# zkkli/I-ViT

Hardware: AMD Instinct MI355X
Metric: images/sec + int8-MFMA-roofline% for DeiT-S bs256@224 on 1/2/4/8 MI355X (higher is better)
Workload: dtype int8; 1 GPU; deit_small int8 forward, batch 256/GPU, 224x224x3 synthetic int8 (BASELINE.json configs[1]: DeiT-S b256 on one GPU); weights seeded synthetic, activation scales from the reference calibration; global_batch=256, parallelism=dp1 (batch-sharded, weights RCCL-broadcast once), streams_per_gpu=1, hipgraph=False

## Files before the change

### i-vit_amd/_lib.py

```python
import ctypes
import os
import subprocess

_CSRC = os.path.join(os.path.dirname(os.path.abspath(__file__)), "csrc")
SO_PATH = os.environ.get("IVIT_LIB") or os.path.join(_CSRC, "libivit_hip.so")
SOURCES = ["ivit_hip.hip"] + sorted(f for f in os.listdir(_CSRC) if f.endswith(".h"))
_THIS = os.path.abspath(__file__)
HIPCC_FLAGS = ["--offload-arch=gfx950", "-O3", "-std=c++17", "-ffp-contract=off", "-Wno-pass-failed", "-fPIC", "-shared",
               "-Xclang", "-target-feature", "-Xclang", "-packed-fp32-ops"]


IVIT_OK, IVIT_ERR_INVALID, IVIT_ERR_HIP, IVIT_ERR_UNSUPPORTED, IVIT_ERR_NO_DEVICE = 0, 1, 2, 3, 4


class IvitError(RuntimeError):
    pass


class Dyadic(ctypes.Structure):
    _fields_ = [("m", ctypes.c_double), ("r", ctypes.c_double)]


def build(force=False, verbose=False):
    srcs = [os.path.join(_CSRC, s) for s in SOURCES]
# ... 1 lines not shown
    newest = max(os.path.getmtime(p) for p in srcs + [hdr, _THIS])
    if not force and os.path.exists(SO_PATH) and os.path.getmtime(SO_PATH) >= newest:
        return SO_PATH
    hipcc = os.environ.get("HIPCC", "/opt/rocm/bin/hipcc")
    import fcntl
    with open(SO_PATH + ".lock", "w") as lock:
        fcntl.flock(lock, fcntl.LOCK_EX)
        if not force and os.path.exists(SO_PATH) and os.path.getmtime(SO_PATH) >= newest:
            return SO_PATH
        tmp = "%s.%d.tmp" % (SO_PATH, os.getpid())
        cmd = [hipcc] + HIPCC_FLAGS + [os.path.join(_CSRC, "ivit_hip.hip"), "-o", tmp]
        if verbose:
            print(" ".join(cmd))
        try:
            subprocess.check_call(cmd)
            os.replace(tmp, SO_PATH)
        finally:
            if os.path.exists(tmp):
                os.remove(tmp)
    return SO_PATH


class VitConfig(ctypes.Structure):
    _fields_ = [(n, ctypes.c_int) for n in ("img_size", "patch_size", "in_chans", "embed_dim", "depth", "num_heads",
                                             "hidden_dim", "num_classes")]


class VitBlock(ctypes.Structure):
    _fields_ = [
        ("s_ln1", ctypes.c_float), ("n1_bias_int", ctypes.c_void_p), ("n1_sc", ctypes.c_void_p), ("n1_dy", ctypes.c_void_p),
        ("qkv_w", ctypes.c_void_p), ("qkv_b", ctypes.c_void_p), ("qkv_dy", ctypes.c_void_p),
        ("dy_qk", Dyadic), ("s_softmax", ctypes.c_float), ("dy_pv", Dyadic),
        ("exp_aq", ctypes.c_void_p), ("exp_t", ctypes.c_void_p), ("exp_cls", ctypes.c_void_p),
        ("exp_nc", ctypes.c_int), ("exp_tcount", ctypes.c_int), ("exp_dmin", ctypes.c_int),
        ("proj_w", ctypes.c_void_p), ("proj_b", ctypes.c_void_p), ("proj_dy", ctypes.c_void_p),
        ("res1_main", Dyadic), ("res1_res", Dyadic),
        ("s_ln2", ctypes.c_float), ("n2_bias_int", ctypes.c_void_p), ("n2_sc", ctypes.c_void_p), ("n2_dy", ctypes.c_void_p),
        ("fc1_w", ctypes.c_void_p), ("fc1_b", ctypes.c_void_p), ("fc1_dy", ctypes.c_void_p),
        ("s_gelu", ctypes.c_float), ("dy_gelu", Dyadic),
        ("fc2_w", ctypes.c_void_p), ("fc2_b", ctypes.c_void_p), ("fc2_dy", ctypes.c_void_p),
        ("res2_main", Dyadic), ("res2_res", Dyadic),
    ]


class VitParams(ctypes.Structure):
    _fields_ = [
        ("pe_w", ctypes.c_void_p), ("pe_b", ctypes.c_void_p), ("pe_dy", ctypes.c_void_p),
        ("z_cls", ctypes.c_void_p), ("pos", ctypes.c_void_p), ("dy_x", Dyadic), ("dy_pos", Dyadic),
        ("blocks_host", ctypes.POINTER(VitBlock)),
        ("s_ln", ctypes.c_float), ("n_bias_int", ctypes.c_void_p), ("n_sc", ctypes.c_void_p), ("n_dy", ctypes.c_void_p),
        ("head_w", ctypes.c_void_p), ("head_b", ctypes.c_void_p),
    ]


class LnParams(ctypes.Structure):
    _fields_ = [("bias_int", ctypes.c_void_p), ("sc", ctypes.c_void_p), ("dy", ctypes.c_void_p)]


class LinParams(ctypes.Structure):
    _fields_ = [("w", ctypes.c_void_p), ("b", ctypes.c_void_p), ("dy", ctypes.c_void_p)]


class SwinConfigC(ctypes.Structure):
    _fields_ = [(n, ctypes.c_int) for n in ("img_size", "patch_size", "in_chans", "embed_dim", "num_layers", "window_size",
                                             "mlp_ratio", "num_classes")] + [("depths", ctypes.c_int * 4), ("num_heads", ctypes.c_int * 4)]


class SwinBlock(ctypes.Structure):
    _fields_ = [
        ("s_in", ctypes.c_float), ("n1", LnParams), ("qkv", LinParams),
        ("dy_qk", Dyadic), ("dy_a", Dyadic), ("relb", ctypes.c_void_p),
        ("s_softmax", ctypes.c_float), ("dy_pv", Dyadic), ("proj", LinParams),
        ("res1_main", Dyadic), ("res1_res", Dyadic),
        ("s_mid", ctypes.c_float), ("n2", LnParams), ("fc1", LinParams), ("s_gelu", ctypes.c_float), ("dy_gelu", Dyadic),
        ("fc2", LinParams), ("res2_main", Dyadic), ("res2_res", Dyadic),
        ("exp_aq", ctypes.c_void_p), ("exp_t", ctypes.c_void_p), ("exp_cls", ctypes.c_void_p),
        ("exp_nc", ctypes.c_int), ("exp_tcount", ctypes.c_int), ("exp_dmin", ctypes.c_int),
    ]


class SwinMerge(ctypes.Structure):
    _fields_ = [("s_in", ctypes.c_float), ("n", LnParams), ("red", LinParams)]


class SwinParams(ctypes.Structure):
    _fields_ = [
        ("pe", LinParams), ("s_bn", ctypes.c_float), ("pn", LnParams), ("dy_qact1", ctypes.c_void_p),
        ("blocks_host", ctypes.POINTER(SwinBlock)), ("merges_host", ctypes.POINTER(SwinMerge)),
        ("s_norm_in", ctypes.c_float), ("n", LnParams), ("dy_pool", Dyadic),
        ("head_w", ctypes.c_void_p), ("head_b", ctypes.c_void_p), ("s_pool", ctypes.c_float),
    ]


_P = ctypes.c_void_p
_I = ctypes.c_int
_L = ctypes.c_int64
_F = ctypes.c_float

SIGNATURES = {
    "ivit_create": [ctypes.POINTER(_P), _I, _P],
    "ivit_destroy": [_P],
    "ivit_set_stream": [_P, _P],
    "ivit_set_cu_share": [_P, ctypes.c_int],
    "ivit_quantize_input_f32": [_P, _P, _F, _P, _L],
    "ivit_normalize_quantize_u8": [_P, _P, _I, _I, _I, ctypes.POINTER(_F), ctypes.POINTER(_F), _F, _P],
    "ivit_resize_center_crop_u8": [_P, _P, _I, _I, _I, _I, _I, _P, _P],
    "ivit_requant_i16": [_P, _P, _P, _I, _P, _P, _I, _P, _L, _I],
    "ivit_layernorm_tokenorder_requant": [_P, _P, _L, _I, _F, _P, _P, _P, _I, _P],
    "ivit_patch_norm_tokenorder": [_P, _P, _L, _I, _F, _P, _P, _P, Dyadic, _I, _P],
    "ivit_window_attention_fused": [_P, _P, Dyadic, Dyadic, _P, _F, Dyadic, _P, _I, _I, _I, _I, _I, _I],
    "ivit_window_attention_fused_lut": [_P, _P, Dyadic, Dyadic, _P, _F, _P, _P, _P, _I, _I, _I, Dyadic, _P, _I, _I, _I, _I, _I, _I],
    "ivit_mlp_plan_create": [_P, _P, _P, ctypes.POINTER(_P)],
    "ivit_mlp_fused_planned": [_P, _P, _P, _P, Dyadic, Dyadic, _P, _P, _L],
    "ivit_layernorm_mlp_fused_planned": [_P, _P, _P, _F, _P, _P, _P, _P, _P, Dyadic, Dyadic, _P, _L],
    "ivit_layernorm_mlp_lockstep_planned": [_P, _P, _P, _F, _P, _P, _P, _P, Dyadic, Dyadic, _P, _L],
    "ivit_mlp_fused": [_P, _P, _P, _P, _P, _P, _P, _P, _P, Dyadic, Dyadic, _P, _P, _L, _I, _I],
    "ivit_patch_merge_gather": [_P, _P, _I, _I, _I, _I, _P],
    "ivit_widen_i8_i16": [_P, _P, _P, _L],
    "ivit_linear_i8_requant8_store16": [_P, _P, _P, _P, _P, _P, _I, _I, _I],
    "ivit_patch_merge_layernorm_requant": [_P, _P, _I, _I, _I, _F, _P, _P, _P, _P],
    "ivit_swin_create": [_P, ctypes.POINTER(SwinConfigC), ctypes.POINTER(SwinParams), _I, ctypes.POINTER(_P)],
    "ivit_swin_destroy": [_P],
    "ivit_swin_workspace_bytes": [_P, _I, _I, ctypes.POINTER(ctypes.c_size_t)],
    "ivit_swin_forward": [_P, _P, _I, _I, _P, ctypes.c_size_t, _P],
    "ivit_swin_graph_create": [_P, _P, _I, _I, _P, ctypes.c_size_t, _P, ctypes.POINTER(_P)],
    "ivit_vit_create": [_P, ctypes.POINTER(VitConfig), ctypes.POINTER(VitParams), _I, ctypes.POINTER(_P)],
    "ivit_vit_destroy": [_P],
    "ivit_vit_workspace_bytes": [_P, _I, _I, ctypes.POINTER(ctypes.c_size_t)],
    "ivit_vit_fused_mlp_blocks": [_P, _I, ctypes.POINTER(_I)],
    "ivit_vit_fused_ln_mlp_blocks": [_P, _I, ctypes.POINTER(_I)],
    "ivit_vit_fused_qkv_blocks": [_P, _I, ctypes.POINTER(_I)],
    "ivit_vit_cls_tail": [_P, _I, ctypes.POINTER(_I)],
    "ivit_swin_fused_mlp_blocks": [_P, _I, ctypes.POINTER(_I * 4)],
    "ivit_vit_workspace_init": [_P, _P, ctypes.c_size_t, _I, _I],
    "ivit_vit_forward": [_P, _P, _I, _I, _P, ctypes.c_size_t, _P],
    "ivit_vit_graph_create": [_P, _P, _I, _I, _P, ctypes.c_size_t, _P, ctypes.POINTER(_P)],
    "ivit_graph_launch": [_P],
    "ivit_graph_destroy": [_P],
    "ivit_linear_i8": [_P, _P, _P, _P, _P, _I, _I, _I],
    "ivit_linear_i8_requant": [_P, _P, _P, _P, _P, _I, _P, _I, _I, _I],
    "ivit_linear_i8_requant_residual": [_P, _P, _P, _P, _P, Dyadic, Dyadic, _P, _P, _I, _I, _I],
    "ivit_linear_i8_qkv": [_P, _P, _P, _P, _P, _P, _P, _P, _I, _I, _I, _I, _I],
    "ivit_constants_upload": [_P, _P, ctypes.c_size_t, _P],
    "ivit_constants_broadcast": [_P, _P, ctypes.c_size_t, _I, _P],
    "ivit_linear_plan_create": [_P, _P, _P, _P, _I, _I, ctypes.POINTER(_P)],
    "ivit_linear_i8_requant_planned": [_P, _P, _P, _I, _P, _I],
    "ivit_linear_i8_requant_residual_planned": [_P, _P, _P, Dyadic, Dyadic, _P, _P, _I],
    "ivit_linear_i8_qkv_planned": [_P, _P, _P, _P, _P, _P, _I, _I, _I, _I, _I],
    "ivit_linear_plan_prepare_ws": [_P, _P],
    "ivit_layernorm_linear_i8_requant_planned": [_P, _P, _P, _F, _P, _P, _P, _P, _I],
    "ivit_linear_i8_requant_residual_layernorm_planned": [_P, _P, _P, Dyadic, Dyadic, _P, _P, _I, _F, _P, _P, _P, _P],
    "ivit_layernorm_linear_i8_qkv_planned": [_P, _P, _P, _F, _P, _P, _P, _P, _P, _P, _I, _I, _I, _I],
    "ivit_layernorm_linear_i8_qkv_ldv_planned": [_P, _P, _P, _F, _P, _P, _P, _P, _P, _P, _I, _I, _I, _I, _I],
    "ivit_bmm_nt_i8": [_P, _P, _P, _P, _I, _I, _I, _I, _I, _I, _I, _L, _L, _L],
    "ivit_bmm_nt_u16i8": [_P, _P, _P, _P, _I, _I, _I, _I, _I, _I, _I, _L, _L, _L],
    "ivit_attn_qk_requant": [_P, _P, _P, Dyadic, _P, _I, _I, _I, _I],
    "ivit_attn_pv_requant": [_P, _P, _P, Dyadic, _P, _I, _I, _I, _I, _I, _I],
    "ivit_attention_fused": [_P, _P, _P, _P, Dyadic, _F, Dyadic, _P, _I, _I, _I, _I, _I],
    "ivit_attention_fused_lut": [_P, _P, _P, _P, Dyadic, _F, _P, _P, _P, _I, _I, _I, Dyadic, _P, _I, _I, _I, _I, _I],
    "ivit_shiftmax_rowtable": [_P, _P, _P, _P, _I, _I, _I, _P],
    "ivit_attention_fused_rowlut": [_P, _P, _P, _P, Dyadic, _F, _P, _I, Dyadic, _P, _I, _I, _I, _I, _I],
    "ivit_attention_fused_cls": [_P, _P, _P, _P, Dyadic, _F, Dyadic, _P, _P, _P, _I, _I, _I, _I, _I],
    "ivit_attention_fused_lut_cls": [_P, _P, _P, _P, Dyadic, _F, _P, _P, _P, _I, _I, _I, Dyadic, _P, _P, _P, _I, _I, _I, _I, _I],
    "ivit_attention_fused_rowlut_cls": [_P, _P, _P, _P, Dyadic, _F, _P, _I, Dyadic, _P, _P, _P, _I, _I, _I, _I, _I],
    "ivit_gather_rows_i16": [_P, _P, _L, _I, _L, _P],
    "ivit_requant_i32": [_P, _P, _P, _I, _P, _P, _I, _P, _L, _I],
    "ivit_requant_f32": [_P, _P, _P, _I, _P, _P, _I, _P, _L, _I],
    "ivit_shiftmax": [_P, _P, _L, _I, _I, _F, _I, _P, _I],
    "ivit_shiftgelu": [_P, _P, _L, _I, _F, _P],
    "ivit_shiftgelu_requant": [_P, _P, _L, _I, _F, Dyadic, _P],
    "ivit_shiftgelu_build_table": [_P, _F, Dyadic, _P],
    "ivit_shiftgelu_requant_lut": [_P, _P, _L, _I, _P, _P],
    "ivit_layernorm": [_P, _P, _L, _I, _F, _P, _P, _P],
    "ivit_layernorm_requant": [_P, _P, _L, _I, _L, _F, _P, _P, _P, _P],
    "ivit_shiftmax_masked": [_P, _P, _L, _I, _I, _F, _I, _P, _I, _I, _P, _I],
    "ivit_requant_i32_bcast": [_P, _P, Dyadic, _P, _L, Dyadic, _I, _P, _L],
    "ivit_avgpool_requant": [_P, _P, _I, _I, _I, Dyadic, _P],
    "ivit_avgpool_requant_scaled": [_P, _P, _I, _I, _I, _F, Dyadic, _P],
    "ivit_layernorm_tokenorder": [_P, _P, _L, _I, _F, _P, _P, _I, _P],
    "ivit_debug_div": [_P, _P, _P, _P, _P, _L],
    "ivit_debug_requotient": [_P, _P, _P, _P, _P, _L],
    "ivit_im2col_patch": [_P, _P, _I, _I, _I, _I, _I, _P],
    "ivit_embed_finish": [_P, _P, _P, _P, Dyadic, Dyadic, _P, _I, _I, _I],
    "ivit_patch_embed": [_P, _P, _I, _I, _I, _I, _I, _P, _P, _P, _P, _P, Dyadic, Dyadic, _P, _I],
    "ivit_logits_topk": [_P, _P, _P, _I, _I, _I, _P, _P],
    "ivit_vit_predict": [_P, _P, _I, _I, _P, ctypes.c_size_t, _P, _P, _I, _P, _P],
    "ivit_swin_predict": [_P, _P, _I, _I, _P, ctypes.c_size_t, _P, _P, _I, _P, _P],
    "ivit_vit_predict_graph_create": [_P, _P, _I, _I, _P, ctypes.c_size_t, _P, _P, _I, _P, _P, ctypes.POINTER(_P)],
    "ivit_swin_predict_graph_create": [_P, _P, _I, _I, _P, ctypes.c_size_t, _P, _P, _I, _P, _P, ctypes.POINTER(_P)],
}
OTHER_SYMBOLS = ["ivit_version", "ivit_status_string", "ivit_last_error", "ivit_linear_plan_destroy", "ivit_mlp_plan_destroy", "ivit_linear_plan_query", "ivit_mlp_plan_select"]

_lib = None


def load():
    global _lib
    if _lib is not None:
        return _lib
    if not os.path.exists(SO_PATH):
        raise IvitError(f"{SO_PATH} not built — run `python -c 'import __graft_entry__ as g; g.build()'`; "
                        "there is no CPU fallback for the product path")
    lib = ctypes.CDLL(SO_PATH)
    for name, args in SIGNATURES.items():
        fn = getattr(lib, name)
        fn.argtypes = args
        fn.restype = ctypes.c_int
    lib.ivit_version.restype = ctypes.c_int
    lib.ivit_status_string.restype = ctypes.c_char_p
    lib.ivit_status_string.argtypes = [ctypes.c_int]
    lib.ivit_last_error.restype = ctypes.c_char_p
    lib.ivit_last_error.argtypes = [_P]
    lib.ivit_linear_plan_destroy.argtypes = [_P]
    lib.ivit_linear_plan_destroy.restype = ctypes.c_int
    lib.ivit_linear_plan_query.argtypes = [_P, ctypes.POINTER(_I), ctypes.POINTER(_I)]
    lib.ivit_linear_plan_query.restype = ctypes.c_int
    lib.ivit_mlp_plan_select.argtypes = [_P, _I]
    lib.ivit_mlp_plan_select.restype = ctypes.c_int
    lib.ivit_mlp_plan_destroy.argtypes = [_P]
    lib.ivit_mlp_plan_destroy.restype = ctypes.c_int
    _lib = lib
    return lib


class Handle:

    def __init__(self, device=0, stream=None):
        self.lib = load()
        h = _P()
        st = self.lib.ivit_create(ctypes.byref(h), int(device), _P(stream or 0))
        if st != 0:
            raise IvitError(f"ivit_create(device={device}): {self.lib.ivit_status_string(st).decode()}")
        self.h = h
        self.device = device

    def set_stream(self, stream):
        self._check(self.lib.ivit_set_stream(self.h, _P(stream or 0)), "ivit_set_stream")

    def set_cu_share(self, cus):
        self._check(self.lib.ivit_set_cu_share(self.h, int(cus)), "ivit_set_cu_share")

    def _check(self, st, name):
        if st != 0:
            raise IvitError(f"{name}: {self.lib.ivit_status_string(st).decode()} "
                            f"({self.lib.ivit_last_error(self.h).decode()})")

    def call(self, name, *args):
        self._check(getattr(self.lib, name)(self.h, *args), name)

    def try_call(self, name, *args):
        self.unsupported = False

        def check(st, nm):
            if st == IVIT_ERR_UNSUPPORTED:
                self.unsupported = True
            else:
                self._check_plain(st, nm)
        self._check_plain, self._check = self._check, check
        try:
            self.call(name, *args)
        finally:
            self._check = self._check_plain
        return not self.unsupported

    def linear_plan(self, w, bias, dy, N, K):
        return LinearPlan(self, w, bias, dy, N, K)

    def close(self):
        if self.h:
            self.lib.ivit_destroy(self.h)
            self.h = None

    def __del__(self):
        try:
            self.close()
        except Exception:
            pass


class LinearPlan:

    def __init__(self, handle, w, bias, dy, N, K):
        self.lib = handle.lib
        p = _P()
        handle._check(self.lib.ivit_linear_plan_create(handle.h, w, bias, dy, int(N), int(K), ctypes.byref(p)),
                      "ivit_linear_plan_create")
        self.p = p
        a, b = _I(0), _I(0)
        self.lib.ivit_linear_plan_query(p, ctypes.byref(a), ctypes.byref(b))
        self.pipelined_ok, self.single_fma_ok = bool(a.value), bool(b.value)

    def close(self):
        if self.p:
            self.lib.ivit_linear_plan_destroy(self.p)
            self.p = None

    def __del__(self):
        try:
            self.close()
        except Exception:
            pass
```

### i-vit_amd/csrc/ivit_gemm_ws.h

```cpp
#pragma once
#include "ivit_layernorm.h"
#include <type_traits>

template <int K_, int MAXT_, bool VT_>
struct WsGeo {
    static constexpr int K = K_;
    static constexpr int KS = K_ / 32;
    static constexpr int KB = K_ / 64;
    static constexpr int MAXT = MAXT_;
    static constexpr int TOK = MAXT * 32;
    static constexpr int KBLK = TOK * 64;
    static constexpr int SOFF = KB * KBLK;
    static constexpr int SBIAS = SOFF + TOK * 4;
    static constexpr int MAXN = 1536;
    static constexpr int SCQ = SBIAS + MAXN * 4;
    static constexpr int SLN = SCQ + MAXN * 8;
    static constexpr int SVOFF = SLN + K * 20;
    static constexpr bool VT = VT_;
    static constexpr int SMEM = SVOFF + (VT ? TOK * 4 : 0);
    static_assert(K % 64 == 0 && TOK <= 512 && KBLK % 256 == 0, "whole K blocks; one thread per token of a panel; K blocks a whole number of bank periods apart");
    static_assert(SMEM <= 160 * 1024, "one workgroup per CU");
};
typedef WsGeo<384, 7, false> Ws384Geo;
typedef WsGeo<192, 14, true> Ws192Geo;
#define WS_MAXN 1536
inline bool ws_width(int K) { return K == Ws384Geo::K || K == Ws192Geo::K; }
#define WS_THREADS 512
#define WS_MAGIC 6755399441055744.0

struct WsArgs {
    const int8_t *x;
    const v4i *wf;
    const int32_t *bias;
    const double *cq;
    int8_t *q, *k, *v;
    int M, N, T, H;
    void *dummy;
    const int16_t *x16;
    float ln_s;
    int ldv;
    const float *ln_bias_int, *ln_sc;
    const ivit_dyadic *ln_dy;
    const int16_t *residual;
    int16_t *out16;
    double cm, cr;
    int8_t *ln_out8;
};
#define WS_EPI_QKV8 0
#define WS_EPI_RES16 1
#define WS_EPI_RQ8 2

__device__ __forceinline__ int ws_chan_of_row(int rho) { return ((rho >> 2) & 1) * 16 + (rho >> 3) * 4 + (rho & 3); }
__device__ __forceinline__ int ws_g(int tok) { return ((tok >> 1) & 3) ^ ((tok >> 3) & 3) ^ ((tok >> 4) & 1); }

__global__ __launch_bounds__(256) void ws_swizzle_kernel(const int8_t *__restrict__ w, v4i *__restrict__ wf, int N, int K) {
    const int nks = K / 32, nfrag = N / 32 * nks;
    for (int i = blockIdx.x * 256 + threadIdx.x; i < nfrag * 64; i += gridDim.x * 256) {
        const int l = i & 63, f = i >> 6, ct = f / nks, ks = f - ct * nks;
        const int ch = 32 * ct + ws_chan_of_row(l & 31);
        wf[i] = *reinterpret_cast<const v4i *>(w + (size_t)ch * K + 32 * ks + 16 * (l >> 5));
    }
}

template <class G, bool FMA, bool LN, int EPI = WS_EPI_QKV8, bool VT = false>
__global__ __launch_bounds__(WS_THREADS, 2) void gemm_ws_qkv_kernel(WsArgs p) {
    static_assert(!VT || (G::VT && EPI == WS_EPI_QKV8), "the v^T store form belongs to the qkv scatter of a geometry that keeps its table");
    static_assert(!(LN && EPI == WS_EPI_RES16) || G::K == 384, "norm2 in the proj launch is built at 384 only");
    extern __shared__ __attribute__((aligned(256))) char sm[];
    typedef double v2d __attribute__((ext_vector_type(2)));
    typedef __attribute__((address_space(3))) char lds_c;
    typedef __attribute__((address_space(3))) v4i lds_v4i;
    typedef __attribute__((address_space(3))) int lds_i32;
    typedef __attribute__((address_space(3))) unsigned lds_u32;
    typedef __attribute__((address_space(3))) v2d lds_v2d;
    const int wave = __builtin_amdgcn_readfirstlane(threadIdx.x >> 6);
    const unsigned sm_lds = (unsigned)(size_t)(lds_c *)sm;
    int tid = threadIdx.x;
    asm volatile("" : "+v"(tid));
    const int lane = tid & 63, tok = lane & 31, kh = lane >> 5, e = kh ^ ws_g(tok);

    const int ntt = (p.M + 31) >> 5;
    const int t_beg = (int)((long long)ntt * blockIdx.x / gridDim.x), t_end = (int)((long long)ntt * (blockIdx.x + 1) / gridDim.x);
    const int ncp = p.N >> 6, ncp3 = ncp / 3;
    for (int i = tid; i < p.N; i += WS_THREADS) {
        reinterpret_cast<int *>(sm + G::SBIAS)[i] = p.bias[i];
        reinterpret_cast<double *>(sm + G::SCQ)[i] = p.cq[i];
    }
    const unsigned lane16 = lane * 16;
    double *cC = reinterpret_cast<double *>(sm + G::SLN);
    float *cB = reinterpret_cast<float *>(sm + G::SLN + G::K * 8), *cSc = cB + G::K, *cY = cSc + G::K;
    bool ln_fast = false;
    constexpr bool LN_HEAD = LN && EPI != WS_EPI_RES16, LN_TAIL = LN && EPI == WS_EPI_RES16;
    if constexpr (LN) ln_fast = ln_stage_constants<G::K, WS_THREADS>(p.ln_bias_int, p.ln_sc, p.ln_dy, cC, cB, cSc, cY);

    for (int t0 = t_beg; t0 < t_end; t0 += G::MAXT) {
        const int n_own = min(G::MAXT, t_end - t0);
        if (t0 != t_beg) __syncthreads();
        if constexpr (LN_HEAD) {
            typedef LnGroup<G::K, 2> LG;
            const int j = lane & 7, k = j >> 1, hh = j & 1;
            const float ys = rcp_rn(p.ln_s);
            for (int r0 = wave * 8; r0 < n_own * 32; r0 += 64) {
                const int tokl = r0 + (lane >> 3);
                const long long row_raw = (long long)t0 * 32 + tokl;
                const bool live = row_raw < p.M;
                const int16_t *xp = p.x16 + (live ? row_raw : (long long)p.M - 1) * G::K + 8 * k + 4 * hh;
                float xv[LG::NSTEP][LG::EPC];
#pragma unroll
                for (int i = 0; i < LG::NSTEP; ++i) {
                    const LnRaw<4>::T t = *reinterpret_cast<const LnRaw<4>::T *>(xp + 32 * i);
#pragma unroll
                    for (int c = 0; c < 4; ++c) xv[i][c] = requotient_m((float)t[c], p.ln_s, ys);
                }
                const unsigned rowa = sm_lds + tokl * 64 + (k & 1) * 8 + 4 * hh, gk = (unsigned)((k >> 1) ^ ws_g(tokl));
                LG::run(xv, j, k, 8 * k + 4 * hh, ln_fast, live, cC, cB, cSc, cY,
                       [&](int i, unsigned pk0, unsigned) __attribute__((always_inline)) {
                           *(lds_u32 *)(size_t)(rowa + (i >> 1) * G::KBLK + ((gk ^ ((i & 1) * 2)) << 4)) = pk0;
                       });
            }
        } else {
            for (int tg = wave; tg < n_own * 2; tg += 8) {
                const int tokl = tg * 16 + (lane >> 2), c = (lane & 3) ^ ws_g(tokl);
                const long long grow = min((long long)t0 * 32 + tokl, (long long)p.M - 1);
                const int8_t *src = p.x + grow * G::K + c * 16;
#pragma unroll
                for (int kb = 0; kb < G::KB; ++kb) {
                    const unsigned dst = __builtin_amdgcn_readfirstlane((unsigned)(kb * G::KBLK + tg * 1024));
                    __builtin_amdgcn_global_load_lds((const __attribute__((address_space(1))) void *)(src + kb * 64),
                                                     (__attribute__((address_space(3))) void *)(sm + dst), 16, 0, 0);
                }
            }
        }
        if (tid < G::TOK) {
            const int row = min(t0 * 32 + tid, p.M - 1), b = row / p.T;
            reinterpret_cast<int *>(sm + G::SOFF)[tid] = (b * p.H * p.T + (row - b * p.T)) * 64;
            if constexpr (VT) reinterpret_cast<int *>(sm + G::SVOFF)[tid] = b * p.H * 64 * p.ldv + (row - b * p.T);
        }
        const int na = (n_own + 1) >> 1, ntask = n_own > 1 ? 2 * ncp : ncp;
        asm volatile("s_waitcnt vmcnt(0)" ::: "memory");
        __syncthreads();

        const unsigned fa0 = sm_lds + tok * 64 + e * 16, fa1 = sm_lds + tok * 64 + (e ^ 2) * 16;
        for (int task = wave; task < ntask; task += 8) {
            const int half = task >= ncp, cp = task - half * ncp;
            const int tb0 = half ? na : 0, te = half ? n_own : na;
            v4i W[2][G::KS];
            {
                const char *wq = reinterpret_cast<const char *>(p.wf + (size_t)cp * 2 * G::KS * 64);
#pragma unroll
                for (int c = 0; c < 2; ++c)
#pragma unroll
                    for (int ks = 0; ks < G::KS; ++ks) W[c][ks] = *reinterpret_cast<const v4i *>(wq + lane16 + (c * G::KS + ks) * 1024);
            }
            const int chb = 64 * cp + 16 * kh;
            const int which = EPI == WS_EPI_QKV8 ? cp / max(ncp3, 1) : 0;
            int8_t *obase = (which == 0 ? p.q : which == 1 ? p.k : p.v) + (size_t)(cp - which * ncp3) * p.T * 64 + 16 * kh;
            const bool vslab = VT && which == 2;
            int8_t *vbase = VT ? p.v + (size_t)((cp - 2 * ncp3) * 64 + 16 * kh) * p.ldv : nullptr;
            auto sweep = [&](auto nt_c, const int tb) __attribute__((always_inline)) {
                constexpr int NT = decltype(nt_c)::value;
                v4i bf[2][NT];
                v16i acc[2][NT];
                const unsigned fb0 = fa0 + tb * 2048, fb1 = fa1 + tb * 2048;
                int toff[NT];
#pragma unroll
                for (int t = 0; t < NT; ++t)
                    toff[t] = *(lds_i32 *)(size_t)(sm_lds + (vslab ? G::SVOFF : G::SOFF) + ((tb + t) * 32 + tok) * 4);
                auto load_b = [&](int ks, int slot) __attribute__((always_inline)) {
#pragma unroll
                    for (int t = 0; t < NT; ++t)
                        bf[slot][t] = *(lds_v4i *)(size_t)(((ks & 1) ? fb1 : fb0) + (ks >> 1) * G::KBLK + t * 2048);
                };
                load_b(0, 0);
                v4i idr[EPI == WS_EPI_RES16 ? 2 : 1][EPI == WS_EPI_RES16 ? NT : 1][2];
                if constexpr (EPI == WS_EPI_RES16) {
#pragma unroll
                    for (int c = 0; c < 2; ++c)
#pragma unroll
                        for (int t = 0; t < NT; ++t) {
                            const long long row = min((long long)(t0 + tb + t) * 32 + tok, (long long)p.M - 1);
                            const int16_t *rp = p.residual + row * p.N + chb + 32 * c;
                            idr[c][t][0] = *reinterpret_cast<const v4i *>(rp);
                            idr[c][t][1] = *reinterpret_cast<const v4i *>(rp + 8);
                        }
                }
#pragma unroll
                for (int c = 0; c < 2; ++c)
#pragma unroll
                    for (int q4 = 0; q4 < 4; ++q4) {
                        const v4i b4 = *(lds_v4i *)(size_t)(sm_lds + G::SBIAS + (chb + 32 * c + 4 * q4) * 4);
#pragma unroll
                        for (int t = 0; t < NT; ++t) { acc[c][t][4 * q4] = b4[0]; acc[c][t][4 * q4 + 1] = b4[1]; acc[c][t][4 * q4 + 2] = b4[2]; acc[c][t][4 * q4 + 3] = b4[3]; }
                    }
#pragma unroll
                for (int ks = 0; ks < G::KS; ++ks) {
                    __builtin_amdgcn_sched_barrier(0);
                    if (ks + 1 < G::KS) load_b(ks + 1, (ks + 1) & 1);
                    __builtin_amdgcn_sched_barrier(0);
#pragma unroll
                    for (int c = 0; c < 2; ++c)
#pragma unroll
                        for (int t = 0; t < NT; ++t)
                            acc[c][t] = __builtin_amdgcn_mfma_i32_32x32x32_i8(W[c][ks], bf[ks & 1][t], acc[c][t], 0, 0, 0);
                }
#pragma unroll
                for (int c = 0; c < 2; ++c) {
                    v2d cqv[8];
#pragma unroll
                    for (int j = 0; j < 8; ++j) cqv[j] = *(lds_v2d *)(size_t)(sm_lds + G::SCQ + (chb + 32 * c + 2 * j) * 8);
#pragma unroll
                    for (int t = 0; t < NT; ++t) {
                        if constexpr (EPI == WS_EPI_RES16) {
                            v4i o0, o1;
#pragma unroll
                            for (int d = 0; d < 8; ++d) {
                                const unsigned rw = (unsigned)(d < 4 ? idr[c][t][0][d] : idr[c][t][1][d - 4]);
                                int o[2];
#pragma unroll
                                for (int h2 = 0; h2 < 2; ++h2) {
                                    const int v = 2 * d + h2;
                                    const double m = cqv[v >> 1][v & 1];
                                    const double tq = FMA ? __builtin_fma((double)acc[c][t][v], m, WS_MAGIC) : ((double)acc[c][t][v] * m + WS_MAGIC);
                                    const int t16 = min(max(__double2loint(tq), -32768), 32767);
                                    const int r = h2 ? ((int)rw >> 16) : (int)(short)(rw & 0xffffu);
                                    o[h2] = rq_fast(r, p.cr) + rq_fast(t16, p.cm);
                                }
                                int pk;
                                asm("v_cvt_pk_i16_i32 %0, %1, %2" : "=v"(pk) : "v"(o[0]), "v"(o[1]));
                                if (d < 4) o0[d] = pk; else o1[d - 4] = pk;
                            }
                            asm volatile("" : "+v"(o0), "+v"(o1));
                            const long long row = (long long)(t0 + tb + t) * 32 + tok;
                            if (row < p.M) {
                                int16_t *op = p.out16 + row * p.N + chb + 32 * c;
                                *reinterpret_cast<v4i *>(op) = o0;
                                *reinterpret_cast<v4i *>(op + 8) = o1;
                            }
                            continue;
                        }
                        v4i o4;
#pragma unroll
                        for (int q4 = 0; q4 < 4; ++q4) {
                            int o[4];
#pragma unroll
                            for (int i = 0; i < 4; ++i) {
                                const double m = cqv[2 * q4 + (i >> 1)][i & 1];
                                const double tq = FMA ? __builtin_fma((double)acc[c][t][4 * q4 + i], m, WS_MAGIC + 128.0)
                                                      : ((double)acc[c][t][4 * q4 + i] * m + (WS_MAGIC + 128.0));
                                o[i] = __double2loint(tq);
                            }
                            unsigned p01, p23, b01, b23;
                            asm("v_cvt_pk_i16_i32 %0, %1, %2" : "=v"(p01) : "v"(o[0]), "v"(o[1]));
                            asm("v_cvt_pk_i16_i32 %0, %1, %2" : "=v"(p23) : "v"(o[2]), "v"(o[3]));
                            asm("v_sat_pk_u8_i16 %0, %1" : "=v"(b01) : "v"(p01));
                            asm("v_sat_pk_u8_i16 %0, %1" : "=v"(b23) : "v"(p23));
                            int hq = (int)(__builtin_amdgcn_perm(b23, b01, 0x05040100u) ^ 0x80808080u);
                            asm volatile("" : "+v"(hq));
                            o4[q4] = hq;
                        }
                        const int row = (t0 + tb + t) * 32 + tok;
                        if constexpr (EPI == WS_EPI_RQ8) {
                            if (row < p.M) *reinterpret_cast<v4i *>(p.q + (long long)row * p.N + chb + 32 * c) = o4;
                        } else if (vslab) {
                            if (row < p.M) {
                                int8_t *vp = vbase + toff[t] + (size_t)(32 * c) * p.ldv;
#pragma unroll
                                for (int i = 0; i < 16; ++i) vp[(size_t)i * p.ldv] = (int8_t)(o4[i >> 2] >> (8 * (i & 3)));
                            }
                        } else if constexpr (G::MAXT > 8) {
                            if (row < p.M) *reinterpret_cast<v4i *>(obase + toff[t] + 32 * c) = o4;
                        } else {
                            *reinterpret_cast<v4i *>(row < p.M ? obase + toff[t] + 32 * c : (int8_t *)p.dummy + lane16) = o4;
                        }
                    }
                }
            };
            int tb = tb0;
            if constexpr (G::MAXT <= 8) {
                if (te - tb > 2) { sweep(std::integral_constant<int, 2>{}, tb); tb += 2; }
                if (te - tb == 2) sweep(std::integral_constant<int, 2>{}, tb);
                else sweep(std::integral_constant<int, 1>{}, tb);
            } else {
                for (; te - tb >= 2; tb += 2) sweep(std::integral_constant<int, 2>{}, tb);
                if (te - tb == 1) sweep(std::integral_constant<int, 1>{}, tb);
            }
        }
        if constexpr (LN_TAIL) {
            asm volatile("s_waitcnt vmcnt(0)" ::: "memory");
            __syncthreads();
            typedef LnGroup<G::K, 2> LG;
            const int j = lane & 7, k = j >> 1, hh = j & 1;
            const float ys = rcp_rn(p.ln_s);
            for (int r0 = wave * 8; r0 < n_own * 32; r0 += 64) {
                const long long row_raw = (long long)t0 * 32 + r0 + (lane >> 3);
                const bool live = row_raw < p.M;
                const long long row = live ? row_raw : (long long)p.M - 1;
                const int16_t *xp = p.out16 + row * G::K + 8 * k + 4 * hh;
                float xv[LG::NSTEP][LG::EPC];
#pragma unroll
                for (int i = 0; i < LG::NSTEP; ++i) {
                    const LnRaw<4>::T t = *reinterpret_cast<const LnRaw<4>::T *>(xp + 32 * i);
#pragma unroll
                    for (int c = 0; c < 4; ++c) xv[i][c] = requotient_m((float)t[c], p.ln_s, ys);
                }
                LG::run(xv, j, k, 8 * k + 4 * hh, ln_fast, live, cC, cB, cSc, cY, p.ln_out8 + row * G::K + 8 * k + 4 * hh);
            }
        }
    }
}
```

### i-vit_amd/csrc/ivit_hip.hip

```cpp
#include <hip/hip_runtime.h>
#include <algorithm>
#include <stdio.h>
#include <stdlib.h>
#include <string.h>
#include <new>
#include <dlfcn.h>
#include <mutex>
#include <atomic>
#include <type_traits>
#include "ivit_device.h"
#include "ivit_elementwise.h"
#include "ivit_layernorm.h"
#include "ivit_gemm.h"
#include "ivit_attention.h"
#include "ivit_gemm2.h"
#include "ivit_gemm3.h"
#include "ivit_gemm_wreg.h"
#include "ivit_swin.h"
#include "ivit_mlp.h"
#include "ivit_mlp_rs.h"
#include "ivit_swin_mlp_rs.h"
#include "ivit_gemm_ws.h"
#include "ivit_swin12.h"
#include "ivit_topk.h"

#define IVIT_MAX_DEVICES 64
struct ivit_ctx {
    int device;
    hipStream_t stream;
    int num_cu;
    int cu_share;
    char err[256];
};
static inline int persistent_cus(const ivit_ctx *h) { return h->cu_share > 0 ? h->cu_share : h->num_cu; }

struct ivit_device_guard {
    int prev = -1;
    bool restore = false;
    bool enter(int dev) {
        if (hipGetDevice(&prev) != hipSuccess) prev = -1;
        if (prev == dev) return true;
        if (hipSetDevice(dev) != hipSuccess) return false;
        restore = prev >= 0;
        return true;
    }
    ~ivit_device_guard() { if (restore) (void)hipSetDevice(prev); }
};
#define CHECK_H(h) if (!(h)) return IVIT_ERR_INVALID; ivit_device_guard ivit_dev_guard_; if (!ivit_dev_guard_.enter((h)->device)) return IVIT_ERR_HIP
#define REQUIRE(h, cond, msg) do { if (!(cond)) { snprintf((h)->err, sizeof((h)->err), "%s: %s", __func__, msg); return IVIT_ERR_INVALID; } } while (0)
#define LAUNCH_CHECK(h) do { hipError_t e_ = hipGetLastError(); if (e_ != hipSuccess) { snprintf((h)->err, sizeof((h)->err), "%s: %s", __func__, hipGetErrorString(e_)); return IVIT_ERR_HIP; } } while (0)

template <auto Kernel, class... Args>
static int launch_dyn(ivit_handle h, dim3 grid, dim3 block, size_t lds, const Args &...args) {
    if (lds > 65536) {
        static std::atomic<int> max_dev[IVIT_MAX_DEVICES];
        const bool cached = h->device >= 0 && h->device < IVIT_MAX_DEVICES;
        if (!cached || max_dev[h->device].load(std::memory_order_acquire) < (int)lds) {
            hipError_t e = hipFuncSetAttribute((const void *)Kernel, hipFuncAttributeMaxDynamicSharedMemorySize, (int)lds);
            if (e != hipSuccess) { snprintf(h->err, sizeof(h->err), "hipFuncSetAttribute: %s", hipGetErrorString(e)); return IVIT_ERR_HIP; }
            if (cached) max_dev[h->device].store((int)lds, std::memory_order_release);
        }
    }
    Kernel<<<grid, block, lds, h->stream>>>(args...);
    return IVIT_OK;
}

template <class F>
static inline auto with_bool(bool on, F &&f) {
    if (on) return f(std::true_type{});
    return f(std::false_type{});
}
template <class F>
static inline auto with_width(int C, F &&f) {
    if (C == 96) return f(std::integral_constant<int, 96>{});
    return f(std::integral_constant<int, 128>{});
}

static inline bool rq_fast(ivit_dyadic d) { return fabs(d.m * d.r) < RQ_FAST_CLIM; }
static inline bool rq_fast2(ivit_dyadic a, ivit_dyadic b) { return rq_fast(a) && rq_fast(b); }
static inline bool attn_fast(ivit_dyadic dy_qk, ivit_dyadic dy_pv) { return fabs(dy_qk.m * dy_qk.r) < 512.0 && fabs(dy_pv.m * dy_pv.r) < 512.0; }

extern "C" {

int ivit_version(void) { return IVIT_VERSION; }

const char *ivit_status_string(int s) {
    switch (s) {
        case IVIT_OK: return "ok";
        case IVIT_ERR_INVALID: return "invalid argument";
        case IVIT_ERR_HIP: return "HIP runtime error";
        case IVIT_ERR_UNSUPPORTED: return "unsupported shape";
        case IVIT_ERR_NO_DEVICE: return "no HIP device";
        default: return "unknown status";
    }
}

int ivit_create(ivit_handle *out, int device, void *hip_stream) {
    if (!out) return IVIT_ERR_INVALID;
    int n = 0;
    if (hipGetDeviceCount(&n) != hipSuccess || n <= 0 || device < 0 || device >= n) return IVIT_ERR_NO_DEVICE;
    if (hipSetDevice(device) != hipSuccess) return IVIT_ERR_HIP;
    ivit_ctx *c = new (std::nothrow) ivit_ctx();
    if (!c) return IVIT_ERR_HIP;
    c->device = device;
    c->stream = (hipStream_t)hip_stream;
    c->err[0] = 0;
    c->cu_share = 0;
    hipDeviceProp_t prop;
    c->num_cu = (hipGetDeviceProperties(&prop, device) == hipSuccess) ? prop.multiProcessorCount : 256;
    *out = c;
    return IVIT_OK;
}

int ivit_destroy(ivit_handle h) {
    CHECK_H(h);
    delete h;
    return IVIT_OK;
}

int ivit_set_stream(ivit_handle h, void *hip_stream) {
    CHECK_H(h);
    h->stream = (hipStream_t)hip_stream;
    return IVIT_OK;
}

int ivit_set_cu_share(ivit_handle h, int cus) {
    CHECK_H(h);
    REQUIRE(h, cus >= 0, "cus must be >= 0 (0 = the whole device)");
    h->cu_share = cus > h->num_cu ? h->num_cu : cus;
    return IVIT_OK;
}

const char *ivit_last_error(ivit_handle h) { return h ? h->err : "null handle"; }

static inline int grid_for(ivit_handle h, long long work_items, int per_block) {
    long long g = (work_items + per_block - 1) / per_block;
    long long cap = (long long)h->num_cu * 16;
    if (g > cap) g = cap;
    if (g < 1) g = 1;
    return (int)g;
}

int ivit_quantize_input_f32(ivit_handle h, const float *x, float scale, int8_t *q, int64_t n) {
    CHECK_H(h);
    REQUIRE(h, x && q && n >= 0 && scale > 0.f, "bad arguments");
    if (n == 0) return IVIT_OK;
    quantize_input_kernel<<<grid_for(h, n, 1024), 256, 0, h->stream>>>(x, scale, q, n);
    LAUNCH_CHECK(h);
    return IVIT_OK;
}

int ivit_resize_center_crop_u8(ivit_handle h, const uint8_t *hwc, int B, int H0, int W0, int size, int crop,
                               float *workspace, uint8_t *out_hwc) {
    CHECK_H(h);
    REQUIRE(h, hwc && workspace && out_hwc && B > 0 && H0 > 0 && W0 > 0 && size > 0 && crop > 0, "bad arguments");
    int Hr, Wr;
    if (H0 <= W0) { Hr = size; Wr = (int)((long long)size * W0 / H0); }
    else { Wr = size; Hr = (int)((long long)size * H0 / W0); }
    REQUIRE(h, crop <= Hr && crop <= Wr, "crop larger than the resized image");
    const int top = (int)__builtin_rint((Hr - crop) / 2.0), left = (int)__builtin_rint((Wr - crop) / 2.0);
    resize_h_kernel<<<grid_for(h, (long long)B * H0 * crop, 256), 256, 0, h->stream>>>(hwc, B, H0, W0, Wr, left, crop, workspace);
    resize_v_kernel<<<grid_for(h, (long long)B * crop * crop, 256), 256, 0, h->stream>>>(workspace, B, H0, Hr, top, crop, out_hwc);
    LAUNCH_CHECK(h);
    return IVIT_OK;
}

int ivit_normalize_quantize_u8(ivit_handle h, const uint8_t *hwc, int B, int H, int W, const float mean[3],
// ... 220 lines not shown
    });
    if (!fn) { snprintf(h->err, sizeof(h->err), "ivit_constants_broadcast: librccl.so / ncclBroadcast not found"); return IVIT_ERR_UNSUPPORTED; }
    const int rc = fn(device_blob, device_blob, bytes,  1, root, rccl_comm, h->stream);
    if (rc != 0) { snprintf(h->err, sizeof(h->err), "ivit_constants_broadcast: ncclBroadcast returned %d", rc); return IVIT_ERR_HIP; }
    return IVIT_OK;
}

}

__global__ __launch_bounds__(256) void linear_plan_kernel(const int8_t *__restrict__ w, const int32_t *__restrict__ bias,
                                                          const ivit_dyadic *__restrict__ dy, int N, int K,
                                                          double *__restrict__ cq, int *__restrict__ bad) {
    const int lane = threadIdx.x & 63, n = blockIdx.x * 4 + (threadIdx.x >> 6);
    if (n >= N) return;
    const int8_t *wp = w + (long long)n * K;
    int l1 = 0;
    for (int k = lane; k < K; k += 64) l1 += abs((int)wp[k]);
#pragma unroll
    for (int o = 32; o > 0; o >>= 1) l1 += __shfl_xor(l1, o);
    if (lane == 0) {
        const double c = dy[n].m * dy[n].r;
        cq[n] = c;
        const double zmax = 128.0 * (double)l1 + fabs((double)(bias ? bias[n] : 0));
        int b = 0;
        if (!(fabs(c) * zmax < 2147483000.0)) b |= 1;
        if (!(fabs(dy[n].m) * zmax < 9007199254740992.0)) b |= 4;
        if (b) atomicOr(bad, b);
    }
}

__global__ __launch_bounds__(256) void linear_plan_fma_kernel(const int8_t *__restrict__ w, const int32_t *__restrict__ bias,
                                                              const ivit_dyadic *__restrict__ dy, int N, int K, int *__restrict__ bad) {
    __shared__ int s_l1, s_fail;
    const int n = blockIdx.x, tid = threadIdx.x;
    if (tid == 0) { s_l1 = 0; s_fail = 0; }
    __syncthreads();
    int l1 = 0;
    for (int k = tid; k < K; k += 256) l1 += abs((int)w[(long long)n * K + k]);
    atomicAdd(&s_l1, l1);
    __syncthreads();
    const double m = dy[n].m, r = dy[n].r, c = m * r;
    const double zmax = 128.0 * (double)s_l1 + fabs((double)(bias ? bias[n] : 0));
    if (fabs(m) * zmax < 9007199254740992.0) return;
    if (!(c > 0.0) || !(zmax < 2147483000.0)) { if (tid == 0) atomicOr(bad, 2); return; }
    auto f1 = [&](double z) { return __double2loint(__builtin_fma(z, c, 6755399441055744.0)); };
    auto f2 = [&](double z) { return (int)__builtin_rint((z * m) * r); };
    bool fail = false;
    for (int i = 0; i < 256 && !fail; ++i) {
        const int k = -32767 + tid + 256 * i;
        double z0 = __builtin_ceil(((double)k - 0.5) / c);
        for (int it = 0; it < 4 && z0 - 1.0 >= -zmax && f1(z0 - 1.0) >= k; ++it) z0 -= 1.0;
        for (int it = 0; it < 4 && z0 <= zmax && f1(z0) < k; ++it) z0 += 1.0;
        if (fabs(z0) * fabs(m) < 9.0e15) continue;
        if (z0 <= zmax && z0 >= -zmax && (f1(z0) < k || f2(z0) < k)) fail = true;
        if (z0 - 1.0 <= zmax && z0 - 1.0 >= -zmax && (f1(z0 - 1.0) >= k || f2(z0 - 1.0) >= k)) fail = true;
    }
    if (fail) atomicOr(&s_fail, 1);
    __syncthreads();
    if (tid == 0 && s_fail) atomicOr(bad, 2);
}

struct ivit_linear_plan_s {
    const int8_t *w;
    const int32_t *bias;
    const int32_t *bias_eff;
    const ivit_dyadic *dy;
    int N, K;
    char *dev;
    double *cq;
    void *dummy;
    int pipelined_ok, single_fma_ok;
    v4i *wf;
    int device;
};

extern "C" {

int ivit_linear_plan_create(ivit_handle h, const int8_t *w, const int32_t *bias, const ivit_dyadic *dy_ch, int N, int K,
                            ivit_linear_plan *out) {
    CHECK_H(h);
    REQUIRE(h, w && dy_ch && out && N > 0 && K > 0, "bad arguments");
    const size_t cq_bytes = ((size_t)N * 8 + 255) & ~(size_t)255, b_bytes = ((size_t)N * 4 + 255) & ~(size_t)255;
    char *dev = nullptr;
    hipError_t e = hipMalloc((void **)&dev, cq_bytes + b_bytes + 256 + 1024 + 8192);
    if (e != hipSuccess) { snprintf(h->err, sizeof(h->err), "ivit_linear_plan_create: hipMalloc: %s", hipGetErrorString(e)); return IVIT_ERR_HIP; }
    int *flag = (int *)(dev + cq_bytes + b_bytes);
    int host_bad = 3;
    bool ok = hipMemsetAsync(dev + cq_bytes, 0, b_bytes + 256 + 1024 + 8192, h->stream) == hipSuccess;
    if (ok) {
        linear_plan_kernel<<<(N + 3) / 4, 256, 0, h->stream>>>(w, bias, dy_ch, N, K, (double *)dev, flag);
        ok = hipGetLastError() == hipSuccess;
    }
    ok = ok && hipMemcpyAsync(&host_bad, flag, sizeof(int), hipMemcpyDeviceToHost, h->stream) == hipSuccess;
    ok = ok && hipStreamSynchronize(h->stream) == hipSuccess;
    if (ok && (host_bad & 4) && !(host_bad & 1)) {
        linear_plan_fma_kernel<<<N, 256, 0, h->stream>>>(w, bias, dy_ch, N, K, flag);
        ok = hipGetLastError() == hipSuccess;
        ok = ok && hipMemcpyAsync(&host_bad, flag, sizeof(int), hipMemcpyDeviceToHost, h->stream) == hipSuccess;
        ok = ok && hipStreamSynchronize(h->stream) == hipSuccess;
    } else if (host_bad & 4) {
        host_bad |= 2;
    }
    if (!ok) {
        snprintf(h->err, sizeof(h->err), "ivit_linear_plan_create: HIP error");
        (void)hipFree(dev);
        return IVIT_ERR_HIP;
    }
    ivit_linear_plan_s *p = new (std::nothrow) ivit_linear_plan_s();
    if (!p) { (void)hipFree(dev); return IVIT_ERR_HIP; }
    p->w = w; p->bias = bias; p->dy = dy_ch; p->N = N; p->K = K; p->dev = dev; p->cq = (double *)dev;
    p->bias_eff = bias ? bias : (const int32_t *)(dev + cq_bytes);
    p->dummy = dev + cq_bytes + b_bytes + 256;
    p->pipelined_ok = !(host_bad & 1);
    p->single_fma_ok = !(host_bad & 2);
    p->device = h->device;
    p->wf = nullptr;
    *out = p;
    return IVIT_OK;
}

int ivit_linear_plan_destroy(ivit_linear_plan p) {
    if (!p) return IVIT_ERR_INVALID;
    ivit_device_guard g;
    if (!g.enter(p->device)) return IVIT_ERR_HIP;
    (void)hipFree(p->dev);
    if (p->wf) (void)hipFree(p->wf);
    delete p;
    return IVIT_OK;
}

int ivit_linear_plan_query(ivit_linear_plan p, int *pipelined_ok, int *single_fma_ok) {
    if (!p) return IVIT_ERR_INVALID;
    if (pipelined_ok) *pipelined_ok = p->pipelined_ok;
    if (single_fma_ok) *single_fma_ok = p->single_fma_ok;
    return IVIT_OK;
}

}

static inline bool use_gemm3(const ivit_linear_plan_s *pl, const GemmArgs &a, int epi_bit) {
    constexpr int res_min_n = 512;
    if (epi_bit == 4 && a.N < res_min_n) return false;
    return pl->pipelined_ok && (a.K % 64) == 0 && a.K >= 320 && (a.N % 16) == 0 && (a.ldc % 16) == 0 &&
           (a.lda % 16) == 0 && (a.ldb % 16) == 0 && a.M >= 128;
}

static inline bool ws_plan_ok(const ivit_linear_plan_s *pl, long long M) { return pl->wf && ws_width(pl->K) && M < (1 << 26); }
static inline bool qkv_ws_ok(const ivit_linear_plan_s *pl, int B, int T, int H, int dh, int ldv = 0) {
    if (!(pl->wf && dh == 64 && ws_width(pl->K) && pl->N == 3 * H * dh && pl->N % 192 == 0 && (long long)B * H * T * 64 < (1ll << 31) &&
          (long long)B * T < (1ll << 26)))
        return false;
    return ldv == 0 || (pl->K == Ws192Geo::K && ldv >= T && ldv % 16 == 0 && (long long)B * H * 64 * ldv < (1ll << 31));
}
template <class G, bool LN, int EPI, bool VT = false>
static int ws_launch(ivit_handle h, const ivit_linear_plan_s *pl, const WsArgs &a) {
    const int ntt = (a.M + 31) / 32;
    const unsigned grid = (unsigned)(ntt < persistent_cus(h) ? ntt : persistent_cus(h));
    return with_bool(pl->single_fma_ok, [&](auto FMA) {
        return launch_dyn<gemm_ws_qkv_kernel<G, FMA(), LN, EPI, VT>>(h, grid, WS_THREADS, G::SMEM, a);
    });
}
template <class G>
static int launch_qkv_ws_g(ivit_handle h, const ivit_linear_plan_s *pl, const int8_t *x8, const int16_t *x16, float ln_s,
                           const float *ln_bias_int, const float *ln_sc, const ivit_dyadic *ln_dy, int8_t *q, int8_t *k, int8_t *v,
                           int B, int T, int H, int ldv) {
    if (h->device != pl->device) { snprintf(h->err, sizeof(h->err), "qkv: plan and handle live on different devices"); return IVIT_ERR_INVALID; }
    if (ldv != 0 && !G::VT) { snprintf(h->err, sizeof(h->err), "qkv: no v^T store form at K = %d", G::K); return IVIT_ERR_UNSUPPORTED; }
    WsArgs a;
    a.x = x8; a.wf = pl->wf; a.bias = pl->bias_eff; a.cq = pl->cq; a.q = q; a.k = k; a.v = v;
    a.M = B * T; a.N = pl->N; a.T = T; a.H = H; a.dummy = pl->dummy;
    a.x16 = x16; a.ln_s = ln_s; a.ln_bias_int = ln_bias_int; a.ln_sc = ln_sc; a.ln_dy = ln_dy;
    a.residual = nullptr; a.out16 = nullptr; a.cm = a.cr = 0.0; a.ln_out8 = nullptr; a.ldv = ldv;
    if (H == 0) { a.T = 1; a.H = 1; }
    const int st = with_bool(x16 != nullptr, [&](auto LN) {
        if (H == 0) return ws_launch<G, LN(), WS_EPI_RQ8>(h, pl, a);
        if constexpr (G::VT) {
            if (ldv != 0) return ws_launch<G, LN(), WS_EPI_QKV8, true>(h, pl, a);
        }
        return ws_launch<G, LN(), WS_EPI_QKV8>(h, pl, a);
    });
    if (st) return st;
    LAUNCH_CHECK(h);
    return IVIT_OK;
}
static int launch_qkv_ws(ivit_handle h, const ivit_linear_plan_s *pl, const int8_t *x8, const int16_t *x16, float ln_s,
                         const float *ln_bias_int, const float *ln_sc, const ivit_dyadic *ln_dy, int8_t *q, int8_t *k, int8_t *v,
                         int B, int T, int H, int ldv = 0) {
    return pl->K == Ws192Geo::K ? launch_qkv_ws_g<Ws192Geo>(h, pl, x8, x16, ln_s, ln_bias_int, ln_sc, ln_dy, q, k, v, B, T, H, ldv)
                                : launch_qkv_ws_g<Ws384Geo>(h, pl, x8, x16, ln_s, ln_bias_int, ln_sc, ln_dy, q, k, v, B, T, H, ldv);
}

template <class G>
static int launch_res_ws_g(ivit_handle h, const ivit_linear_plan_s *pl, const int8_t *x8, ivit_dyadic dy_main, ivit_dyadic dy_res, const int16_t *residual,
                           int16_t *out, int M, float ln_s, const float *ln_bias_int, const float *ln_sc, const ivit_dyadic *ln_dy,
                           int8_t *ln_out8) {
    constexpr bool TAIL = G::K == 384;
    if (h->device != pl->device) { snprintf(h->err, sizeof(h->err), "linear: plan and handle live on different devices"); return IVIT_ERR_INVALID; }
    if (ln_out8 && !TAIL) { snprintf(h->err, sizeof(h->err), "linear: no LayerNorm tail at K = %d", G::K); return IVIT_ERR_UNSUPPORTED; }
    WsArgs a;
    a.x = x8; a.wf = pl->wf; a.bias = pl->bias_eff; a.cq = pl->cq; a.q = a.k = a.v = nullptr;
    a.M = M; a.N = pl->N; a.T = 1; a.H = 1; a.dummy = pl->dummy;
    a.x16 = nullptr; a.ln_s = ln_s; a.ln_bias_int = ln_bias_int; a.ln_sc = ln_sc; a.ln_dy = ln_dy;
    a.residual = residual; a.out16 = out; a.cm = dy_main.m * dy_main.r; a.cr = dy_res.m * dy_res.r; a.ln_out8 = ln_out8; a.ldv = 0;
    int st = IVIT_OK;
    if (!ln_out8) st = ws_launch<G, false, WS_EPI_RES16>(h, pl, a);
    else if constexpr (TAIL) st = ws_launch<G, true, WS_EPI_RES16>(h, pl, a);
    if (st) return st;
    LAUNCH_CHECK(h);
    return IVIT_OK;
}
static int launch_res_ws(ivit_handle h, const ivit_linear_plan_s *pl, const int8_t *x8, ivit_dyadic dy_main, ivit_dyadic dy_res, const int16_t *residual,
                         int16_t *out, int M, float ln_s = 0.f, const float *ln_bias_int = nullptr, const float *ln_sc = nullptr,
                         const ivit_dyadic *ln_dy = nullptr, int8_t *ln_out8 = nullptr) {
    return pl->K == Ws192Geo::K ? launch_res_ws_g<Ws192Geo>(h, pl, x8, dy_main, dy_res, residual, out, M, ln_s, ln_bias_int, ln_sc, ln_dy, ln_out8)
                                : launch_res_ws_g<Ws384Geo>(h, pl, x8, dy_main, dy_res, residual, out, M, ln_s, ln_bias_int, ln_sc, ln_dy, ln_out8);
}

template <int EPI>
static int launch_gemm3(ivit_handle h, const ivit_linear_plan_s *pl, GemmArgs &a) {
    a.tiles_n = (a.N + 127) / 128;
    a.cq = pl->cq;
    a.bias = pl->bias_eff;
    a.dummy = pl->dummy;
    constexpr int wg_per_cu = 2;
    const bool fma = pl->single_fma_ok != 0;
    const long long out_bytes = (EPI == EPI_QKV) ? std::max((long long)a.M * a.D, (long long)(a.M / (a.T > 0 ? a.T : 1) + 1) * a.D * a.ldv)
                                                 : (long long)a.M * a.ldc * ((EPI == EPI_RQ8_CH) ? 1 : 2);
    const bool astat = (a.K % (GA_BK * GA_NK)) == 0 && a.M >= 256 && (a.N % 32) == 0 &&
                       (long long)a.M * a.lda < (1LL << 32) && (long long)a.N * a.ldb < (1LL << 32) &&
                       out_bytes < (1LL << 31) &&
                       (EPI != EPI_QKV || ((a.D % 128) == 0 && (a.dh % 32) == 0));
    if (astat) {
        const long long nunits = (long long)((a.M + 255) / 256) * a.tiles_n;
        long long grid = h->num_cu;
        if (grid > nunits) grid = nunits;
        const dim3 g((unsigned)grid);
        with_bool(fma, [&](auto FMA) {
            if (a.K == GA_BK * GA_NK) gemm_as_kernel<EPI, false, FMA()><<<g, 512, 0, h->stream>>>(a);
            else gemm_as_kernel<EPI, true, FMA()><<<g, 512, 0, h->stream>>>(a);
        });
    } else {
        const long long nunits = (long long)((a.M + 127) / 128) * a.tiles_n;
        long long grid = (long long)h->num_cu * wg_per_cu;
        if (grid > nunits) grid = nunits;
        with_bool(fma, [&](auto FMA) { gemm_ps_kernel<EPI, FMA(), false><<<dim3((unsigned)grid), 256, 0, h->stream>>>(a); });
    }
    LAUNCH_CHECK(h);
    return IVIT_OK;
}

extern "C" {

int ivit_linear_i8_requant_planned(ivit_handle h, ivit_linear_plan pl, const int8_t *x, int bits, void *out, int M) {
    CHECK_H(h);
    REQUIRE(h, pl && x && out && M > 0, "bad arguments");
    REQUIRE(h, bits == 8 || bits == 16, "bits must be 8 or 16");
    GemmArgs a = linear_args(x, pl->w, pl->bias, M, pl->N, pl->K);
    a.out = out; a.dy_ch = pl->dy;
    if (bits == 8 && ws_plan_ok(pl, M))
        return launch_qkv_ws(h, pl, x, nullptr, 0.f, nullptr, nullptr, nullptr, (int8_t *)out, nullptr, nullptr, M, 1, 0);
    if (use_gemm3(pl, a, 1)) return bits == 8 ? launch_gemm3<EPI_RQ8_CH>(h, pl, a) : launch_gemm3<EPI_RQ16_CH>(h, pl, a);
    return ivit_linear_i8_requant(h, x, pl->w, pl->bias, pl->dy, bits, out, M, pl->N, pl->K);
}

int ivit_layernorm_linear_i8_requant_planned(ivit_handle h, ivit_linear_plan pl, const int16_t *x16, float scale, const float *bias_int,
                                             const float *sc, const ivit_dyadic *ln_dy, int8_t *out8, int M) {
    CHECK_H(h);
    REQUIRE(h, pl && x16 && bias_int && sc && ln_dy && out8 && M > 0, "bad arguments");
    if (!ws_plan_ok(pl, M)) {
        snprintf(h->err, sizeof(h->err), "%s: needs ivit_linear_plan_prepare_ws on a K = 192 or 384 plan", __func__);
        return IVIT_ERR_UNSUPPORTED;
    }
    return launch_qkv_ws(h, pl, nullptr, x16, scale, bias_int, sc, ln_dy, out8, nullptr, nullptr, M, 1, 0);
}

int ivit_linear_i8_requant_residual_planned(ivit_handle h, ivit_linear_plan pl, const int8_t *x, ivit_dyadic dy_main,
                                            ivit_dyadic dy_res, const int16_t *residual, int16_t *out, int M) {
    CHECK_H(h);
    REQUIRE(h, pl && x && out && residual && M > 0, "bad arguments");
    GemmArgs a = linear_args(x, pl->w, pl->bias, M, pl->N, pl->K);
    a.out = out; a.dy_ch = pl->dy; a.dy_main = dy_main; a.dy_res = dy_res; a.residual = residual;
    const bool res_fast = rq_fast2(dy_main, dy_res);
    if (res_fast && ws_plan_ok(pl, M)) return launch_res_ws(h, pl, x, dy_main, dy_res, residual, out, M);
    if (use_gemm3(pl, a, 4) && res_fast) return launch_gemm3<EPI_RQ16_CH_RES>(h, pl, a);
    return ivit_linear_i8_requant_residual(h, x, pl->w, pl->bias, pl->dy, dy_main, dy_res, residual, out, M, pl->N, pl->K);
}

int ivit_linear_i8_requant_residual_layernorm_planned(ivit_handle h, ivit_linear_plan pl, const int8_t *x, ivit_dyadic dy_main,
                                                      ivit_dyadic dy_res, const int16_t *residual, int16_t *out, int M, float ln_scale,
                                                      const float *ln_bias_int, const float *ln_sc, const ivit_dyadic *ln_dy,
                                                      int8_t *ln_out8) {
    CHECK_H(h);
    REQUIRE(h, pl && x && out && residual && M > 0 && ln_bias_int && ln_sc && ln_dy && ln_out8, "bad arguments");
    if (!(pl->wf && rq_fast2(dy_main, dy_res) && pl->K == Ws384Geo::K && pl->N == Ws384Geo::K && M < (1 << 26))) {
        snprintf(h->err, sizeof(h->err), "%s: needs ivit_linear_plan_prepare_ws on a 384 x 384 plan and residual multipliers in the fast range", __func__);
        return IVIT_ERR_UNSUPPORTED;
    }
    return launch_res_ws(h, pl, x, dy_main, dy_res, residual, out, M, ln_scale, ln_bias_int, ln_sc, ln_dy, ln_out8);
}

int ivit_linear_i8_qkv_planned(ivit_handle h, ivit_linear_plan pl, const int8_t *x, int8_t *q, int8_t *k, int8_t *vt,
                               int B, int T, int H, int dh, int ldv) {
    CHECK_H(h);
    REQUIRE(h, pl && x && q && k && vt && B > 0 && T > 0 && H > 0 && dh > 0, "bad arguments");
    REQUIRE(h, (dh % 16) == 0, "head dim must be a multiple of 16");
    REQUIRE(h, ldv == 0 || ldv >= T, "ldv < T (0 = v row-major [B*H, T, dh])");
    const int D = H * dh;
    REQUIRE(h, pl->N == 3 * D && pl->K == D, "plan shape is not [3*H*dh, H*dh]");
    GemmArgs a = linear_args(x, pl->w, pl->bias, B * T, 3 * D, D);
    a.dy_ch = pl->dy; a.q = q; a.k = k; a.vt = vt;
    a.T = T; a.H = H; a.dh = dh; a.ldv = ldv; a.D = D;
    if (qkv_ws_ok(pl, B, T, H, dh, ldv)) return launch_qkv_ws(h, pl, x, nullptr, 0.f, nullptr, nullptr, nullptr, q, k, vt, B, T, H, ldv);
    if (use_gemm3(pl, a, 2) && (long long)B * T < (1 << 23)) return launch_gemm3<EPI_QKV>(h, pl, a);
    return ivit_linear_i8_qkv(h, x, pl->w, pl->bias, pl->dy, q, k, vt, B, T, H, dh, ldv);
}

int ivit_linear_plan_prepare_ws(ivit_handle h, ivit_linear_plan pl) {
    CHECK_H(h);
    REQUIRE(h, pl, "null plan");
    REQUIRE(h, h->device == pl->device, "plan and handle live on different devices");
    if (pl->wf) return IVIT_OK;
    if (!ws_width(pl->K) || pl->N % 64 != 0 || pl->N > WS_MAXN || !pl->pipelined_ok) {
        snprintf(h->err, sizeof(h->err), "%s: built for K = 192 or 384, N a multiple of 64 up to %d, |(acc + bias) * c| < 2^31", __func__, WS_MAXN);
        return IVIT_ERR_UNSUPPORTED;
    }
    v4i *wf = nullptr;
    hipError_t e = hipMalloc((void **)&wf, (size_t)pl->N * pl->K);
    if (e != hipSuccess) { snprintf(h->err, sizeof(h->err), "%s: hipMalloc: %s", __func__, hipGetErrorString(e)); return IVIT_ERR_HIP; }
    ws_swizzle_kernel<<<64, 256, 0, h->stream>>>(pl->w, wf, pl->N, pl->K);
    e = hipGetLastError();
    if (e == hipSuccess) e = hipStreamSynchronize(h->stream);
    if (e != hipSuccess) { (void)hipFree(wf); snprintf(h->err, sizeof(h->err), "%s: %s", __func__, hipGetErrorString(e)); return IVIT_ERR_HIP; }
    pl->wf = wf;
    return IVIT_OK;
}

int ivit_layernorm_linear_i8_qkv_planned(ivit_handle h, ivit_linear_plan pl, const int16_t *x16, float scale, const float *bias_int,
                                         const float *sc, const ivit_dyadic *ln_dy, int8_t *q, int8_t *k, int8_t *v, int B, int T,
                                         int H, int dh) {
    return ivit_layernorm_linear_i8_qkv_ldv_planned(h, pl, x16, scale, bias_int, sc, ln_dy, q, k, v, B, T, H, dh, 0);
}

int ivit_layernorm_linear_i8_qkv_ldv_planned(ivit_handle h, ivit_linear_plan pl, const int16_t *x16, float scale, const float *bias_int,
                                             const float *sc, const ivit_dyadic *ln_dy, int8_t *q, int8_t *k, int8_t *vt, int B, int T,
                                             int H, int dh, int ldv) {
    CHECK_H(h);
    REQUIRE(h, pl && x16 && bias_int && sc && ln_dy && q && k && vt && B > 0 && T > 0 && H > 0 && dh > 0, "bad arguments");
    REQUIRE(h, pl->N == 3 * H * dh && pl->K == H * dh, "plan shape is not [3*H*dh, H*dh]");
    REQUIRE(h, ldv == 0 || (ldv >= T && ldv % 16 == 0), "ldv: 0 (v row-major [B*H, T, dh]) or a multiple of 16 >= T (v^T)");
    if (!qkv_ws_ok(pl, B, T, H, dh, ldv)) {
        snprintf(h->err, sizeof(h->err), "%s: needs ivit_linear_plan_prepare_ws on a K = 192 or 384, dh = 64 plan, B*H*T*64 < 2^31, and K = 192 "
                                         "with B*H*64*ldv < 2^31 for v^T", __func__);
        return IVIT_ERR_UNSUPPORTED;
    }
    return launch_qkv_ws(h, pl, nullptr, x16, scale, bias_int, sc, ln_dy, q, k, vt, B, T, H, ldv);
}

}

struct ivit_mlp_plan_s {
    ivit_linear_plan fc1, fc2;
    int width;
    v4i *w1f, *w2f;
    v4i *w1r, *w2r;
    int fma;
    int kernel;
    int device;
};

extern "C" {

int ivit_mlp_plan_create(ivit_handle h, ivit_linear_plan fc1, ivit_linear_plan fc2, ivit_mlp_plan *out) {
    CHECK_H(h);
    REQUIRE(h, fc1 && fc2 && out, "null argument");
    const bool w384 = fc1->K == Mlp384Geo::C && fc1->N == Mlp384Geo::HD && fc2->K == Mlp384Geo::HD && fc2->N == Mlp384Geo::C;
    const bool w192 = fc1->K == Mlp192Geo::C && fc1->N == Mlp192Geo::HD && fc2->K == Mlp192Geo::HD && fc2->N == Mlp192Geo::C;
    const bool w256 = fc1->K == Mlp256Geo::C && fc1->N == Mlp256Geo::HD && fc2->K == Mlp256Geo::HD && fc2->N == Mlp256Geo::C;
    if (!w384 && !w256 && !w192) {
        snprintf(h->err, sizeof(h->err), "%s: built for 384 -> 1536 -> 384, 256 -> 1024 -> 256 and 192 -> 768 -> 192", __func__);
        return IVIT_ERR_UNSUPPORTED;
    }
    if (!fc1->pipelined_ok || !fc2->pipelined_ok) {
        snprintf(h->err, sizeof(h->err), "%s: |(acc + bias) * c| < 2^31 not provable for these weights", __func__);
        return IVIT_ERR_UNSUPPORTED;
    }
    const size_t wbytes = (size_t)fc1->K * fc1->N;
    char *dev = nullptr;
    if (hipMalloc((void **)&dev, (w384 ? 4 : 2) * wbytes) != hipSuccess) { snprintf(h->err, sizeof(h->err), "%s: hipMalloc failed", __func__); return IVIT_ERR_HIP; }
    if (w384) {
        mlp_swizzle_kernel<<<256, 256, 0, h->stream>>>(fc1->w, fc1->N, fc1->K, (v4i *)dev);
        mlp_swizzle_kernel<<<256, 256, 0, h->stream>>>(fc2->w, fc2->N, fc2->K, (v4i *)(dev + wbytes));
        rs_swizzle_w1_kernel<<<144, 256, 0, h->stream>>>(fc1->w, (v4i *)(dev + 2 * wbytes));
        rs_swizzle_w2_kernel<<<144, 256, 0, h->stream>>>(fc2->w, (v4i *)(dev + 3 * wbytes));
    } else if (w256) {
        mlp256_swizzle_kernel<<<256, 256, 0, h->stream>>>(fc1->w, fc1->N, fc1->K, (v4i *)dev);
        mlp256_swizzle_kernel<<<256, 256, 0, h->stream>>>(fc2->w, fc2->N, fc2->K, (v4i *)(dev + wbytes));
    } else {
        mlp192_swizzle_kernel<<<144, 256, 0, h->stream>>>(fc1->w, fc1->N, fc1->K, (v4i *)dev);
        mlp192_swizzle_kernel<<<144, 256, 0, h->stream>>>(fc2->w, fc2->N, fc2->K, (v4i *)(dev + wbytes));
    }
    hipError_t e = hipGetLastError();
    if (e == hipSuccess) e = hipStreamSynchronize(h->stream);
    ivit_mlp_plan_s *p = e == hipSuccess ? new (std::nothrow) ivit_mlp_plan_s() : nullptr;
    if (!p) {
        (void)hipFree(dev);
        snprintf(h->err, sizeof(h->err), "%s: %s", __func__, e == hipSuccess ? "out of memory" : hipGetErrorString(e));
        return IVIT_ERR_HIP;
    }
    p->fc1 = fc1; p->fc2 = fc2; p->width = fc1->K; p->w1f = (v4i *)dev; p->w2f = (v4i *)(dev + wbytes);
    p->w1r = w384 ? (v4i *)(dev + 2 * wbytes) : nullptr; p->w2r = w384 ? (v4i *)(dev + 3 * wbytes) : nullptr;
    p->fma = fc1->single_fma_ok && fc2->single_fma_ok;
    p->kernel = 0;
    p->device = h->device;
    *out = p;
    return IVIT_OK;
}

int ivit_mlp_plan_select(ivit_mlp_plan p, int kernel) {
    if (!p || kernel < 0 || kernel > 2) return IVIT_ERR_INVALID;
    if (p->width != Mlp384Geo::C && kernel == 2) return IVIT_ERR_UNSUPPORTED;
    p->kernel = kernel;
    return IVIT_OK;
}

int ivit_mlp_plan_destroy(ivit_mlp_plan p) {
    if (!p) return IVIT_ERR_INVALID;
    ivit_device_guard g;
    if (!g.enter(p->device)) return IVIT_ERR_HIP;
    (void)hipFree(p->w1f);
    delete p;
    return IVIT_OK;
}

static bool mlp_role_split(const ivit_ctx *h, ivit_mlp_plan p, long long M) {
    if (p->width != Mlp384Geo::C) return false;
    const long long ntiles = (M + 15) / 16, nunits = (ntiles + MLP_TT - 2) / (MLP_TT - 1);
    return p->kernel == 2 || (p->kernel == 0 && nunits > (long long)persistent_cus(h));
}
static bool ln_mlp_lockstep_ok(ivit_mlp_plan p, ivit_dyadic dy_main, ivit_dyadic dy_res) {
    return p && (p->width == Mlp192Geo::C || p->width == Mlp384Geo::C) && rq_fast2(dy_main, dy_res);
}
enum { LN_MLP_TWO_LAUNCHES = 0, LN_MLP_ROLE_SPLIT = 1, LN_MLP_LOCKSTEP = 2 };
static int ln_mlp_plan_fuses(const ivit_ctx *h, ivit_mlp_plan p, ivit_dyadic dy_main, ivit_dyadic dy_res, long long M) {
    if (!p || !rq_fast2(dy_main, dy_res)) return LN_MLP_TWO_LAUNCHES;
    if (mlp_role_split(h, p, M)) return LN_MLP_ROLE_SPLIT;
    return ln_mlp_lockstep_ok(p, dy_main, dy_res) ? LN_MLP_LOCKSTEP : LN_MLP_TWO_LAUNCHES;
}

static int mlp_fused_launch(ivit_handle h, ivit_mlp_plan p, const int8_t *x, const int8_t *gelu_table, ivit_dyadic dy_main,
                            ivit_dyadic dy_res, const int16_t *residual, int16_t *out, int64_t M, float ln_s, const float *ln_bias_int,
                            const float *ln_sc, const ivit_dyadic *ln_dy, bool ln_lockstep = false) {
    MlpArgs a;
    a.ln_s = ln_s; a.ln_bias_int = ln_bias_int; a.ln_sc = ln_sc; a.ln_dy = ln_dy;
    a.x = x; a.w1f = p->w1f; a.w2f = p->w2f; a.b1 = p->fc1->bias_eff; a.b2 = p->fc2->bias_eff;
    a.cq1 = p->fc1->cq; a.cq2 = p->fc2->cq; a.tab = gelu_table; a.residual = residual; a.out = out;
    a.cm = dy_main.m * dy_main.r; a.cr = dy_res.m * dy_res.r; a.M = M;
    if (!rq_fast2(dy_main, dy_res)) {
        snprintf(h->err, sizeof(h->err), "%s: residual multipliers out of the fast range", __func__);
        return IVIT_ERR_UNSUPPORTED;
    }
    REQUIRE(h, h->device == p->device, "plan and handle live on different devices");
    const long long ntiles = (M + 15) / 16;
    if (p->width != Mlp384Geo::C) {
        const bool w256 = p->width == Mlp256Geo::C;
        const long long slots = (long long)(w256 ? Mlp256Geo::WG_PER_CU : Mlp192Geo::WG_PER_CU) * persistent_cus(h);
        const unsigned grid = (unsigned)(ntiles < slots ? ntiles : slots);
        a.balanced = 1;
        const int st = with_bool(p->fma, [&](auto FMA) {
            if (ln_lockstep) return launch_dyn<mlp192ln_kernel<FMA()>>(h, grid, Mlp192Geo::THREADS, Mlp192Geo::SMEM_LN, a);
            return w256 ? launch_dyn<mlp256_kernel<FMA()>>(h, grid, Mlp256Geo::THREADS, Mlp256Geo::SMEM, a)
                        : launch_dyn<mlp192_kernel<FMA()>>(h, grid, Mlp192Geo::THREADS, Mlp192Geo::SMEM, a);
        });
        if (st) return st;
        LAUNCH_CHECK(h);
        return IVIT_OK;
    }
    const long long nunits = (ntiles + MLP_TT - 2) / (MLP_TT - 1);
    const unsigned grid = (unsigned)(nunits < persistent_cus(h) ? nunits : persistent_cus(h));
    const long long rounds_fixed = (nunits + grid - 1) / grid, rounds_bal = (ntiles + (long long)MLP_TT * grid - 1) / ((long long)MLP_TT * grid);
    a.balanced = rounds_bal < rounds_fixed;
    const bool role_split = !ln_lockstep && mlp_role_split(h, p, M);
    if (ln_dy && !role_split && !ln_lockstep) {
        snprintf(h->err, sizeof(h->err), "%s: the LayerNorm prologue exists in the role-split kernel only (two units per CU or more)", __func__);
        return IVIT_ERR_UNSUPPORTED;
    }
    if (role_split) { a.w1f = p->w1r; a.w2f = p->w2r; }
    const int st = with_bool(p->fma, [&](auto FMA) {
        if (ln_lockstep) return launch_dyn<mlp384ln_kernel<FMA()>>(h, grid, MLP_THREADS, Mlp384Geo::SMEM_LN, a);
        if (!role_split) return launch_dyn<mlp384_kernel<FMA()>>(h, grid, MLP_THREADS, MLP_SMEM, a);
        return ln_dy ? launch_dyn<mlp384rs_kernel<FMA(), 1>>(h, grid, RS_THREADS, RS_SMEM, a)
                     : launch_dyn<mlp384rs_kernel<FMA()>>(h, grid, RS_THREADS, RS_SMEM, a);
    });
    if (st) return st;
    LAUNCH_CHECK(h);
    return IVIT_OK;
}

static int mlp128_launch(ivit_handle h, const int8_t *x, const int8_t *w1, const int32_t *b1, const ivit_dyadic *dy1, const int8_t *gelu_table,
                         const int8_t *w2, const int32_t *b2, const ivit_dyadic *dy2, ivit_dyadic dy_main, ivit_dyadic dy_res,
                         const int16_t *residual, int16_t *out, int64_t M) {
    MlpArgs a;
    memset(&a, 0, sizeof(a));
    a.x = x; a.w1f = reinterpret_cast<const v4i *>(w1); a.w2f = reinterpret_cast<const v4i *>(w2); a.b1 = b1; a.b2 = b2;
    a.cq1 = reinterpret_cast<const double *>(dy1); a.cq2 = reinterpret_cast<const double *>(dy2);
    a.tab = gelu_table; a.residual = residual; a.out = out;
    a.cm = dy_main.m * dy_main.r; a.cr = dy_res.m * dy_res.r; a.M = M; a.balanced = 1;
    if (!rq_fast2(dy_main, dy_res)) {
        snprintf(h->err, sizeof(h->err), "ivit_mlp_fused: residual multipliers out of the fast range at C = 128");
        return IVIT_ERR_UNSUPPORTED;
    }
// ... 42 lines not shown

template <int NB, bool FAST, int TT = 0, int LUT = 0, bool VROW = false, bool CLS = false>
static int launch_attn2(ivit_handle h, const AttnArgs &a, int BH) {
    const size_t lds = AttCfg<NB>::SMEM + (LUT == 2 ? (size_t)ATT_ROWLINE_BYTES
                                                   : (LUT == 1 ? (size_t)((a.t_count + 3) & ~3) * 4 + (size_t)a.nc * 512 + 256 : 0));
    if (int st = launch_dyn<attn_fused_kernel<NB, FAST, TT, LUT, VROW, CLS>>(h, BH, ATT_WAVES * 64, lds, a)) return st;
    LAUNCH_CHECK(h);
    return IVIT_OK;
}

template <int NB>
static int launch_attn(ivit_handle h, const AttnArgs &a, int BH) {
    const bool fast = attn_fast(a.dy_qk, a.dy_pv);
    const bool lut = a.aq && a.et && a.cls;
    if (a.rowtab)
        return with_bool(a.ldv == 0, [&](auto VROW) {
            if (NB == 4 && a.T == 197) return launch_attn2<NB, true, 197, 2, VROW()>(h, a, BH);
            if (NB == 10 && a.T == 577) return launch_attn2<NB, true, 577, 2, VROW()>(h, a, BH);
            return launch_attn2<NB, true, 0, 2, VROW()>(h, a, BH);
        });
    if (fast) {
        if (NB == 4 && a.T == 197) return lut ? launch_attn2<NB, true, 197, true>(h, a, BH) : launch_attn2<NB, true, 197>(h, a, BH);
        if (NB == 10 && a.T == 577) return lut ? launch_attn2<NB, true, 577, true>(h, a, BH) : launch_attn2<NB, true, 577>(h, a, BH);
    }
    if (fast && lut) return launch_attn2<NB, true, 0, true>(h, a, BH);
    return fast ? launch_attn2<NB, true>(h, a, BH) : launch_attn2<NB, false>(h, a, BH);
}

template <int NB>
static int launch_attn_cls(ivit_handle h, const AttnArgs &a, int BH) {
    const bool fast = attn_fast(a.dy_qk, a.dy_pv);
    const bool lut = a.aq && a.et && a.cls;
    if (a.rowtab) return with_bool(a.ldv == 0, [&](auto VROW) { return launch_attn2<NB, true, 0, 2, VROW(), true>(h, a, BH); });
    if (fast && lut) return launch_attn2<NB, true, 0, 1, false, true>(h, a, BH);
    return fast ? launch_attn2<NB, true, 0, 0, false, true>(h, a, BH) : launch_attn2<NB, false, 0, 0, false, true>(h, a, BH);
}

static int attention_fused_impl(ivit_handle h, const int8_t *q, const int8_t *k, const int8_t *vt, ivit_dyadic dy_qk,
                                float s_softmax, ivit_dyadic dy_pv, int8_t *ctx8, int B, int H, int T, int dh, int ldv,
                                const uint16_t *aq, const float *et, const uint8_t *cls, int nc, int t_count, int dmin,
                                const float *rowtab = nullptr, bool cls_out = false, const int16_t *x16 = nullptr, int16_t *x_cls = nullptr) {
    CHECK_H(h);
    REQUIRE(h, q && k && vt && ctx8 && B > 0 && H > 0 && T > 0 && s_softmax > 0.f, "bad arguments");
    REQUIRE(h, (x16 == nullptr) == (x_cls == nullptr) && (cls_out || !x16), "x16 and x_cls go together (both null: no identity rows)");
    REQUIRE(h, !cls_out || (((uintptr_t)x16 | (uintptr_t)x_cls | (uintptr_t)ctx8) & 15) == 0, "ctx_cls, x16 and x_cls must be 16-byte aligned");
    REQUIRE(h, ((ldv % 16) == 0 && ldv >= T) || (ldv == 0 && rowtab), "ldv must be a multiple of 16 and >= T (0 = v row-major: ivit_attention_fused_rowlut only)");
    if (dh != 64 || T > 640) {
        snprintf(h->err, sizeof(h->err), "ivit_attention_fused: built for dh == 64, T <= 640");
        return IVIT_ERR_UNSUPPORTED;
    }
    if (aq) REQUIRE(h, et && cls && nc >= 1 && nc <= 64 && t_count >= 1 && t_count <= 16384 && dmin <= 0 && dmin >= -255,
                    "bad Shiftmax tables");
    if (aq) REQUIRE(h, (((uintptr_t)aq | (uintptr_t)et) & 15) == 0 && ((uintptr_t)cls & 3) == 0,
                    "Shiftmax tables: exp_aq and exp_t must be 16-byte aligned, exp_cls 4-byte aligned (copied in 16-byte pieces)");
    AttnArgs a;
    a.q = q; a.k = k; a.vt = vt; a.ctx = ctx8; a.T = T; a.H = H; a.ldv = ldv;
    a.s_softmax = s_softmax; a.dy_qk = dy_qk; a.dy_pv = dy_pv;
    a.aq = aq; a.et = et; a.cls = cls; a.nc = nc; a.t_count = t_count; a.dmin = dmin; a.rowtab = rowtab;
    a.nq = cls_out ? 1 : 0; a.ctx_rows = cls_out ? 1 : T; a.x16 = x16; a.x_cls = x_cls;
    if (cls_out) {
        if (T <= 64) return launch_attn_cls<1>(h, a, B * H);
        if (T <= 256) return launch_attn_cls<4>(h, a, B * H);
        return launch_attn_cls<10>(h, a, B * H);
    }
    if (T <= 64) return launch_attn<1>(h, a, B * H);
    if (T <= 256) return launch_attn<4>(h, a, B * H);
    return launch_attn<10>(h, a, B * H);
}

extern "C" int ivit_attention_fused(ivit_handle h, const int8_t *q, const int8_t *k, const int8_t *vt,
                                    ivit_dyadic dy_qk, float s_softmax, ivit_dyadic dy_pv, int8_t *ctx8, int B,
                                    int H, int T, int dh, int ldv) {
    return attention_fused_impl(h, q, k, vt, dy_qk, s_softmax, dy_pv, ctx8, B, H, T, dh, ldv, nullptr, nullptr, nullptr, 0, 0, 0);
}

extern "C" int ivit_attention_fused_lut(ivit_handle h, const int8_t *q, const int8_t *k, const int8_t *vt,
                                        ivit_dyadic dy_qk, float s_softmax, const uint16_t *exp_aq, const float *exp_t,
                                        const uint8_t *exp_cls, int nclass, int t_count, int dmin, ivit_dyadic dy_pv,
                                        int8_t *ctx8, int B, int H, int T, int dh, int ldv) {
    if (h && !(exp_aq && exp_t && exp_cls)) { snprintf(h->err, sizeof(h->err), "ivit_attention_fused_lut: null table"); return IVIT_ERR_INVALID; }
    return attention_fused_impl(h, q, k, vt, dy_qk, s_softmax, dy_pv, ctx8, B, H, T, dh, ldv, exp_aq, exp_t, exp_cls, nclass, t_count, dmin);
}

__global__ __launch_bounds__(64) void shiftmax_rowtable_kernel(const uint16_t *__restrict__ aq, const float *__restrict__ et,
                                                               const uint8_t *__restrict__ cls, int dmin, float *__restrict__ rowtab) {
    const int q = blockIdx.x, dd = threadIdx.x, R = 1 - dmin;
    int vi = q + dmin + dd;
    float val = 0.f;
    if (dd < R && (vi >= 0 || dd == 0)) {
        vi = vi < 0 ? 0 : vi;
        val = et[(int)aq[(int)cls[q] * 256 + vi] + dd];
    }
    rowtab[q * 64 + dd] = val;
}

extern "C" int ivit_shiftmax_rowtable(ivit_handle h, const uint16_t *exp_aq, const float *exp_t, const uint8_t *exp_cls,
                                      int nclass, int t_count, int dmin, float *rowtab) {
    CHECK_H(h);
    REQUIRE(h, exp_aq && exp_t && exp_cls && rowtab && nclass >= 1 && nclass <= 64 && t_count >= 1 && t_count <= 16384 &&
                   dmin <= 0 && dmin >= -255, "bad Shiftmax tables");
    if (1 - dmin > 64) {
        snprintf(h->err, sizeof(h->err), "%s: a table line holds 64 entries, this scale needs %d (use ivit_attention_fused_lut)", __func__, 1 - dmin);
        return IVIT_ERR_UNSUPPORTED;
    }
    REQUIRE(h, ((uintptr_t)rowtab & 15) == 0, "rowtab must be 16-byte aligned");
    shiftmax_rowtable_kernel<<<256, 64, 0, h->stream>>>(exp_aq, exp_t, exp_cls, dmin, rowtab);
    LAUNCH_CHECK(h);
    return IVIT_OK;
}

static int attention_rowlut(ivit_handle h, const int8_t *q, const int8_t *k, const int8_t *vt, ivit_dyadic dy_qk, float s_softmax,
                            const float *rowtab, int dmin, ivit_dyadic dy_pv, int8_t *ctx8, int B, int H, int T, int dh, int ldv,
                            bool cls_out, const int16_t *x16, int16_t *x_cls) {
    if (!h) return IVIT_ERR_INVALID;
    const char *entry = cls_out ? "ivit_attention_fused_rowlut_cls" : "ivit_attention_fused_rowlut";
    if (!(rowtab && ((uintptr_t)rowtab & 15) == 0 && dmin <= 0 && dmin >= -63)) {
        snprintf(h->err, sizeof(h->err), "%s: bad row table (16-byte aligned, 1 - dmin <= 64)", entry);
        return IVIT_ERR_INVALID;
    }
    if (!attn_fast(dy_qk, dy_pv)) {
        snprintf(h->err, sizeof(h->err), "%s: requant multipliers out of the fast range (use ivit_attention_fused_lut%s)", entry, cls_out ? "_cls" : "");
        return IVIT_ERR_UNSUPPORTED;
    }
    return attention_fused_impl(h, q, k, vt, dy_qk, s_softmax, dy_pv, ctx8, B, H, T, dh, ldv, nullptr, nullptr, nullptr, 0, 0, dmin, rowtab,
                                cls_out, x16, x_cls);
}

extern "C" int ivit_attention_fused_rowlut(ivit_handle h, const int8_t *q, const int8_t *k, const int8_t *vt,
                                           ivit_dyadic dy_qk, float s_softmax, const float *rowtab, int dmin, ivit_dyadic dy_pv,
                                           int8_t *ctx8, int B, int H, int T, int dh, int ldv) {
    return attention_rowlut(h, q, k, vt, dy_qk, s_softmax, rowtab, dmin, dy_pv, ctx8, B, H, T, dh, ldv, false, nullptr, nullptr);
}

extern "C" int ivit_attention_fused_cls(ivit_handle h, const int8_t *q, const int8_t *k, const int8_t *vt, ivit_dyadic dy_qk,
                                        float s_softmax, ivit_dyadic dy_pv, int8_t *ctx_cls, const int16_t *x16, int16_t *x_cls,
                                        int B, int H, int T, int dh, int ldv) {
    return attention_fused_impl(h, q, k, vt, dy_qk, s_softmax, dy_pv, ctx_cls, B, H, T, dh, ldv, nullptr, nullptr, nullptr, 0, 0, 0,
                                nullptr, true, x16, x_cls);
}

extern "C" int ivit_attention_fused_lut_cls(ivit_handle h, const int8_t *q, const int8_t *k, const int8_t *vt, ivit_dyadic dy_qk,
                                            float s_softmax, const uint16_t *exp_aq, const float *exp_t, const uint8_t *exp_cls,
                                            int nclass, int t_count, int dmin, ivit_dyadic dy_pv, int8_t *ctx_cls,
                                            const int16_t *x16, int16_t *x_cls, int B, int H, int T, int dh, int ldv) {
    if (h && !(exp_aq && exp_t && exp_cls)) { snprintf(h->err, sizeof(h->err), "%s: null table", __func__); return IVIT_ERR_INVALID; }
    return attention_fused_impl(h, q, k, vt, dy_qk, s_softmax, dy_pv, ctx_cls, B, H, T, dh, ldv, exp_aq, exp_t, exp_cls, nclass, t_count,
                                dmin, nullptr, true, x16, x_cls);
}

extern "C" int ivit_attention_fused_rowlut_cls(ivit_handle h, const int8_t *q, const int8_t *k, const int8_t *vt, ivit_dyadic dy_qk,
                                               float s_softmax, const float *rowtab, int dmin, ivit_dyadic dy_pv, int8_t *ctx_cls,
                                               const int16_t *x16, int16_t *x_cls, int B, int H, int T, int dh, int ldv) {
    return attention_rowlut(h, q, k, vt, dy_qk, s_softmax, rowtab, dmin, dy_pv, ctx_cls, B, H, T, dh, ldv, true, x16, x_cls);
}

__global__ __launch_bounds__(256) void gather_rows16_kernel(const int16_t *__restrict__ x, long long row_stride, int C8, long long n,
                                                            int16_t *__restrict__ out) {
    const long long i = (long long)blockIdx.x * 256 + threadIdx.x;
    if (i >= n) return;
    const long long r = i / C8;
    const int c = (int)(i - r * C8);
    reinterpret_cast<v4i *>(out)[i] = *reinterpret_cast<const v4i *>(x + r * row_stride + c * 8);
}

extern "C" int ivit_gather_rows_i16(ivit_handle h, const int16_t *x, int64_t rows, int C, int64_t row_stride, int16_t *out) {
    CHECK_H(h);
    REQUIRE(h, x && out && rows > 0 && C > 0 && row_stride >= C, "bad arguments");
    REQUIRE(h, (C % 8) == 0 && (row_stride % 8) == 0 && (((uintptr_t)x | (uintptr_t)out) & 15) == 0, "C and row_stride multiples of 8, x and out 16-byte aligned");
    const long long n = (long long)rows * (C / 8);
    REQUIRE(h, n < (1LL << 31) * 256, "too many rows");
    gather_rows16_kernel<<<(unsigned)((n + 255) / 256), 256, 0, h->stream>>>(x, row_stride, C / 8, n, out);
    LAUNCH_CHECK(h);
    return IVIT_OK;
}

template <typename ZT>
static int requant_any(ivit_handle h, const ZT *z, const ivit_dyadic *dy, int nch, const int32_t *z_id,
                       const ivit_dyadic *dy_id, int bits, void *out, int64_t rows, int C) {
    const long long total = (long long)rows * C;
    if ((C % 8) == 0 && nch == 1) {
        const int g8 = grid_for(h, total / 8, 256 * 2);
        if (bits == 8) requant_vec8_kernel<ZT, 8><<<g8, 256, 0, h->stream>>>(z, dy, nch, z_id, dy_id, out, total / 8, C / 8);
        else if (bits == 16) requant_vec8_kernel<ZT, 16><<<g8, 256, 0, h->stream>>>(z, dy, nch, z_id, dy_id, out, total / 8, C / 8);
        else requant_vec8_kernel<ZT, 32><<<g8, 256, 0, h->stream>>>(z, dy, nch, z_id, dy_id, out, total / 8, C / 8);
        LAUNCH_CHECK(h);
        return IVIT_OK;
    }
    const int g = grid_for(h, total, 256 * 4);
    if (bits == 8) requant_kernel<ZT, 8><<<g, 256, 0, h->stream>>>(z, dy, nch, z_id, dy_id, out, total, C);
    else if (bits == 16) requant_kernel<ZT, 16><<<g, 256, 0, h->stream>>>(z, dy, nch, z_id, dy_id, out, total, C);
    else requant_kernel<ZT, 32><<<g, 256, 0, h->stream>>>(z, dy, nch, z_id, dy_id, out, total, C);
    LAUNCH_CHECK(h);
    return IVIT_OK;
}

extern "C" {

int ivit_requant_i32(ivit_handle h, const int32_t *z, const ivit_dyadic *dy, int nch, const int32_t *z_id,
                     const ivit_dyadic *dy_id, int bits, void *out, int64_t rows, int C) {
    CHECK_H(h);
    REQUIRE(h, z && dy && out && rows > 0 && C > 0, "bad arguments");
    REQUIRE(h, nch == 1 || nch == C, "nch must be 1 or C");
    REQUIRE(h, bits == 8 || bits == 16 || bits == 32, "bits must be 8, 16 or 32");
    REQUIRE(h, (z_id == nullptr) == (dy_id == nullptr), "z_id and dy_id go together");
    return requant_any<int32_t>(h, z, dy, nch, z_id, dy_id, bits, out, rows, C);
}

int ivit_requant_i16(ivit_handle h, const int16_t *z, const ivit_dyadic *dy, int nch, const int32_t *z_id,
                     const ivit_dyadic *dy_id, int bits, void *out, int64_t rows, int C) {
    CHECK_H(h);
    REQUIRE(h, z && dy && out && rows > 0 && C > 0, "bad arguments");
    REQUIRE(h, nch == 1 || nch == C, "nch must be 1 or C");
    REQUIRE(h, bits == 8 || bits == 16 || bits == 32, "bits must be 8, 16 or 32");
    REQUIRE(h, (z_id == nullptr) == (dy_id == nullptr), "z_id and dy_id go together");
    return requant_any<int16_t>(h, z, dy, nch, z_id, dy_id, bits, out, rows, C);
}

int ivit_requant_f32(ivit_handle h, const float *z, const ivit_dyadic *dy, int nch, const int32_t *z_id,
                     const ivit_dyadic *dy_id, int bits, void *out, int64_t rows, int C) {
    CHECK_H(h);
    REQUIRE(h, z && dy && out && rows > 0 && C > 0, "bad arguments");
    REQUIRE(h, nch == 1 || nch == C, "nch must be 1 or C");
    REQUIRE(h, bits == 8 || bits == 16 || bits == 32, "bits must be 8, 16 or 32");
    REQUIRE(h, (z_id == nullptr) == (dy_id == nullptr), "z_id and dy_id go together");
    return requant_any<float>(h, z, dy, nch, z_id, dy_id, bits, out, rows, C);
}


int ivit_shiftmax(ivit_handle h, const int8_t *x, int64_t rows, int n, int ld_in, float scale, int out_bits,
                  uint16_t *out, int ld_out) {
    CHECK_H(h);
    REQUIRE(h, x && out && rows > 0 && n > 0 && ld_in >= n && ld_out >= n && scale > 0.f, "bad arguments");
    REQUIRE(h, out_bits == 8 || out_bits == 16, "out_bits must be 8 or 16");
    const size_t lds = (size_t)4 * n * sizeof(float);
    REQUIRE(h, lds <= 160 * 1024, "row too long for LDS staging");
    if (int st = launch_dyn<shiftmax_kernel>(h, (unsigned)((rows + 3) / 4), 256, lds, x, rows, n, ld_in, scale, out_bits, out, ld_out)) return st;
    LAUNCH_CHECK(h);
    return IVIT_OK;
}

static float host_shift_exp(float x, float x0, float nx0, int n) {
    float t = x + floorf(x * 0.5f);
    t = t - floorf(x * 0.0625f);
    t = fmaxf(t, nx0);
    const float q = floorf(t / x0);
    const float r = t - x0 * q;
    float e = r * 0.5f - x0;
    e = floorf(ldexpf(e, n - (int)q));
    return fmaxf(e, 0.0f);
}

static void shiftgelu_product_range(float s, int *lo, int *hi) {
    static thread_local float cs = 0.f;
    static thread_local int clo = 0, chi = 0;
    if (s != cs) {
        const float x0 = floorf(-1.0f / (s * 1.702f)), nx0 = 23.0f * x0;
        float p[256];
        for (int q = -128; q < 128; ++q) p[q + 128] = ((float)q * s) / s;
        float mn = 0.f, mxv = 0.f;
        for (int qmax = -128; qmax < 128; ++qmax) {
            const float mx = p[qmax + 128];
            const float emax = host_shift_exp(-mx, x0, nx0, 23);
            for (int q = -128; q <= qmax; ++q) {
                const float e = host_shift_exp(p[q + 128] - mx, x0, nx0, 23);
                const float S = fminf(e + emax, 2147483648.0f);
                const float F = floorf((1.0f / S) * 2147483648.0f);
                const float sig = floorf((e * F) * 5.9604644775390625e-08f);
                const float prod = rintf(p[q + 128] * sig);
                mn = fminf(mn, prod);
                mxv = fmaxf(mxv, prod);
            }
        }
        clo = (int)fmaxf(mn, -2147483648.0f);
        chi = (int)fminf(mxv, 2147483520.0f);
        cs = s;
    }
    *lo = clo;
    *hi = chi;
}

int ivit_shiftgelu(ivit_handle h, const int8_t *x, int64_t rows, int C, float scale, int16_t *out16) {
    CHECK_H(h);
    REQUIRE(h, x && out16 && rows > 0 && C > 0 && scale > 0.f, "bad arguments");
    REQUIRE(h, (C % 16) == 0, "C must be a multiple of 16");
    int lo, hi;
    shiftgelu_product_range(scale, &lo, &hi);
    if (lo < -32768 || hi > 32767) {
        snprintf(h->err, sizeof(h->err),
                 "ivit_shiftgelu: at scale %.9g Q*sigmoid_int spans [%d, %d] and does not fit the 16-bit output; use "
                 "ivit_shiftgelu_requant or the table form", (double)scale, lo, hi);
        return IVIT_ERR_UNSUPPORTED;
    }
    ivit_dyadic d = {0.0, 0.0};
    shiftgelu_kernel<false><<<(unsigned)((rows + 3) / 4), 256, 0, h->stream>>>(x, rows, C, scale, d, out16);
    LAUNCH_CHECK(h);
    return IVIT_OK;
}

int ivit_shiftgelu_requant(ivit_handle h, const int8_t *x, int64_t rows, int C, float scale, ivit_dyadic dy,
                           int8_t *out8) {
    CHECK_H(h);
    REQUIRE(h, x && out8 && rows > 0 && C > 0 && scale > 0.f, "bad arguments");
    REQUIRE(h, (C % 16) == 0, "C must be a multiple of 16");
    shiftgelu_kernel<true><<<(unsigned)((rows + 3) / 4), 256, 0, h->stream>>>(x, rows, C, scale, dy, out8);
    LAUNCH_CHECK(h);
    return IVIT_OK;
// ... 440 lines not shown
```

### i-vit_amd/csrc/ivit_model.h

```cpp
#pragma once
#include <vector>

struct ivit_graph_s {
    ivit_handle h;
    hipGraph_t graph;
    hipGraphExec_t exec;
};

namespace {

struct SliceRunner {
    std::vector<ivit_handle> slice_h;
    std::vector<hipStream_t> streams;
    std::vector<hipEvent_t> done;
    hipEvent_t fork = nullptr;

    bool create(ivit_handle h, int max_slices) {
        if (max_slices <= 1) return true;
        bool ok = hipEventCreateWithFlags(&fork, hipEventDisableTiming) == hipSuccess;
        for (int i = 0; ok && i < max_slices; ++i) {
            hipStream_t st = nullptr;
            hipEvent_t ev = nullptr;
            ivit_handle sh = nullptr;
            ok = hipStreamCreateWithFlags(&st, hipStreamNonBlocking) == hipSuccess;
            if (ok) streams.push_back(st);
            ok = ok && hipEventCreateWithFlags(&ev, hipEventDisableTiming) == hipSuccess;
            if (ok) done.push_back(ev);
            ok = ok && ivit_create(&sh, h->device, st) == IVIT_OK;
            if (ok) slice_h.push_back(sh);
        }
        return ok;
    }
    void destroy() {
        for (auto sh : slice_h) ivit_destroy(sh);
        for (auto ev : done) (void)hipEventDestroy(ev);
        for (auto st : streams) (void)hipStreamDestroy(st);
        if (fork) (void)hipEventDestroy(fork);
    }
};

inline int slice_begin(int batch, int nslices, int i) { return (int)(((long long)batch * i) / nslices); }
inline int max_slice(int batch, int nslices) { return (batch + nslices - 1) / nslices; }

template <class Body>
int fork_join(const SliceRunner &r, ivit_handle h, int batch, int nslices, Body &&body) {
    if (nslices == 1) return body(h, 0, 0, batch);
    if (hipEventRecord(r.fork, h->stream) != hipSuccess) return IVIT_ERR_HIP;
    for (int i = 0; i < nslices; ++i) {
        const int b0 = slice_begin(batch, nslices, i), b1 = slice_begin(batch, nslices, i + 1);
        if (hipStreamWaitEvent(r.streams[i], r.fork, 0) != hipSuccess) return IVIT_ERR_HIP;
        r.slice_h[i]->cu_share = std::max(1, persistent_cus(h) / nslices);
        const int rc = body(r.slice_h[i], i, b0, b1 - b0);
        if (rc != IVIT_OK) { snprintf(h->err, sizeof(h->err), "%s", r.slice_h[i]->err); return rc; }
        if (hipEventRecord(r.done[i], r.streams[i]) != hipSuccess) return IVIT_ERR_HIP;
    }
    for (int i = 0; i < nslices; ++i)
        if (hipStreamWaitEvent(h->stream, r.done[i], 0) != hipSuccess) return IVIT_ERR_HIP;
    return IVIT_OK;
}

template <class Fwd>
int graph_capture(ivit_handle h, ivit_graph *out, Fwd &&forward) {
    REQUIRE(h, out, "null argument");
    REQUIRE(h, h->stream != nullptr, "graph capture needs a non-default stream on the handle");
    hipError_t e = hipStreamBeginCapture(h->stream, hipStreamCaptureModeRelaxed);
    if (e != hipSuccess) { snprintf(h->err, sizeof(h->err), "begin capture: %s", hipGetErrorString(e)); return IVIT_ERR_HIP; }
    const int rc = forward();
    hipGraph_t graph = nullptr;
    e = hipStreamEndCapture(h->stream, &graph);
    if (rc != IVIT_OK) { if (graph) (void)hipGraphDestroy(graph); return rc; }
    if (e != hipSuccess || !graph) { snprintf(h->err, sizeof(h->err), "end capture: %s", hipGetErrorString(e)); return IVIT_ERR_HIP; }
    hipGraphExec_t exec = nullptr;
    e = hipGraphInstantiate(&exec, graph, nullptr, nullptr, 0);
    if (e != hipSuccess) { (void)hipGraphDestroy(graph); snprintf(h->err, sizeof(h->err), "instantiate: %s", hipGetErrorString(e)); return IVIT_ERR_HIP; }
    ivit_graph_s *g = new (std::nothrow) ivit_graph_s();
    if (!g) { (void)hipGraphExecDestroy(exec); (void)hipGraphDestroy(graph); return IVIT_ERR_HIP; }
    g->h = h; g->graph = graph; g->exec = exec;
    *out = g;
    return IVIT_OK;
}

#define RUN(call) do { const int rc_ = (call); if (rc_ != IVIT_OK) return rc_; } while (0)
template <class Fallback>
int fused_or(int fused, Fallback &&fallback) { return fused == IVIT_ERR_UNSUPPORTED ? fallback() : fused; }

template <class Model>
int8_t *gelu_table(const Model *m, int i) { return m->gelu_tab + (size_t)i * 65536; }

}

struct ivit_vit_s {
    ivit_handle h;
    ivit_vit_config cfg;
    ivit_vit_params prm;
    std::vector<ivit_vit_block> blocks;
    int T, ld, Kp, num_patches;
    bool fused_attention;
    int8_t *gelu_tab;
    float *rowtab;
    std::vector<char> has_rowtab;
    std::vector<ivit_linear_plan> plans;
    std::vector<ivit_mlp_plan> mlp_plans;
    int max_slices;
    SliceRunner run;
};

namespace {

inline size_t al256(size_t n) { return (n + 255) & ~(size_t)255; }

struct SliceLayout {
    size_t patches, patch16, xa, xb, a8, q, k, vt, ctx8, h8, g8, cls8, s8, p16, total;
};

SliceLayout slice_layout(const ivit_vit_s *m, int B) {
    const ivit_vit_config &c = m->cfg;
    const size_t M = (size_t)B * m->T, D = c.embed_dim, H = c.num_heads, dh = D / H, Hd = c.hidden_dim;
    SliceLayout L;
    size_t o = 0;
    auto take = [&](size_t bytes) { size_t at = o; o = al256(o + bytes); return at; };
    L.patches = take((size_t)B * m->num_patches * m->Kp);
    L.patch16 = take((size_t)B * m->num_patches * D * 2);
    L.xa = take(M * D * 2);
    L.xb = take(M * D * 2);
    L.a8 = take(M * D);
    L.q = take((size_t)B * H * m->T * dh);
    L.k = take((size_t)B * H * m->T * dh);
    L.vt = take((size_t)B * H * dh * m->ld);
    L.ctx8 = take(M * D);
    L.h8 = take(M * Hd);
    L.g8 = take(M * Hd);
    L.cls8 = take((size_t)B * D);
    L.s8 = L.p16 = 0;
    if (!m->fused_attention) {
        L.s8 = take((size_t)B * H * m->T * m->ld);
        L.p16 = take((size_t)B * H * m->T * m->ld * 2);
    }
    L.total = o;
    return L;
}

inline bool mlp_plan_shape(int C, int Hd) {
    return (C == Mlp384Geo::C && Hd == Mlp384Geo::HD) || (C == Mlp256Geo::C && Hd == Mlp256Geo::HD) || (C == Mlp192Geo::C && Hd == Mlp192Geo::HD);
}

inline bool mlp_plan_fuses(ivit_mlp_plan mp, ivit_dyadic res_main, ivit_dyadic res_res, long long ) {
    return mp && rq_fast2(res_main, res_res);
}

inline bool qkv_plan_fuses(const ivit_vit_s *m, int i, int B) {
    const int H = m->cfg.num_heads, ldv = (m->fused_attention && m->has_rowtab[i]) ? 0 : m->ld;
    return qkv_ws_ok(m->plans[4 * i], B, m->T, H, m->cfg.embed_dim / H, ldv);
}

inline bool cls_tail(const ivit_vit_s *m) {
    return m->fused_attention && (size_t)m->num_patches * m->Kp >= (size_t)m->cfg.embed_dim;
}

int vit_attention(const ivit_vit_s *m, ivit_handle h, int i, const int8_t *q, const int8_t *k, const int8_t *vt, int8_t *ctx, int B, int ldv,
                  bool cls, const int16_t *x16, int16_t *x_cls) {
    const ivit_vit_block &b = m->blocks[i];
    const int T = m->T, H = m->cfg.num_heads, dh = m->cfg.embed_dim / H;
    if (m->has_rowtab[i]) {
        const float *rowtab = m->rowtab + (size_t)i * 256 * 64;
        return cls ? ivit_attention_fused_rowlut_cls(h, q, k, vt, b.dy_qk, b.s_softmax, rowtab, b.exp_dmin, b.dy_pv, ctx, x16, x_cls, B, H, T, dh, ldv)
                   : ivit_attention_fused_rowlut(h, q, k, vt, b.dy_qk, b.s_softmax, rowtab, b.exp_dmin, b.dy_pv, ctx, B, H, T, dh, ldv);
    }
    if (b.exp_aq)
        return cls ? ivit_attention_fused_lut_cls(h, q, k, vt, b.dy_qk, b.s_softmax, b.exp_aq, b.exp_t, b.exp_cls, b.exp_nc, b.exp_tcount, b.exp_dmin,
                                                  b.dy_pv, ctx, x16, x_cls, B, H, T, dh, ldv)
                   : ivit_attention_fused_lut(h, q, k, vt, b.dy_qk, b.s_softmax, b.exp_aq, b.exp_t, b.exp_cls, b.exp_nc, b.exp_tcount, b.exp_dmin,
                                              b.dy_pv, ctx, B, H, T, dh, ldv);
    return cls ? ivit_attention_fused_cls(h, q, k, vt, b.dy_qk, b.s_softmax, b.dy_pv, ctx, x16, x_cls, B, H, T, dh, ldv)
               : ivit_attention_fused(h, q, k, vt, b.dy_qk, b.s_softmax, b.dy_pv, ctx, B, H, T, dh, ldv);
}

int run_slice(const ivit_vit_s *m, ivit_handle h, const int8_t *images, int B, int Bmax, char *ws, int32_t *logits) {
    const ivit_vit_config &c = m->cfg;
    const ivit_vit_params &P = m->prm;
    const int T = m->T, D = c.embed_dim, H = c.num_heads, dh = D / H, Hd = c.hidden_dim, ld = m->ld;
    const int M = B * T;
    const SliceLayout L = slice_layout(m, Bmax);
    int8_t *patches = (int8_t *)(ws + L.patches), *a8 = (int8_t *)(ws + L.a8), *q = (int8_t *)(ws + L.q),
           *k = (int8_t *)(ws + L.k), *vt = (int8_t *)(ws + L.vt), *ctx8 = (int8_t *)(ws + L.ctx8),
           *h8 = (int8_t *)(ws + L.h8), *g8 = (int8_t *)(ws + L.g8), *cls8 = (int8_t *)(ws + L.cls8);
    int16_t *patch16 = (int16_t *)(ws + L.patch16), *x = (int16_t *)(ws + L.xa), *y = (int16_t *)(ws + L.xb);
    RUN(fused_or((m->Kp == c.in_chans * c.patch_size * c.patch_size)
                     ? ivit_patch_embed(h, images, B, c.in_chans, c.img_size, c.img_size, c.patch_size, P.pe_w, P.pe_b, P.pe_dy, P.z_cls, P.pos, P.dy_x, P.dy_pos, x, D)
                     : IVIT_ERR_UNSUPPORTED,
                 [&] {
                     RUN(ivit_im2col_patch(h, images, B, c.in_chans, c.img_size, c.img_size, c.patch_size, patches));
                     RUN(ivit_linear_i8_requant(h, patches, P.pe_w, P.pe_b, P.pe_dy, 16, patch16, B * m->num_patches, D, m->Kp));
                     return ivit_embed_finish(h, patch16, P.z_cls, P.pos, P.dy_x, P.dy_pos, x, B, T, D);
                 }));
    for (int i = 0; i < c.depth; ++i) {
        const ivit_vit_block &b = m->blocks[i];
        const int ldv = (m->fused_attention && m->has_rowtab[i]) ? 0 : ld;
        const bool tail = i == c.depth - 1 && cls_tail(m);
        const int Mb = tail ? B : M;
        RUN(fused_or(qkv_plan_fuses(m, i, B) ? ivit_layernorm_linear_i8_qkv_ldv_planned(h, m->plans[4 * i], x, b.s_ln1, b.n1_bias_int, b.n1_sc, b.n1_dy,
                                                                                        q, k, vt, B, T, H, dh, ldv)
                                             : IVIT_ERR_UNSUPPORTED,
                     [&] {
                         RUN(ivit_layernorm_requant(h, x, M, D, D, b.s_ln1, b.n1_bias_int, b.n1_sc, b.n1_dy, a8));
                         return ivit_linear_i8_qkv_planned(h, m->plans[4 * i], a8, q, k, vt, B, T, H, dh, ldv);
                     }));
        if (tail) {
            ctx8 = patches;
            RUN(vit_attention(m, h, i, q, k, vt, ctx8, B, ldv, true, x, patch16));
            x = patch16;
        } else if (m->fused_attention) {
            RUN(vit_attention(m, h, i, q, k, vt, ctx8, B, ldv, false, nullptr, nullptr));
        } else {
            int8_t *s8 = (int8_t *)(ws + L.s8);
            uint16_t *p16 = (uint16_t *)(ws + L.p16);
            RUN(ivit_attn_qk_requant(h, q, k, b.dy_qk, s8, B * H, T, dh, ld));
            RUN(ivit_shiftmax(h, s8, (int64_t)B * H * T, T, ld, b.s_softmax, 16, p16, ld));
            RUN(ivit_attn_pv_requant(h, p16, vt, b.dy_pv, ctx8, B, H, T, dh, ld, ld));
        }
        const bool mlp_fast = mlp_plan_fuses(m->mlp_plans[i], b.res2_main, b.res2_res, Mb);
        const bool ln_lockstep = ln_mlp_plan_fuses(h, m->mlp_plans[i], b.res2_main, b.res2_res, Mb) == LN_MLP_LOCKSTEP;
        RUN(ivit_linear_i8_requant_residual_planned(h, m->plans[4 * i + 1], ctx8, b.res1_main, b.res1_res, x, y, Mb));
        { int16_t *t = x; x = y; y = t; }
        const int8_t *tab = gelu_table(m, i);
        RUN(fused_or(mlp_fast ? ivit_layernorm_mlp_fused_planned(h, m->mlp_plans[i], x, b.s_ln2, b.n2_bias_int, b.n2_sc, b.n2_dy, a8, tab, b.res2_main,
                                                                 b.res2_res, y, Mb)
                              : IVIT_ERR_UNSUPPORTED,
                     [&] {
                         return fused_or(ln_lockstep ? ivit_layernorm_mlp_lockstep_planned(h, m->mlp_plans[i], x, b.s_ln2, b.n2_bias_int, b.n2_sc,
                                                                                           b.n2_dy, tab, b.res2_main, b.res2_res, y, Mb)
                                                     : IVIT_ERR_UNSUPPORTED,
                                         [&] {
                                             RUN(ivit_layernorm_requant(h, x, Mb, D, D, b.s_ln2, b.n2_bias_int, b.n2_sc, b.n2_dy, a8));
                                             if (mlp_fast)
                                                 return ivit_mlp_fused_planned(h, m->mlp_plans[i], a8, tab, b.res2_main, b.res2_res, x, y, Mb);
                                             RUN(ivit_linear_i8_requant_planned(h, m->plans[4 * i + 2], a8, 8, h8, Mb));
                                             RUN(ivit_shiftgelu_requant_lut(h, h8, Mb, Hd, tab, g8));
                                             return ivit_linear_i8_requant_residual_planned(h, m->plans[4 * i + 3], g8, b.res2_main, b.res2_res, x, y, Mb);
                                         });
                     }));
        { int16_t *t = x; x = y; y = t; }
    }
    RUN(ivit_layernorm_requant(h, x, B, D, cls_tail(m) ? (int64_t)D : (int64_t)T * D, P.s_ln, P.n_bias_int, P.n_sc, P.n_dy, cls8));
    RUN(ivit_linear_i8(h, cls8, P.head_w, P.head_b, logits, B, c.num_classes, D));
    return IVIT_OK;
}

}

extern "C" {

int ivit_vit_create(ivit_handle h, const ivit_vit_config *cfg, const ivit_vit_params *params, int max_slices,
                    ivit_vit *out) {
    CHECK_H(h);
    REQUIRE(h, cfg && params && out && params->blocks_host, "null argument");
    REQUIRE(h, cfg->depth > 0 && cfg->embed_dim > 0 && cfg->num_heads > 0 && cfg->embed_dim % cfg->num_heads == 0 &&
                   cfg->patch_size > 0 && cfg->img_size % cfg->patch_size == 0 && cfg->hidden_dim > 0 &&
                   cfg->num_classes > 0 && cfg->in_chans > 0,
            "bad model configuration");
    REQUIRE(h, max_slices >= 1 && max_slices <= 16, "max_slices must be in [1, 16]");
    ivit_vit_s *m = new (std::nothrow) ivit_vit_s();
    if (!m) return IVIT_ERR_HIP;
    m->h = h;
    m->cfg = *cfg;
    m->prm = *params;
    m->blocks.assign(params->blocks_host, params->blocks_host + cfg->depth);
    m->prm.blocks_host = m->blocks.data();
    const int g = cfg->img_size / cfg->patch_size;
    m->num_patches = g * g;
    m->T = m->num_patches + 1;
    m->ld = (m->T + 15) / 16 * 16;
    m->Kp = cfg->in_chans * cfg->patch_size * cfg->patch_size;
    m->fused_attention = (cfg->embed_dim / cfg->num_heads == 64) && m->T <= 640;
    m->gelu_tab = nullptr;
    m->rowtab = nullptr;
    m->has_rowtab.assign(cfg->depth, 0);
    m->max_slices = max_slices;
    hipError_t e = hipMalloc((void **)&m->gelu_tab, (size_t)cfg->depth * 65536);
    if (e == hipSuccess && m->fused_attention) e = hipMalloc((void **)&m->rowtab, (size_t)cfg->depth * 256 * 64 * sizeof(float));
    if (e != hipSuccess) {
        snprintf(h->err, sizeof(h->err), "ivit_vit_create: hipMalloc: %s", hipGetErrorString(e));
        delete m;
        return IVIT_ERR_HIP;
    }
    for (int i = 0; i < cfg->depth; ++i) {
        int rc = ivit_shiftgelu_build_table(h, m->blocks[i].s_gelu, m->blocks[i].dy_gelu, gelu_table(m, i));
        if (rc != IVIT_OK) { ivit_vit_destroy(m); return rc; }
        const ivit_vit_block &b = m->blocks[i];
        if (m->rowtab && b.exp_aq && 1 - b.exp_dmin <= 64 && attn_fast(b.dy_qk, b.dy_pv)) {
            rc = ivit_shiftmax_rowtable(h, b.exp_aq, b.exp_t, b.exp_cls, b.exp_nc, b.exp_tcount, b.exp_dmin, m->rowtab + (size_t)i * 256 * 64);
            if (rc != IVIT_OK) { ivit_vit_destroy(m); return rc; }
            m->has_rowtab[i] = 1;
        }
        const int D = cfg->embed_dim, Hd = cfg->hidden_dim;
        const struct { const int8_t *w; const int32_t *bias; const ivit_dyadic *dy; int N, K; } lin[4] = {
            {b.qkv_w, b.qkv_b, b.qkv_dy, 3 * D, D}, {b.proj_w, b.proj_b, b.proj_dy, D, D},
            {b.fc1_w, b.fc1_b, b.fc1_dy, Hd, D}, {b.fc2_w, b.fc2_b, b.fc2_dy, D, Hd}};
        for (int k = 0; k < 4; ++k) {
            ivit_linear_plan pl = nullptr;
            rc = ivit_linear_plan_create(h, lin[k].w, lin[k].bias, lin[k].dy, lin[k].N, lin[k].K, &pl);
            if (rc != IVIT_OK) { ivit_vit_destroy(m); return rc; }
            if (k == 0 && ws_width(D) && D / cfg->num_heads == 64) (void)ivit_linear_plan_prepare_ws(h, pl);
            if (k == 1 && ws_width(D)) (void)ivit_linear_plan_prepare_ws(h, pl);
            m->plans.push_back(pl);
        }
        ivit_mlp_plan mp = nullptr;
        if (mlp_plan_shape(D, Hd) && ivit_mlp_plan_create(h, m->plans[4 * i + 2], m->plans[4 * i + 3], &mp) != IVIT_OK) mp = nullptr;
        m->mlp_plans.push_back(mp);
    }
    if (!m->run.create(h, max_slices)) {
        snprintf(h->err, sizeof(h->err), "ivit_vit_create: stream/event creation failed");
        ivit_vit_destroy(m);
        return IVIT_ERR_HIP;
    }
    *out = m;
    return IVIT_OK;
}

int ivit_vit_destroy(ivit_vit m) {
    if (!m) return IVIT_ERR_INVALID;
    m->run.destroy();
    if (m->gelu_tab) (void)hipFree(m->gelu_tab);
    if (m->rowtab) (void)hipFree(m->rowtab);
    for (auto mp : m->mlp_plans) if (mp) (void)ivit_mlp_plan_destroy(mp);
    for (auto pl : m->plans) (void)ivit_linear_plan_destroy(pl);
    delete m;
    return IVIT_OK;
}

int ivit_vit_workspace_bytes(ivit_vit m, int batch, int nslices, size_t *bytes) {
    if (!m) return IVIT_ERR_INVALID;
    REQUIRE(m->h, bytes && batch > 0 && nslices >= 1 && nslices <= m->max_slices && nslices <= batch, "bad arguments");
    *bytes = slice_layout(m, max_slice(batch, nslices)).total * (size_t)nslices;
    return IVIT_OK;
}

int ivit_vit_fused_mlp_blocks(ivit_vit m, int batch, int *blocks) {
    if (!m) return IVIT_ERR_INVALID;
    REQUIRE(m->h, blocks && batch > 0, "bad arguments");
    int n = 0;
    for (int i = 0; i < m->cfg.depth; ++i)
        n += mlp_plan_fuses(m->mlp_plans[i], m->blocks[i].res2_main, m->blocks[i].res2_res, (long long)batch * m->T);
    *blocks = n;
    return IVIT_OK;
}

int ivit_vit_fused_ln_mlp_blocks(ivit_vit m, int batch, int *blocks) {
    if (!m) return IVIT_ERR_INVALID;
    REQUIRE(m->h, blocks && batch > 0, "bad arguments");
    int n = 0;
    for (int i = 0; i < m->cfg.depth; ++i) {
        const bool tail = i == m->cfg.depth - 1 && cls_tail(m);
        n += ln_mlp_plan_fuses(m->h, m->mlp_plans[i], m->blocks[i].res2_main, m->blocks[i].res2_res, tail ? batch : (long long)batch * m->T) !=
             LN_MLP_TWO_LAUNCHES;
// ... 394 lines not shown
```

### include/ivit.h

```cpp
#ifndef IVIT_H
#define IVIT_H

#include <stddef.h>
#include <stdint.h>

#ifdef __cplusplus
extern "C" {
#endif

typedef struct ivit_ctx *ivit_handle;

typedef struct ivit_dyadic {
    double m;
    double r;
} ivit_dyadic;

enum {
    IVIT_OK = 0,
    IVIT_ERR_INVALID = 1,
    IVIT_ERR_HIP = 2,
    IVIT_ERR_UNSUPPORTED = 3,
    IVIT_ERR_NO_DEVICE = 4
};

#define IVIT_VERSION 111
int ivit_version(void);
const char *ivit_status_string(int status);

int ivit_create(ivit_handle *out, int device, void *hip_stream);
int ivit_destroy(ivit_handle h);
int ivit_set_stream(ivit_handle h, void *hip_stream);
int ivit_set_cu_share(ivit_handle h, int cus);
const char *ivit_last_error(ivit_handle h);

int ivit_quantize_input_f32(ivit_handle h, const float *x, float scale, int8_t *q, int64_t n);
int ivit_normalize_quantize_u8(ivit_handle h, const uint8_t *hwc, int B, int H, int W, const float mean_host[3],
                               const float std_host[3], float scale, int8_t *nchw);

int ivit_resize_center_crop_u8(ivit_handle h, const uint8_t *hwc, int B, int H0, int W0, int size, int crop,
                               float *workspace, uint8_t *out_hwc);

int ivit_linear_i8(ivit_handle h, const int8_t *x, const int8_t *w, const int32_t *bias,
                   int32_t *acc, int M, int N, int K);

int ivit_linear_i8_requant(ivit_handle h, const int8_t *x, const int8_t *w, const int32_t *bias,
                           const ivit_dyadic *dy_ch, int bits, void *out, int M, int N, int K);

int ivit_linear_i8_requant_residual(ivit_handle h, const int8_t *x, const int8_t *w,
                                    const int32_t *bias, const ivit_dyadic *dy_ch,
                                    ivit_dyadic dy_main, ivit_dyadic dy_res,
                                    const int16_t *residual, int16_t *out, int M, int N, int K);

int ivit_linear_i8_qkv(ivit_handle h, const int8_t *x, const int8_t *w, const int32_t *bias,
                       const ivit_dyadic *dy_ch, int8_t *q, int8_t *k, int8_t *vt, int B, int T,
                       int H, int dh, int ldv);

int ivit_constants_upload(ivit_handle h, const void *host_blob, size_t bytes, void *device_blob);
int ivit_constants_broadcast(ivit_handle h, void *device_blob, size_t bytes, int root, void *rccl_comm);

typedef struct ivit_linear_plan_s *ivit_linear_plan;
int ivit_linear_plan_create(ivit_handle h, const int8_t *w, const int32_t *bias, const ivit_dyadic *dy_ch, int N, int K,
                            ivit_linear_plan *out);
int ivit_linear_plan_destroy(ivit_linear_plan p);
int ivit_linear_plan_query(ivit_linear_plan p, int *pipelined_ok, int *single_fma_ok);
int ivit_linear_i8_requant_planned(ivit_handle h, ivit_linear_plan p, const int8_t *x, int bits, void *out, int M);
int ivit_linear_i8_requant_residual_planned(ivit_handle h, ivit_linear_plan p, const int8_t *x, ivit_dyadic dy_main,
                                            ivit_dyadic dy_res, const int16_t *residual, int16_t *out, int M);
int ivit_linear_i8_qkv_planned(ivit_handle h, ivit_linear_plan p, const int8_t *x, int8_t *q, int8_t *k, int8_t *vt,
                               int B, int T, int H, int dh, int ldv);
int ivit_linear_plan_prepare_ws(ivit_handle h, ivit_linear_plan p);
int ivit_layernorm_linear_i8_requant_planned(ivit_handle h, ivit_linear_plan p, const int16_t *x16, float scale,
                                             const float *bias_int, const float *sc, const ivit_dyadic *ln_dy, int8_t *out8, int M);
int ivit_linear_i8_requant_residual_layernorm_planned(ivit_handle h, ivit_linear_plan p, const int8_t *x, ivit_dyadic dy_main,
                                                      ivit_dyadic dy_res, const int16_t *residual, int16_t *out, int M,
                                                      float ln_scale, const float *ln_bias_int, const float *ln_sc,
                                                      const ivit_dyadic *ln_dy, int8_t *ln_out8);
int ivit_layernorm_linear_i8_qkv_planned(ivit_handle h, ivit_linear_plan p, const int16_t *x16, float scale,
                                         const float *bias_int, const float *sc, const ivit_dyadic *ln_dy, int8_t *q,
                                         int8_t *k, int8_t *v, int B, int T, int H, int dh);
int ivit_layernorm_linear_i8_qkv_ldv_planned(ivit_handle h, ivit_linear_plan p, const int16_t *x16, float scale,
                                             const float *bias_int, const float *sc, const ivit_dyadic *ln_dy, int8_t *q,
                                             int8_t *k, int8_t *vt, int B, int T, int H, int dh, int ldv);

int ivit_bmm_nt_i8(ivit_handle h, const int8_t *A, const int8_t *B, int32_t *C, int nb, int M,
                   int N, int K, int lda, int ldb, int ldc, int64_t strideA, int64_t strideB,
                   int64_t strideC);
int ivit_bmm_nt_u16i8(ivit_handle h, const uint16_t *A, const int8_t *B, int32_t *C, int nb,
                      int M, int N, int K, int lda, int ldb, int ldc, int64_t strideA,
                      int64_t strideB, int64_t strideC);

int ivit_attn_qk_requant(ivit_handle h, const int8_t *q, const int8_t *k, ivit_dyadic dy,
                         int8_t *scores8, int BH, int T, int dh, int lds);
int ivit_attn_pv_requant(ivit_handle h, const uint16_t *p, const int8_t *vt, ivit_dyadic dy,
                         int8_t *ctx8, int B, int H, int T, int dh, int ldp, int ldv);

int ivit_attention_fused(ivit_handle h, const int8_t *q, const int8_t *k, const int8_t *vt,
                         ivit_dyadic dy_qk, float s_softmax, ivit_dyadic dy_pv, int8_t *ctx8,
                         int B, int H, int T, int dh, int ldv);

int ivit_attention_fused_lut(ivit_handle h, const int8_t *q, const int8_t *k, const int8_t *vt,
                             ivit_dyadic dy_qk, float s_softmax, const uint16_t *exp_aq, const float *exp_t,
                             const uint8_t *exp_cls, int nclass, int t_count, int dmin, ivit_dyadic dy_pv,
                             int8_t *ctx8, int B, int H, int T, int dh, int ldv);

int ivit_shiftmax_rowtable(ivit_handle h, const uint16_t *exp_aq, const float *exp_t, const uint8_t *exp_cls,
                           int nclass, int t_count, int dmin, float *rowtab);
int ivit_attention_fused_rowlut(ivit_handle h, const int8_t *q, const int8_t *k, const int8_t *vt,
                                ivit_dyadic dy_qk, float s_softmax, const float *rowtab, int dmin, ivit_dyadic dy_pv,
                                int8_t *ctx8, int B, int H, int T, int dh, int ldv);

int ivit_attention_fused_cls(ivit_handle h, const int8_t *q, const int8_t *k, const int8_t *vt,
                             ivit_dyadic dy_qk, float s_softmax, ivit_dyadic dy_pv, int8_t *ctx_cls,
                             const int16_t *x16, int16_t *x_cls, int B, int H, int T, int dh, int ldv);
int ivit_attention_fused_lut_cls(ivit_handle h, const int8_t *q, const int8_t *k, const int8_t *vt,
                                 ivit_dyadic dy_qk, float s_softmax, const uint16_t *exp_aq, const float *exp_t,
                                 const uint8_t *exp_cls, int nclass, int t_count, int dmin, ivit_dyadic dy_pv,
                                 int8_t *ctx_cls, const int16_t *x16, int16_t *x_cls, int B, int H, int T, int dh, int ldv);
int ivit_attention_fused_rowlut_cls(ivit_handle h, const int8_t *q, const int8_t *k, const int8_t *vt,
                                    ivit_dyadic dy_qk, float s_softmax, const float *rowtab, int dmin, ivit_dyadic dy_pv,
                                    int8_t *ctx_cls, const int16_t *x16, int16_t *x_cls, int B, int H, int T, int dh, int ldv);
int ivit_gather_rows_i16(ivit_handle h, const int16_t *x, int64_t rows, int C, int64_t row_stride, int16_t *out);

int ivit_requant_i32(ivit_handle h, const int32_t *z, const ivit_dyadic *dy, int nch,
                     const int32_t *z_id, const ivit_dyadic *dy_id, int bits, void *out,
                     int64_t rows, int C);
int ivit_requant_i16(ivit_handle h, const int16_t *z, const ivit_dyadic *dy, int nch,
                     const int32_t *z_id, const ivit_dyadic *dy_id, int bits, void *out,
                     int64_t rows, int C);
int ivit_requant_f32(ivit_handle h, const float *z, const ivit_dyadic *dy, int nch,
                     const int32_t *z_id, const ivit_dyadic *dy_id, int bits, void *out,
                     int64_t rows, int C);

int ivit_shiftmax(ivit_handle h, const int8_t *x, int64_t rows, int n, int ld_in, float scale,
                  int out_bits, uint16_t *out, int ld_out);

int ivit_shiftgelu(ivit_handle h, const int8_t *x, int64_t rows, int C, float scale,
                   int16_t *out16);
int ivit_shiftgelu_requant(ivit_handle h, const int8_t *x, int64_t rows, int C, float scale,
                           ivit_dyadic dy, int8_t *out8);

int ivit_shiftgelu_build_table(ivit_handle h, float scale, ivit_dyadic dy, int8_t *table);
int ivit_shiftgelu_requant_lut(ivit_handle h, const int8_t *x, int64_t rows, int C,
                               const int8_t *table, int8_t *out8);

int ivit_layernorm(ivit_handle h, const int16_t *x, int64_t rows, int C, float scale,
                   const float *bias_int, const float *sc, float *z);
int ivit_layernorm_requant(ivit_handle h, const int16_t *x, int64_t rows, int C,
                           int64_t row_stride, float scale, const float *bias_int,
                           const float *sc, const ivit_dyadic *dy_ch, int8_t *out8);

int ivit_im2col_patch(ivit_handle h, const int8_t *img, int B, int Cin, int H, int W, int P,
                      int8_t *rows);
int ivit_embed_finish(ivit_handle h, const int16_t *patch16, const int32_t *z_cls,
                      const int16_t *pos, ivit_dyadic dy_x, ivit_dyadic dy_pos, int16_t *x16,
                      int B, int T, int D);
int ivit_patch_embed(ivit_handle h, const int8_t *images, int B, int Cin, int H, int W, int P, const int8_t *w,
                     const int32_t *bias, const ivit_dyadic *dy_ch, const int32_t *z_cls, const int16_t *pos,
                     ivit_dyadic dy_x, ivit_dyadic dy_pos, int16_t *x16, int D);

typedef struct ivit_vit_config {
    int img_size, patch_size, in_chans, embed_dim, depth, num_heads, hidden_dim, num_classes;
} ivit_vit_config;

typedef struct ivit_vit_block {
    float s_ln1; const float *n1_bias_int; const float *n1_sc; const ivit_dyadic *n1_dy;
    const int8_t *qkv_w; const int32_t *qkv_b; const ivit_dyadic *qkv_dy;
    ivit_dyadic dy_qk; float s_softmax; ivit_dyadic dy_pv;
    const uint16_t *exp_aq; const float *exp_t; const uint8_t *exp_cls;
    int exp_nc, exp_tcount, exp_dmin;
    const int8_t *proj_w; const int32_t *proj_b; const ivit_dyadic *proj_dy;
    ivit_dyadic res1_main, res1_res;
    float s_ln2; const float *n2_bias_int; const float *n2_sc; const ivit_dyadic *n2_dy;
    const int8_t *fc1_w; const int32_t *fc1_b; const ivit_dyadic *fc1_dy;
    float s_gelu; ivit_dyadic dy_gelu;
    const int8_t *fc2_w; const int32_t *fc2_b; const ivit_dyadic *fc2_dy;
    ivit_dyadic res2_main, res2_res;
} ivit_vit_block;

typedef struct ivit_vit_params {
    const int8_t *pe_w; const int32_t *pe_b; const ivit_dyadic *pe_dy;
    const int32_t *z_cls; const int16_t *pos; ivit_dyadic dy_x, dy_pos;
    const ivit_vit_block *blocks_host;
    float s_ln; const float *n_bias_int; const float *n_sc; const ivit_dyadic *n_dy;
    const int8_t *head_w; const int32_t *head_b;
} ivit_vit_params;

typedef struct ivit_vit_s *ivit_vit;

int ivit_vit_create(ivit_handle h, const ivit_vit_config *cfg, const ivit_vit_params *params,
                    int max_slices, ivit_vit *out);
int ivit_vit_destroy(ivit_vit m);
int ivit_vit_workspace_bytes(ivit_vit m, int batch, int nslices, size_t *bytes);
int ivit_vit_fused_mlp_blocks(ivit_vit m, int batch, int *blocks);
int ivit_vit_fused_ln_mlp_blocks(ivit_vit m, int batch, int *blocks);
int ivit_vit_fused_qkv_blocks(ivit_vit m, int batch, int *blocks);
int ivit_vit_cls_tail(ivit_vit m, int batch, int *on);
int ivit_vit_workspace_init(ivit_vit m, void *workspace, size_t bytes, int batch, int nslices);
int ivit_vit_forward(ivit_vit m, const int8_t *images, int batch, int nslices, void *workspace,
                     size_t bytes, int32_t *logits);
typedef struct ivit_graph_s *ivit_graph;
int ivit_vit_graph_create(ivit_vit m, const int8_t *images, int batch, int nslices, void *workspace,
                          size_t bytes, int32_t *logits, ivit_graph *out);
int ivit_graph_launch(ivit_graph g);
int ivit_graph_destroy(ivit_graph g);

typedef struct ivit_ln_params { const float *bias_int; const float *sc; const ivit_dyadic *dy; } ivit_ln_params;
typedef struct ivit_lin_params { const int8_t *w; const int32_t *b; const ivit_dyadic *dy; } ivit_lin_params;

typedef struct ivit_swin_config {
    int img_size, patch_size, in_chans, embed_dim, num_layers, window_size, mlp_ratio, num_classes;
    int depths[4];
    int num_heads[4];
} ivit_swin_config;

typedef struct ivit_swin_block {
    float s_in; ivit_ln_params n1;
    ivit_lin_params qkv;
    ivit_dyadic dy_qk, dy_a; const int16_t *relb;
    float s_softmax; ivit_dyadic dy_pv;
    ivit_lin_params proj;
    ivit_dyadic res1_main, res1_res;
    float s_mid; ivit_ln_params n2;
    ivit_lin_params fc1; float s_gelu; ivit_dyadic dy_gelu; ivit_lin_params fc2;
    ivit_dyadic res2_main, res2_res;
    const uint16_t *exp_aq; const float *exp_t; const uint8_t *exp_cls;
    int exp_nc, exp_tcount, exp_dmin;
} ivit_swin_block;

typedef struct ivit_swin_merge {
    float s_in; ivit_ln_params n; ivit_lin_params red;
} ivit_swin_merge;

typedef struct ivit_swin_params {
    ivit_lin_params pe; float s_bn;
    ivit_ln_params pn; const ivit_dyadic *dy_qact1;
    const ivit_swin_block *blocks_host;
    const ivit_swin_merge *merges_host;
    float s_norm_in; ivit_ln_params n;
    ivit_dyadic dy_pool;
    const int8_t *head_w; const int32_t *head_b;
    float s_pool;
} ivit_swin_params;

typedef struct ivit_swin_s *ivit_swin;
int ivit_swin_create(ivit_handle h, const ivit_swin_config *cfg, const ivit_swin_params *params,
                     int max_slices, ivit_swin *out);
int ivit_swin_destroy(ivit_swin m);
int ivit_swin_workspace_bytes(ivit_swin m, int batch, int nslices, size_t *bytes);
int ivit_swin_fused_mlp_blocks(ivit_swin m, int batch, int blocks_per_stage[4]);
int ivit_swin_forward(ivit_swin m, const int8_t *images, int batch, int nslices, void *workspace,
                      size_t bytes, int32_t *logits);
int ivit_swin_graph_create(ivit_swin m, const int8_t *images, int batch, int nslices, void *workspace,
                           size_t bytes, int32_t *logits, ivit_graph *out);

int ivit_shiftmax_masked(ivit_handle h, const int8_t *x, int64_t rows, int n, int ld_in, float scale,
                         int out_bits, const float *mask, int nW, int H, uint16_t *out, int ld_out);
int ivit_requant_i32_bcast(ivit_handle h, const int32_t *z, ivit_dyadic dy, const int32_t *z_id,
                           int64_t id_period, ivit_dyadic dy_id, int bits, void *out, int64_t total);
int ivit_avgpool_requant(ivit_handle h, const int8_t *x, int B, int L, int C, ivit_dyadic dy,
                         int8_t *out8);
int ivit_avgpool_requant_scaled(ivit_handle h, const int8_t *x, int B, int L, int C, float scale,
                                ivit_dyadic dy, int8_t *out8);
int ivit_layernorm_tokenorder(ivit_handle h, const int16_t *x, int64_t rows, int C, float scale,
                              const float *bias_int, const float *sc, int tokens_per_image, float *z);

int ivit_layernorm_tokenorder_requant(ivit_handle h, const int16_t *x, int64_t rows, int C, float scale,
                                      const float *bias_int, const float *sc, const ivit_dyadic *dy,
                                      int tokens_per_image, int8_t *out8);
int ivit_patch_norm_tokenorder(ivit_handle h, const int8_t *x8, int64_t rows, int C, float scale,
                               const float *bias_int, const float *sc, const ivit_dyadic *dy_ch,
                               ivit_dyadic dy2, int tokens_per_image, int16_t *out16);
int ivit_window_attention_fused(ivit_handle h, const int8_t *qkv, ivit_dyadic dy_qk, ivit_dyadic dy_a,
                                const int16_t *relb, float s_softmax, ivit_dyadic dy_pv, int8_t *ctx,
// ... 50 lines not shown
```

Measured before the change: 103,700 images/s.

## Add CLS-only last-block attention kernel and CLS-query QKV path

For the final transformer block, where only the CLS token output is needed, a new wave-per-head kernel computes attention for the single CLS query using sdot4 and a row softmax table, reading row-major v. A companion QKV launch (clsq) is meant to write q only for the tiles holding CLS rows, avoiding Q work for the other tokens. This cuts redundant compute in the last block. It adds another kernel variant and a fallback path when ldv is nonzero or shapes fall outside the supported range.

Result: no change. 104,600 images/s (median of 6 runs) (+0.9%).

```diff
diff --git a/i-vit_amd/_lib.py b/i-vit_amd/_lib.py
--- a/i-vit_amd/_lib.py
+++ b/i-vit_amd/_lib.py
@@ -177,6 +177,7 @@
     "ivit_linear_i8_requant_residual_layernorm_planned": [_P, _P, _P, Dyadic, Dyadic, _P, _P, _I, _F, _P, _P, _P, _P],
     "ivit_layernorm_linear_i8_qkv_planned": [_P, _P, _P, _F, _P, _P, _P, _P, _P, _P, _I, _I, _I, _I],
     "ivit_layernorm_linear_i8_qkv_ldv_planned": [_P, _P, _P, _F, _P, _P, _P, _P, _P, _P, _I, _I, _I, _I, _I],
+    "ivit_layernorm_linear_i8_qkv_clsq_planned": [_P, _P, _P, _F, _P, _P, _P, _P, _P, _P, _I, _I, _I, _I, _I],
     "ivit_bmm_nt_i8": [_P, _P, _P, _P, _I, _I, _I, _I, _I, _I, _I, _L, _L, _L],
     "ivit_bmm_nt_u16i8": [_P, _P, _P, _P, _I, _I, _I, _I, _I, _I, _I, _L, _L, _L],
     "ivit_attn_qk_requant": [_P, _P, _P, Dyadic, _P, _I, _I, _I, _I],
@@ -188,6 +189,7 @@
     "ivit_attention_fused_cls": [_P, _P, _P, _P, Dyadic, _F, Dyadic, _P, _P, _P, _I, _I, _I, _I, _I],
     "ivit_attention_fused_lut_cls": [_P, _P, _P, _P, Dyadic, _F, _P, _P, _P, _I, _I, _I, Dyadic, _P, _P, _P, _I, _I, _I, _I, _I],
     "ivit_attention_fused_rowlut_cls": [_P, _P, _P, _P, Dyadic, _F, _P, _I, Dyadic, _P, _P, _P, _I, _I, _I, _I, _I],
+    "ivit_attention_cls_rowlut": [_P, _P, _P, _P, Dyadic, _F, _P, _I, Dyadic, _P, _P, _P, _I, _I, _I, _I],
     "ivit_gather_rows_i16": [_P, _P, _L, _I, _L, _P],
     "ivit_requant_i32": [_P, _P, _P, _I, _P, _P, _I, _P, _L, _I],
     "ivit_requant_f32": [_P, _P, _P, _I, _P, _P, _I, _P, _L, _I],
@@ -228,6 +230,8 @@
                         "there is no CPU fallback for the product path")
     lib = ctypes.CDLL(SO_PATH)
     for name, args in SIGNATURES.items():
+        if os.environ.get("IVIT_LIB") and not hasattr(lib, name):
+            continue
         fn = getattr(lib, name)
         fn.argtypes = args
         fn.restype = ctypes.c_int
diff --git a/i-vit_amd/csrc/ivit_attention_cls.h b/i-vit_amd/csrc/ivit_attention_cls.h
--- /dev/null
+++ b/i-vit_amd/csrc/ivit_attention_cls.h
@@ -0,0 +1,135 @@
+#pragma once
+#include "ivit_device.h"
+
+#define ATC_WAVES 4
+#define ATC_TILES 16
+#define ATC_TMAX 640
+#define ATC_LINE (ATC_TMAX + 16)
+
+struct AttnClsArgs {
+    const int8_t *q, *k, *v;
+    int8_t *ctx;
+    const float *rowtab;
+    const int16_t *x16;
+    int16_t *x_cls;
+    int BH, T, H, dmin;
+    double c_qk, c_pv;
+};
+
+__global__ __launch_bounds__(ATC_WAVES * 64) void attn_cls_wave_kernel(AttnClsArgs p) {
+    __shared__ __attribute__((aligned(16))) int sline[ATC_WAVES][ATC_LINE];
+    const int lane = threadIdx.x & 63, wave = __builtin_amdgcn_readfirstlane(threadIdx.x >> 6);
+    const int bh = blockIdx.x * ATC_WAVES + wave;
+    if (bh >= p.BH) return;
+    const int T = p.T, b = bh / p.H, h = bh - b * p.H;
+    const int cg = lane & 3, kq = lane >> 2;
+    const int8_t *kg = p.k + (long long)bh * T * 64 + cg * 16;
+    const int8_t *vg = p.v + (long long)bh * T * 64 + cg * 16;
+    int *line = sline[wave];
+    const int ntile = (T + 15) >> 4;
+
+    const bool idl = p.x16 && lane >= 8 && lane < 16;
+    v4i idrow = {0, 0, 0, 0};
+    if (idl) idrow = *reinterpret_cast<const v4i *>(p.x16 + (long long)b * T * (p.H * 64) + h * 64 + (lane - 8) * 8);
+    const v4i qf = *reinterpret_cast<const v4i *>(p.q + (long long)bh * T * 64 + cg * 16);
+
+    v4i vreg[ATC_TILES];
+    int vmax = -128;
+    for (int j0 = 0; j0 < ntile; j0 += ATC_TILES) {
+        v4i kreg[ATC_TILES];
+#pragma unroll
+        for (int jj = 0; jj < ATC_TILES; ++jj) {
+            const int t = (j0 + jj) * 16 + kq;
+            kreg[jj] = v4i{0, 0, 0, 0};
+            if (t < T) kreg[jj] = *reinterpret_cast<const v4i *>(kg + t * 64);
+        }
+        if (j0 + ATC_TILES >= ntile) {
+#pragma unroll
+            for (int jj = 0; jj < ATC_TILES; ++jj) {
+                const int t = jj * 16 + kq;
+                vreg[jj] = v4i{0, 0, 0, 0};
+                if (t < T) vreg[jj] = *reinterpret_cast<const v4i *>(vg + t * 64);
+            }
+        }
+#pragma unroll
+        for (int jj = 0; jj < ATC_TILES; ++jj) {
+            const int t = (j0 + jj) * 16 + kq;
+            int s = 0;
+#pragma unroll
+            for (int w = 0; w < 4; ++w) s = __builtin_amdgcn_sdot4(kreg[jj][w], qf[w], s, false);
+            s += __shfl_xor(s, 1);
+            s += __shfl_xor(s, 2);
+            const int v = min(max(rq_fast(s, p.c_qk), -128), 127);
+            if (t < T) {
+                vmax = max(vmax, v);
+                if (cg == 0) line[t] = v;
+            }
+        }
+    }
+#pragma unroll
+    for (int m = 4; m < 64; m <<= 1) vmax = max(vmax, __shfl_xor(vmax, m));
+    __builtin_amdgcn_fence(__ATOMIC_RELEASE, "wavefront");
+    __builtin_amdgcn_wave_barrier();
+    __builtin_amdgcn_fence(__ATOMIC_ACQUIRE, "wavefront");
+
+    {
+        const float *tl = p.rowtab + (vmax + 128) * 64;
+        for (int t = lane; t < T; t += 64) line[t] = __float_as_int(tl[max(line[t] - vmax, p.dmin) - p.dmin]);
+    }
+    __builtin_amdgcn_fence(__ATOMIC_RELEASE, "wavefront");
+    __builtin_amdgcn_wave_barrier();
+    __builtin_amdgcn_fence(__ATOMIC_ACQUIRE, "wavefront");
+    const float S = torch_order_sum32(T, lane & 31, [&](int i) { return __int_as_float(line[i]); });
+    const float F16 = recip_factor(S) * 1.52587890625e-05f;
+
+    int acc[16];
+#pragma unroll
+    for (int c = 0; c < 16; ++c) acc[c] = 0;
+    for (int j0 = 0; j0 < ntile; j0 += ATC_TILES) {
+        if (j0 > 0) {
+#pragma unroll
+            for (int jj = 0; jj < ATC_TILES; ++jj) {
+                const int t = (j0 + jj) * 16 + kq;
+                vreg[jj] = v4i{0, 0, 0, 0};
+                if (t < T) vreg[jj] = *reinterpret_cast<const v4i *>(vg + t * 64);
+            }
+        }
+#pragma unroll
+        for (int jj = 0; jj < ATC_TILES; ++jj) {
+            if (j0 + jj < ntile) {
+                const int t = (j0 + jj) * 16 + kq;
+                const int P = t < T ? (int)(__int_as_float(line[t]) * F16) : 0;
+#pragma unroll
+                for (int w = 0; w < 4; ++w)
+#pragma unroll
+                    for (int bb = 0; bb < 4; ++bb) acc[4 * w + bb] += __mul24(P, (int)(signed char)(vreg[jj][w] >> (8 * bb)));
+            }
+        }
+    }
+    int r8[8], r4[4], r2[2];
+#pragma unroll
+    for (int i = 0; i < 8; ++i) {
+        const bool up = lane & 32;
+        r8[i] = (up ? acc[8 + i] : acc[i]) + __shfl_xor(up ? acc[i] : acc[8 + i], 32);
+    }
+#pragma unroll
+    for (int i = 0; i < 4; ++i) {
+        const bool up = lane & 16;
+        r4[i] = (up ? r8[4 + i] : r8[i]) + __shfl_xor(up ? r8[i] : r8[4 + i], 16);
+    }
+#pragma unroll
+    for (int i = 0; i < 2; ++i) {
+        const bool up = lane & 8;
+        r2[i] = (up ? r4[2 + i] : r4[i]) + __shfl_xor(up ? r4[i] : r4[2 + i], 8);
+    }
+    const bool up = lane & 4;
+    const int o = (up ? r2[1] : r2[0]) + __shfl_xor(up ? r2[0] : r2[1], 4);
+    const int ch = 16 * cg + ((lane >> 5) & 1) * 8 + ((lane >> 4) & 1) * 4 + ((lane >> 3) & 1) * 2 + ((lane >> 2) & 1);
+    reinterpret_cast<signed char *>(line + ATC_TMAX)[ch] = (signed char)min(max(rq_fast(o, p.c_pv), -128), 127);
+    __builtin_amdgcn_fence(__ATOMIC_RELEASE, "wavefront");
+    __builtin_amdgcn_wave_barrier();
+    __builtin_amdgcn_fence(__ATOMIC_ACQUIRE, "wavefront");
+    if (lane < 4)
+        *reinterpret_cast<v4i *>(p.ctx + (long long)b * (p.H * 64) + h * 64 + lane * 16) = *reinterpret_cast<const v4i *>(line + ATC_TMAX + lane * 4);
+    if (idl) *reinterpret_cast<v4i *>(p.x_cls + (long long)b * (p.H * 64) + h * 64 + (lane - 8) * 8) = idrow;
+}
diff --git a/i-vit_amd/csrc/ivit_gemm_ws.h b/i-vit_amd/csrc/ivit_gemm_ws.h
--- a/i-vit_amd/csrc/ivit_gemm_ws.h
+++ b/i-vit_amd/csrc/ivit_gemm_ws.h
@@ -62,249 +62,20 @@
     }
 }
 
+__device__ __forceinline__ bool ws_cls_tile(int tile, int T, int M) {
+    const int r0 = tile * 32, c = (r0 + T - 1) / T * T;
+    return c < r0 + 32 && c < M;
+}
+
 template <class G, bool FMA, bool LN, int EPI = WS_EPI_QKV8, bool VT = false>
 __global__ __launch_bounds__(WS_THREADS, 2) void gemm_ws_qkv_kernel(WsArgs p) {
-    static_assert(!VT || (G::VT && EPI == WS_EPI_QKV8), "the v^T store form belongs to the qkv scatter of a geometry that keeps its table");
-    static_assert(!(LN && EPI == WS_EPI_RES16) || G::K == 384, "norm2 in the proj launch is built at 384 only");
-    extern __shared__ __attribute__((aligned(256))) char sm[];
-    typedef double v2d __attribute__((ext_vector_type(2)));
-    typedef __attribute__((address_space(3))) char lds_c;
-    typedef __attribute__((address_space(3))) v4i lds_v4i;
-    typedef __attribute__((address_space(3))) int lds_i32;
-    typedef __attribute__((address_space(3))) unsigned lds_u32;
-    typedef __attribute__((address_space(3))) v2d lds_v2d;
-    const int wave = __builtin_amdgcn_readfirstlane(threadIdx.x >> 6);
-    const unsigned sm_lds = (unsigned)(size_t)(lds_c *)sm;
-    int tid = threadIdx.x;
-    asm volatile("" : "+v"(tid));
-    const int lane = tid & 63, tok = lane & 31, kh = lane >> 5, e = kh ^ ws_g(tok);
+    constexpr bool CLSQ = false;
+#include "ivit_gemm_ws_body.h"
+}
 
-    const int ntt = (p.M + 31) >> 5;
-    const int t_beg = (int)((long long)ntt * blockIdx.x / gridDim.x), t_end = (int)((long long)ntt * (blockIdx.x + 1) / gridDim.x);
-    const int ncp = p.N >> 6, ncp3 = ncp / 3;
-    for (int i = tid; i < p.N; i += WS_THREADS) {
-        reinterpret_cast<int *>(sm + G::SBIAS)[i] = p.bias[i];
-        reinterpret_cast<double *>(sm + G::SCQ)[i] = p.cq[i];
-    }
-    const unsigned lane16 = lane * 16;
-    double *cC = reinterpret_cast<double *>(sm + G::SLN);
-    float *cB = reinterpret_cast<float *>(sm + G::SLN + G::K * 8), *cSc = cB + G::K, *cY = cSc + G::K;
-    bool ln_fast = false;
-    constexpr bool LN_HEAD = LN && EPI != WS_EPI_RES16, LN_TAIL = LN && EPI == WS_EPI_RES16;
-    if constexpr (LN) ln_fast = ln_stage_constants<G::K, WS_THREADS>(p.ln_bias_int, p.ln_sc, p.ln_dy, cC, cB, cSc, cY);
-
-    for (int t0 = t_beg; t0 < t_end; t0 += G::MAXT) {
-        const int n_own = min(G::MAXT, t_end - t0);
-        if (t0 != t_beg) __syncthreads();
-        if constexpr (LN_HEAD) {
-            typedef LnGroup<G::K, 2> LG;
-            const int j = lane & 7, k = j >> 1, hh = j & 1;
-            const float ys = rcp_rn(p.ln_s);
-            for (int r0 = wave * 8; r0 < n_own * 32; r0 += 64) {
-                const int tokl = r0 + (lane >> 3);
-                const long long row_raw = (long long)t0 * 32 + tokl;
-                const bool live = row_raw < p.M;
-                const int16_t *xp = p.x16 + (live ? row_raw : (long long)p.M - 1) * G::K + 8 * k + 4 * hh;
-                float xv[LG::NSTEP][LG::EPC];
-#pragma unroll
-                for (int i = 0; i < LG::NSTEP; ++i) {
-                    const LnRaw<4>::T t = *reinterpret_cast<const LnRaw<4>::T *>(xp + 32 * i);
-#pragma unroll
-                    for (int c = 0; c < 4; ++c) xv[i][c] = requotient_m((float)t[c], p.ln_s, ys);
-                }
-                const unsigned rowa = sm_lds + tokl * 64 + (k & 1) * 8 + 4 * hh, gk = (unsigned)((k >> 1) ^ ws_g(tokl));
-                LG::run(xv, j, k, 8 * k + 4 * hh, ln_fast, live, cC, cB, cSc, cY,
-                       [&](int i, unsigned pk0, unsigned) __attribute__((always_inline)) {
-                           *(lds_u32 *)(size_t)(rowa + (i >> 1) * G::KBLK + ((gk ^ ((i & 1) * 2)) << 4)) = pk0;
-                       });
-            }
-        } else {
-            for (int tg = wave; tg < n_own * 2; tg += 8) {
-                const int tokl = tg * 16 + (lane >> 2), c = (lane & 3) ^ ws_g(tokl);
-                const long long grow = min((long long)t0 * 32 + tokl, (long long)p.M - 1);
-                const int8_t *src = p.x + grow * G::K + c * 16;
-#pragma unroll
-                for (int kb = 0; kb < G::KB; ++kb) {
-                    const unsigned dst = __builtin_amdgcn_readfirstlane((unsigned)(kb * G::KBLK + tg * 1024));
-                    __builtin_amdgcn_global_load_lds((const __attribute__((address_space(1))) void *)(src + kb * 64),
-                                                     (__attribute__((address_space(3))) void *)(sm + dst), 16, 0, 0);
-                }
-            }
-        }
-        if (tid < G::TOK) {
-            const int row = min(t0 * 32 + tid, p.M - 1), b = row / p.T;
-            reinterpret_cast<int *>(sm + G::SOFF)[tid] = (b * p.H * p.T + (row - b * p.T)) * 64;
-            if constexpr (VT) reinterpret_cast<int *>(sm + G::SVOFF)[tid] = b * p.H * 64 * p.ldv + (row - b * p.T);
-        }
-        const int na = (n_own + 1) >> 1, ntask = n_own > 1 ? 2 * ncp : ncp;
-        asm volatile("s_waitcnt vmcnt(0)" ::: "memory");
-        __syncthreads();
-
-        const unsigned fa0 = sm_lds + tok * 64 + e * 16, fa1 = sm_lds + tok * 64 + (e ^ 2) * 16;
-        for (int task = wave; task < ntask; task += 8) {
-            const int half = task >= ncp, cp = task - half * ncp;
-            const int tb0 = half ? na : 0, te = half ? n_own : na;
-            v4i W[2][G::KS];
-            {
-                const char *wq = reinterpret_cast<const char *>(p.wf + (size_t)cp * 2 * G::KS * 64);
-#pragma unroll
-                for (int c = 0; c < 2; ++c)
-#pragma unroll
-                    for (int ks = 0; ks < G::KS; ++ks) W[c][ks] = *reinterpret_cast<const v4i *>(wq + lane16 + (c * G::KS + ks) * 1024);
-            }
-            const int chb = 64 * cp + 16 * kh;
-            const int which = EPI == WS_EPI_QKV8 ? cp / max(ncp3, 1) : 0;
-            int8_t *obase = (which == 0 ? p.q : which == 1 ? p.k : p.v) + (size_t)(cp - which * ncp3) * p.T * 64 + 16 * kh;
-            const bool vslab = VT && which == 2;
-            int8_t *vbase = VT ? p.v + (size_t)((cp - 2 * ncp3) * 64 + 16 * kh) * p.ldv : nullptr;
-            auto sweep = [&](auto nt_c, const int tb) __attribute__((always_inline)) {
-                constexpr int NT = decltype(nt_c)::value;
-                v4i bf[2][NT];
-                v16i acc[2][NT];
-                const unsigned fb0 = fa0 + tb * 2048, fb1 = fa1 + tb * 2048;
-                int toff[NT];
-#pragma unroll
-                for (int t = 0; t < NT; ++t)
-                    toff[t] = *(lds_i32 *)(size_t)(sm_lds + (vslab ? G::SVOFF : G::SOFF) + ((tb + t) * 32 + tok) * 4);
-                auto load_b = [&](int ks, int slot) __attribute__((always_inline)) {
-#pragma unroll
-                    for (int t = 0; t < NT; ++t)
-                        bf[slot][t] = *(lds_v4i *)(size_t)(((ks & 1) ? fb1 : fb0) + (ks >> 1) * G::KBLK + t * 2048);
-                };
-                load_b(0, 0);
-                v4i idr[EPI == WS_EPI_RES16 ? 2 : 1][EPI == WS_EPI_RES16 ? NT : 1][2];
-                if constexpr (EPI == WS_EPI_RES16) {
-#pragma unroll
-                    for (int c = 0; c < 2; ++c)
-#pragma unroll
-                        for (int t = 0; t < NT; ++t) {
-                            const long long row = min((long long)(t0 + tb + t) * 32 + tok, (long long)p.M - 1);
-                            const int16_t *rp = p.residual + row * p.N + chb + 32 * c;
-                            idr[c][t][0] = *reinterpret_cast<const v4i *>(rp);
-                            idr[c][t][1] = *reinterpret_cast<const v4i *>(rp + 8);
-                        }
-                }
-#pragma unroll
-                for (int c = 0; c < 2; ++c)
-#pragma unroll
-                    for (int q4 = 0; q4 < 4; ++q4) {
-                        const v4i b4 = *(lds_v4i *)(size_t)(sm_lds + G::SBIAS + (chb + 32 * c + 4 * q4) * 4);
-#pragma unroll
-                        for (int t = 0; t < NT; ++t) { acc[c][t][4 * q4] = b4[0]; acc[c][t][4 * q4 + 1] = b4[1]; acc[c][t][4 * q4 + 2] = b4[2]; acc[c][t][4 * q4 + 3] = b4[3]; }
-                    }
-#pragma unroll
-                for (int ks = 0; ks < G::KS; ++ks) {
-                    __builtin_amdgcn_sched_barrier(0);
-                    if (ks + 1 < G::KS) load_b(ks + 1, (ks + 1) & 1);
-                    __builtin_amdgcn_sched_barrier(0);
-#pragma unroll
-                    for (int c = 0; c < 2; ++c)
-#pragma unroll
-                        for (int t = 0; t < NT; ++t)
-                            acc[c][t] = __builtin_amdgcn_mfma_i32_32x32x32_i8(W[c][ks], bf[ks & 1][t], acc[c][t], 0, 0, 0);
-                }
-#pragma unroll
-                for (int c = 0; c < 2; ++c) {
-                    v2d cqv[8];
-#pragma unroll
-                    for (int j = 0; j < 8; ++j) cqv[j] = *(lds_v2d *)(size_t)(sm_lds + G::SCQ + (chb + 32 * c + 2 * j) * 8);
-#pragma unroll
-                    for (int t = 0; t < NT; ++t) {
-                        if constexpr (EPI == WS_EPI_RES16) {
-                            v4i o0, o1;
-#pragma unroll
-                            for (int d = 0; d < 8; ++d) {
-                                const unsigned rw = (unsigned)(d < 4 ? idr[c][t][0][d] : idr[c][t][1][d - 4]);
-                                int o[2];
-#pragma unroll
-                                for (int h2 = 0; h2 < 2; ++h2) {
-                                    const int v = 2 * d + h2;
-                                    const double m = cqv[v >> 1][v & 1];
-                                    const double tq = FMA ? __builtin_fma((double)acc[c][t][v], m, WS_MAGIC) : ((double)acc[c][t][v] * m + WS_MAGIC);
-                                    const int t16 = min(max(__double2loint(tq), -32768), 32767);
-                                    const int r = h2 ? ((int)rw >> 16) : (int)(short)(rw & 0xffffu);
-                                    o[h2] = rq_fast(r, p.cr) + rq_fast(t16, p.cm);
-                                }
-                                int pk;
-                                asm("v_cvt_pk_i16_i32 %0, %1, %2" : "=v"(pk) : "v"(o[0]), "v"(o[1]));
-                                if (d < 4) o0[d] = pk; else o1[d - 4] = pk;
-                            }
-                            asm volatile("" : "+v"(o0), "+v"(o1));
-                            const long long row = (long long)(t0 + tb + t) * 32 + tok;
-                            if (row < p.M) {
-                                int16_t *op = p.out16 + row * p.N + chb + 32 * c;
-                                *reinterpret_cast<v4i *>(op) = o0;
-                                *reinterpret_cast<v4i *>(op + 8) = o1;
-                            }
-                            continue;
-                        }
-                        v4i o4;
-#pragma unroll
-                        for (int q4 = 0; q4 < 4; ++q4) {
-                            int o[4];
-#pragma unroll
-                            for (int i = 0; i < 4; ++i) {
-                                const double m = cqv[2 * q4 + (i >> 1)][i & 1];
-                                const double tq = FMA ? __builtin_fma((double)acc[c][t][4 * q4 + i], m, WS_MAGIC + 128.0)
-                                                      : ((double)acc[c][t][4 * q4 + i] * m + (WS_MAGIC + 128.0));
-                                o[i] = __double2loint(tq);
-                            }
-                            unsigned p01, p23, b01, b23;
-                            asm("v_cvt_pk_i16_i32 %0, %1, %2" : "=v"(p01) : "v"(o[0]), "v"(o[1]));
-                            asm("v_cvt_pk_i16_i32 %0, %1, %2" : "=v"(p23) : "v"(o[2]), "v"(o[3]));
-                            asm("v_sat_pk_u8_i16 %0, %1" : "=v"(b01) : "v"(p01));
-                            asm("v_sat_pk_u8_i16 %0, %1" : "=v"(b23) : "v"(p23));
-                            int hq = (int)(__builtin_amdgcn_perm(b23, b01, 0x05040100u) ^ 0x80808080u);
-                            asm volatile("" : "+v"(hq));
-                            o4[q4] = hq;
-                        }
-                        const int row = (t0 + tb + t) * 32 + tok;
-                        if constexpr (EPI == WS_EPI_RQ8) {
-                            if (row < p.M) *reinterpret_cast<v4i *>(p.q + (long long)row * p.N + chb + 32 * c) = o4;
-                        } else if (vslab) {
-                            if (row < p.M) {
-                                int8_t *vp = vbase + toff[t] + (size_t)(32 * c) * p.ldv;
-#pragma unroll
-                                for (int i = 0; i < 16; ++i) vp[(size_t)i * p.ldv] = (int8_t)(o4[i >> 2] >> (8 * (i & 3)));
-                            }
-                        } else if constexpr (G::MAXT > 8) {
-                            if (row < p.M) *reinterpret_cast<v4i *>(obase + toff[t] + 32 * c) = o4;
-                        } else {
-                            *reinterpret_cast<v4i *>(row < p.M ? obase + toff[t] + 32 * c : (int8_t *)p.dummy + lane16) = o4;
-                        }
-                    }
-                }
-            };
-            int tb = tb0;
-            if constexpr (G::MAXT <= 8) {
-                if (te - tb > 2) { sweep(std::integral_constant<int, 2>{}, tb); tb += 2; }
-                if (te - tb == 2) sweep(std::integral_constant<int, 2>{}, tb);
-                else sweep(std::integral_constant<int, 1>{}, tb);
-            } else {
-                for (; te - tb >= 2; tb += 2) sweep(std::integral_constant<int, 2>{}, tb);
-                if (te - tb == 1) sweep(std::integral_constant<int, 1>{}, tb);
-            }
-        }
-        if constexpr (LN_TAIL) {
-            asm volatile("s_waitcnt vmcnt(0)" ::: "memory");
-            __syncthreads();
-            typedef LnGroup<G::K, 2> LG;
-            const int j = lane & 7, k = j >> 1, hh = j & 1;
-            const float ys = rcp_rn(p.ln_s);
-            for (int r0 = wave * 8; r0 < n_own * 32; r0 += 64) {
-                const long long row_raw = (long long)t0 * 32 + r0 + (lane >> 3);
-                const bool live = row_raw < p.M;
-                const long long row = live ? row_raw : (long long)p.M - 1;
-                const int16_t *xp = p.out16 + row * G::K + 8 * k + 4 * hh;
-                float xv[LG::NSTEP][LG::EPC];
-#pragma unroll
-                for (int i = 0; i < LG::NSTEP; ++i) {
-                    const LnRaw<4>::T t = *reinterpret_cast<const LnRaw<4>::T *>(xp + 32 * i);
-#pragma unroll
-                    for (int c = 0; c < 4; ++c) xv[i][c] = requotient_m((float)t[c], p.ln_s, ys);
-                }
-                LG::run(xv, j, k, 8 * k + 4 * hh, ln_fast, live, cC, cB, cSc, cY, p.ln_out8 + row * G::K + 8 * k + 4 * hh);
-            }
-        }
-    }
+template <class G, bool FMA, bool VT = false>
+__global__ __launch_bounds__(WS_THREADS, 2) void gemm_ws_qkv_clsq_kernel(WsArgs p) {
+    constexpr bool LN = true, CLSQ = true;
+    constexpr int EPI = WS_EPI_QKV8;
+#include "ivit_gemm_ws_body.h"
 }
diff --git a/i-vit_amd/csrc/ivit_gemm_ws_body.h b/i-vit_amd/csrc/ivit_gemm_ws_body.h
--- /dev/null
+++ b/i-vit_amd/csrc/ivit_gemm_ws_body.h
@@ -0,0 +1,265 @@
+    static_assert(!CLSQ || EPI == WS_EPI_QKV8, "q for the class-token rows only: the qkv scatter");
+    static_assert(!VT || (G::VT && EPI == WS_EPI_QKV8), "the v^T store form belongs to the qkv scatter of a geometry that keeps its table");
+    static_assert(!(LN && EPI == WS_EPI_RES16) || G::K == 384, "norm2 in the proj launch is built at 384 only");
+    extern __shared__ __attribute__((aligned(256))) char sm[];
+    typedef double v2d __attribute__((ext_vector_type(2)));
+    typedef __attribute__((address_space(3))) char lds_c;
+    typedef __attribute__((address_space(3))) v4i lds_v4i;
+    typedef __attribute__((address_space(3))) int lds_i32;
+    typedef __attribute__((address_space(3))) unsigned lds_u32;
+    typedef __attribute__((address_space(3))) v2d lds_v2d;
+    const int wave = __builtin_amdgcn_readfirstlane(threadIdx.x >> 6);
+    const unsigned sm_lds = (unsigned)(size_t)(lds_c *)sm;
+    int tid = threadIdx.x;
+    asm volatile("" : "+v"(tid));
+    const int lane = tid & 63, tok = lane & 31, kh = lane >> 5, e = kh ^ ws_g(tok);
+
+    const int ntt = (p.M + 31) >> 5;
+    const int t_beg = (int)((long long)ntt * blockIdx.x / gridDim.x), t_end = (int)((long long)ntt * (blockIdx.x + 1) / gridDim.x);
+    const int ncp = p.N >> 6, ncp3 = ncp / 3;
+    for (int i = tid; i < p.N; i += WS_THREADS) {
+        reinterpret_cast<int *>(sm + G::SBIAS)[i] = p.bias[i];
+        reinterpret_cast<double *>(sm + G::SCQ)[i] = p.cq[i];
+    }
+    const unsigned lane16 = lane * 16;
+    double *cC = reinterpret_cast<double *>(sm + G::SLN);
+    float *cB = reinterpret_cast<float *>(sm + G::SLN + G::K * 8), *cSc = cB + G::K, *cY = cSc + G::K;
+    bool ln_fast = false;
+    constexpr bool LN_HEAD = LN && EPI != WS_EPI_RES16, LN_TAIL = LN && EPI == WS_EPI_RES16;
+    if constexpr (LN) ln_fast = ln_stage_constants<G::K, WS_THREADS>(p.ln_bias_int, p.ln_sc, p.ln_dy, cC, cB, cSc, cY);
+
+    for (int t0 = t_beg; t0 < t_end; t0 += G::MAXT) {
+        const int n_own = min(G::MAXT, t_end - t0);
+        if (t0 != t_beg) __syncthreads();
+        if constexpr (LN_HEAD) {
+            typedef LnGroup<G::K, 2> LG;
+            int lane_ln = lane;
+            if constexpr (CLSQ) asm volatile("" : "+v"(lane_ln));
+            const int j = lane_ln & 7, k = j >> 1, hh = j & 1;
+            const float ys = rcp_rn(p.ln_s);
+            for (int r0 = wave * 8; r0 < n_own * 32; r0 += 64) {
+                const int tokl = r0 + (lane_ln >> 3);
+                const long long row_raw = (long long)t0 * 32 + tokl;
+                const bool live = row_raw < p.M;
+                const int16_t *xp = p.x16 + (live ? row_raw : (long long)p.M - 1) * G::K + 8 * k + 4 * hh;
+                float xv[LG::NSTEP][LG::EPC];
+#pragma unroll
+                for (int i = 0; i < LG::NSTEP; ++i) {
+                    const LnRaw<4>::T t = *reinterpret_cast<const LnRaw<4>::T *>(xp + 32 * i);
+#pragma unroll
+                    for (int c = 0; c < 4; ++c) xv[i][c] = requotient_m((float)t[c], p.ln_s, ys);
+                }
+                const unsigned rowa = sm_lds + tokl * 64 + (k & 1) * 8 + 4 * hh, gk = (unsigned)((k >> 1) ^ ws_g(tokl));
+                LG::run(xv, j, k, 8 * k + 4 * hh, ln_fast, live, cC, cB, cSc, cY,
+                       [&](int i, unsigned pk0, unsigned) __attribute__((always_inline)) {
+                           *(lds_u32 *)(size_t)(rowa + (i >> 1) * G::KBLK + ((gk ^ ((i & 1) * 2)) << 4)) = pk0;
+                       });
+            }
+        } else {
+            for (int tg = wave; tg < n_own * 2; tg += 8) {
+                const int tokl = tg * 16 + (lane >> 2), c = (lane & 3) ^ ws_g(tokl);
+                const long long grow = min((long long)t0 * 32 + tokl, (long long)p.M - 1);
+                const int8_t *src = p.x + grow * G::K + c * 16;
+#pragma unroll
+                for (int kb = 0; kb < G::KB; ++kb) {
+                    const unsigned dst = __builtin_amdgcn_readfirstlane((unsigned)(kb * G::KBLK + tg * 1024));
+                    __builtin_amdgcn_global_load_lds((const __attribute__((address_space(1))) void *)(src + kb * 64),
+                                                     (__attribute__((address_space(3))) void *)(sm + dst), 16, 0, 0);
+                }
+            }
+        }
+        if (tid < G::TOK) {
+            const int row = min(t0 * 32 + tid, p.M - 1), b = row / p.T;
+            reinterpret_cast<int *>(sm + G::SOFF)[tid] = (b * p.H * p.T + (row - b * p.T)) * 64;
+            if constexpr (VT) reinterpret_cast<int *>(sm + G::SVOFF)[tid] = b * p.H * 64 * p.ldv + (row - b * p.T);
+        }
+        const int na = (n_own + 1) >> 1, ntask = n_own > 1 ? 2 * ncp : ncp;
+        asm volatile("s_waitcnt vmcnt(0)" ::: "memory");
+        __syncthreads();
+
+        const unsigned fa0 = sm_lds + tok * 64 + e * 16, fa1 = sm_lds + tok * 64 + (e ^ 2) * 16;
+        for (int task = wave; task < ntask; task += 8) {
+            int half = task >= ncp, cp = task - half * ncp;
+            if constexpr (CLSQ) {
+                const int nkv = (ncp - ncp3) * (n_own > 1 ? 2 : 1), j = task < nkv ? task : task - nkv, nsl = task < nkv ? ncp - ncp3 : ncp3;
+                half = j >= nsl;
+                cp = j - half * nsl + (task < nkv ? ncp3 : 0);
+            }
+            const int tb0 = half ? na : 0, te = half ? n_own : na;
+            if constexpr (CLSQ) {
+                if (cp < ncp3) {
+                    bool any = false;
+                    for (int tb = tb0; tb < te; ++tb) any |= ws_cls_tile(t0 + tb, p.T, p.M);
+                    if (!any) continue;
+                }
+            }
+            v4i W[2][G::KS];
+            {
+                const char *wq = reinterpret_cast<const char *>(p.wf + (size_t)cp * 2 * G::KS * 64);
+#pragma unroll
+                for (int c = 0; c < 2; ++c)
+#pragma unroll
+                    for (int ks = 0; ks < G::KS; ++ks) W[c][ks] = *reinterpret_cast<const v4i *>(wq + lane16 + (c * G::KS + ks) * 1024);
+            }
+            const int chb = 64 * cp + 16 * kh;
+            const int which = EPI == WS_EPI_QKV8 ? cp / max(ncp3, 1) : 0;
+            int8_t *obase = (which == 0 ? p.q : which == 1 ? p.k : p.v) + (size_t)(cp - which * ncp3) * p.T * 64 + 16 * kh;
+            const bool vslab = VT && which == 2;
+            int8_t *vbase = VT ? p.v + (size_t)((cp - 2 * ncp3) * 64 + 16 * kh) * p.ldv : nullptr;
+            auto sweep = [&](auto nt_c, const int tb) __attribute__((always_inline)) {
+                constexpr int NT = decltype(nt_c)::value;
+                v4i bf[2][NT];
+                v16i acc[2][NT];
+                const unsigned fb0 = fa0 + tb * 2048, fb1 = fa1 + tb * 2048;
+                int toff[NT];
+#pragma unroll
+                for (int t = 0; t < NT; ++t)
+                    toff[t] = *(lds_i32 *)(size_t)(sm_lds + (vslab ? G::SVOFF : G::SOFF) + ((tb + t) * 32 + tok) * 4);
+                auto load_b = [&](int ks, int slot) __attribute__((always_inline)) {
+#pragma unroll
+                    for (int t = 0; t < NT; ++t)
+                        bf[slot][t] = *(lds_v4i *)(size_t)(((ks & 1) ? fb1 : fb0) + (ks >> 1) * G::KBLK + t * 2048);
+                };
+                load_b(0, 0);
+                v4i idr[EPI == WS_EPI_RES16 ? 2 : 1][EPI == WS_EPI_RES16 ? NT : 1][2];
+                if constexpr (EPI == WS_EPI_RES16) {
+#pragma unroll
+                    for (int c = 0; c < 2; ++c)
+#pragma unroll
+                        for (int t = 0; t < NT; ++t) {
+                            const long long row = min((long long)(t0 + tb + t) * 32 + tok, (long long)p.M - 1);
+                            const int16_t *rp = p.residual + row * p.N + chb + 32 * c;
+                            idr[c][t][0] = *reinterpret_cast<const v4i *>(rp);
+                            idr[c][t][1] = *reinterpret_cast<const v4i *>(rp + 8);
+                        }
+                }
+#pragma unroll
+                for (int c = 0; c < 2; ++c)
+#pragma unroll
+                    for (int q4 = 0; q4 < 4; ++q4) {
+                        const v4i b4 = *(lds_v4i *)(size_t)(sm_lds + G::SBIAS + (chb + 32 * c + 4 * q4) * 4);
+#pragma unroll
+                        for (int t = 0; t < NT; ++t) { acc[c][t][4 * q4] = b4[0]; acc[c][t][4 * q4 + 1] = b4[1]; acc[c][t][4 * q4 + 2] = b4[2]; acc[c][t][4 * q4 + 3] = b4[3]; }
+                    }
+#pragma unroll
+                for (int ks = 0; ks < G::KS; ++ks) {
+                    __builtin_amdgcn_sched_barrier(0);
+                    if (ks + 1 < G::KS) load_b(ks + 1, (ks + 1) & 1);
+                    __builtin_amdgcn_sched_barrier(0);
+#pragma unroll
+                    for (int c = 0; c < 2; ++c)
+#pragma unroll
+                        for (int t = 0; t < NT; ++t)
+                            acc[c][t] = __builtin_amdgcn_mfma_i32_32x32x32_i8(W[c][ks], bf[ks & 1][t], acc[c][t], 0, 0, 0);
+                }
+#pragma unroll
+                for (int c = 0; c < 2; ++c) {
+                    v2d cqv[8];
+#pragma unroll
+                    for (int j = 0; j < 8; ++j) cqv[j] = *(lds_v2d *)(size_t)(sm_lds + G::SCQ + (chb + 32 * c + 2 * j) * 8);
+#pragma unroll
+                    for (int t = 0; t < NT; ++t) {
+                        if constexpr (EPI == WS_EPI_RES16) {
+                            v4i o0, o1;
+#pragma unroll
+                            for (int d = 0; d < 8; ++d) {
+                                const unsigned rw = (unsigned)(d < 4 ? idr[c][t][0][d] : idr[c][t][1][d - 4]);
+                                int o[2];
+#pragma unroll
+                                for (int h2 = 0; h2 < 2; ++h2) {
+                                    const int v = 2 * d + h2;
+                                    const double m = cqv[v >> 1][v & 1];
+                                    const double tq = FMA ? __builtin_fma((double)acc[c][t][v], m, WS_MAGIC) : ((double)acc[c][t][v] * m + WS_MAGIC);
+                                    const int t16 = min(max(__double2loint(tq), -32768), 32767);
+                                    const int r = h2 ? ((int)rw >> 16) : (int)(short)(rw & 0xffffu);
+                                    o[h2] = rq_fast(r, p.cr) + rq_fast(t16, p.cm);
+                                }
+                                int pk;
+                                asm("v_cvt_pk_i16_i32 %0, %1, %2" : "=v"(pk) : "v"(o[0]), "v"(o[1]));
+                                if (d < 4) o0[d] = pk; else o1[d - 4] = pk;
+                            }
+                            asm volatile("" : "+v"(o0), "+v"(o1));
+                            const long long row = (long long)(t0 + tb + t) * 32 + tok;
+                            if (row < p.M) {
+                                int16_t *op = p.out16 + row * p.N + chb + 32 * c;
+                                *reinterpret_cast<v4i *>(op) = o0;
+                                *reinterpret_cast<v4i *>(op + 8) = o1;
+                            }
+                            continue;
+                        }
+                        v4i o4;
+#pragma unroll
+                        for (int q4 = 0; q4 < 4; ++q4) {
+                            int o[4];
+#pragma unroll
+                            for (int i = 0; i < 4; ++i) {
+                                const double m = cqv[2 * q4 + (i >> 1)][i & 1];
+                                const double tq = FMA ? __builtin_fma((double)acc[c][t][4 * q4 + i], m, WS_MAGIC + 128.0)
+                                                      : ((double)acc[c][t][4 * q4 + i] * m + (WS_MAGIC + 128.0));
+                                o[i] = __double2loint(tq);
+                            }
+                            unsigned p01, p23, b01, b23;
+                            asm("v_cvt_pk_i16_i32 %0, %1, %2" : "=v"(p01) : "v"(o[0]), "v"(o[1]));
+                            asm("v_cvt_pk_i16_i32 %0, %1, %2" : "=v"(p23) : "v"(o[2]), "v"(o[3]));
+                            asm("v_sat_pk_u8_i16 %0, %1" : "=v"(b01) : "v"(p01));
+                            asm("v_sat_pk_u8_i16 %0, %1" : "=v"(b23) : "v"(p23));
+                            int hq = (int)(__builtin_amdgcn_perm(b23, b01, 0x05040100u) ^ 0x80808080u);
+                            asm volatile("" : "+v"(hq));
+                            o4[q4] = hq;
+                        }
+                        const int row = (t0 + tb + t) * 32 + tok;
+                        if constexpr (EPI == WS_EPI_RQ8) {
+                            if (row < p.M) *reinterpret_cast<v4i *>(p.q + (long long)row * p.N + chb + 32 * c) = o4;
+                        } else if (vslab) {
+                            if (row < p.M) {
+                                int8_t *vp = vbase + toff[t] + (size_t)(32 * c) * p.ldv;
+#pragma unroll
+                                for (int i = 0; i < 16; ++i) vp[(size_t)i * p.ldv] = (int8_t)(o4[i >> 2] >> (8 * (i & 3)));
+                            }
+                        } else if constexpr (G::MAXT > 8) {
+                            if (row < p.M) *reinterpret_cast<v4i *>(obase + toff[t] + 32 * c) = o4;
+                        } else {
+                            *reinterpret_cast<v4i *>(row < p.M ? obase + toff[t] + 32 * c : (int8_t *)p.dummy + lane16) = o4;
+                        }
+                    }
+                }
+            };
+            int tb = tb0;
+            if constexpr (CLSQ) {
+                if (which == 0) {
+                    for (; tb < te; ++tb)
+                        if (ws_cls_tile(t0 + tb, p.T, p.M)) sweep(std::integral_constant<int, 1>{}, tb);
+                    continue;
+                }
+            }
+            if constexpr (G::MAXT <= 8) {
+                if (te - tb > 2) { sweep(std::integral_constant<int, 2>{}, tb); tb += 2; }
+                if (te - tb == 2) sweep(std::integral_constant<int, 2>{}, tb);
+                else sweep(std::integral_constant<int, 1>{}, tb);
+            } else {
+                for (; te - tb >= 2; tb += 2) sweep(std::integral_constant<int, 2>{}, tb);
+                if (te - tb == 1) sweep(std::integral_constant<int, 1>{}, tb);
+            }
+        }
+        if constexpr (LN_TAIL) {
+            asm volatile("s_waitcnt vmcnt(0)" ::: "memory");
+            __syncthreads();
+            typedef LnGroup<G::K, 2> LG;
+            const int j = lane & 7, k = j >> 1, hh = j & 1;
+            const float ys = rcp_rn(p.ln_s);
+            for (int r0 = wave * 8; r0 < n_own * 32; r0 += 64) {
+                const long long row_raw = (long long)t0 * 32 + r0 + (lane >> 3);
+                const bool live = row_raw < p.M;
+                const long long row = live ? row_raw : (long long)p.M - 1;
+                const int16_t *xp = p.out16 + row * G::K + 8 * k + 4 * hh;
+                float xv[LG::NSTEP][LG::EPC];
+#pragma unroll
+                for (int i = 0; i < LG::NSTEP; ++i) {
+                    const LnRaw<4>::T t = *reinterpret_cast<const LnRaw<4>::T *>(xp + 32 * i);
+#pragma unroll
+                    for (int c = 0; c < 4; ++c) xv[i][c] = requotient_m((float)t[c], p.ln_s, ys);
+                }
+                LG::run(xv, j, k, 8 * k + 4 * hh, ln_fast, live, cC, cB, cSc, cY, p.ln_out8 + row * G::K + 8 * k + 4 * hh);
+            }
+        }
+    }
diff --git a/i-vit_amd/csrc/ivit_hip.hip b/i-vit_amd/csrc/ivit_hip.hip
--- a/i-vit_amd/csrc/ivit_hip.hip
+++ b/i-vit_amd/csrc/ivit_hip.hip
@@ -13,6 +13,7 @@
 #include "ivit_layernorm.h"
 #include "ivit_gemm.h"
 #include "ivit_attention.h"
+#include "ivit_attention_cls.h"
 #include "ivit_gemm2.h"
 #include "ivit_gemm3.h"
 #include "ivit_gemm_wreg.h"
@@ -539,18 +540,20 @@
         return false;
     return ldv == 0 || (pl->K == Ws192Geo::K && ldv >= T && ldv % 16 == 0 && (long long)B * H * 64 * ldv < (1ll << 31));
 }
-template <class G, bool LN, int EPI, bool VT = false>
+template <class G, bool LN, int EPI, bool VT = false, bool CLSQ = false>
 static int ws_launch(ivit_handle h, const ivit_linear_plan_s *pl, const WsArgs &a) {
+    static_assert(!CLSQ || (LN && EPI == WS_EPI_QKV8), "the class-token q form is built with the LayerNorm head on the qkv scatter");
     const int ntt = (a.M + 31) / 32;
     const unsigned grid = (unsigned)(ntt < persistent_cus(h) ? ntt : persistent_cus(h));
     return with_bool(pl->single_fma_ok, [&](auto FMA) {
-        return launch_dyn<gemm_ws_qkv_kernel<G, FMA(), LN, EPI, VT>>(h, grid, WS_THREADS, G::SMEM, a);
+        if constexpr (CLSQ) return launch_dyn<gemm_ws_qkv_clsq_kernel<G, FMA(), VT>>(h, grid, WS_THREADS, G::SMEM, a);
+        else return launch_dyn<gemm_ws_qkv_kernel<G, FMA(), LN, EPI, VT>>(h, grid, WS_THREADS, G::SMEM, a);
     });
 }
 template <class G>
 static int launch_qkv_ws_g(ivit_handle h, const ivit_linear_plan_s *pl, const int8_t *x8, const int16_t *x16, float ln_s,
                            const float *ln_bias_int, const float *ln_sc, const ivit_dyadic *ln_dy, int8_t *q, int8_t *k, int8_t *v,
-                           int B, int T, int H, int ldv) {
+                           int B, int T, int H, int ldv, bool clsq) {
     if (h->device != pl->device) { snprintf(h->err, sizeof(h->err), "qkv: plan and handle live on different devices"); return IVIT_ERR_INVALID; }
     if (ldv != 0 && !G::VT) { snprintf(h->err, sizeof(h->err), "qkv: no v^T store form at K = %d", G::K); return IVIT_ERR_UNSUPPORTED; }
     WsArgs a;
@@ -560,6 +563,14 @@
     a.residual = nullptr; a.out16 = nullptr; a.cm = a.cr = 0.0; a.ln_out8 = nullptr; a.ldv = ldv;
     if (H == 0) { a.T = 1; a.H = 1; }
     const int st = with_bool(x16 != nullptr, [&](auto LN) {
+        if constexpr (LN()) {
+            if (clsq && H != 0) {
+                if constexpr (G::VT) {
+                    if (ldv != 0) return ws_launch<G, true, WS_EPI_QKV8, true, true>(h, pl, a);
+                }
+                return ws_launch<G, true, WS_EPI_QKV8, false, true>(h, pl, a);
+            }
+        }
         if (H == 0) return ws_launch<G, LN(), WS_EPI_RQ8>(h, pl, a);
         if constexpr (G::VT) {
             if (ldv != 0) return ws_launch<G, LN(), WS_EPI_QKV8, true>(h, pl, a);
@@ -572,9 +583,9 @@
 }
 static int launch_qkv_ws(ivit_handle h, const ivit_linear_plan_s *pl, const int8_t *x8, const int16_t *x16, float ln_s,
                          const float *ln_bias_int, const float *ln_sc, const ivit_dyadic *ln_dy, int8_t *q, int8_t *k, int8_t *v,
-                         int B, int T, int H, int ldv = 0) {
-    return pl->K == Ws192Geo::K ? launch_qkv_ws_g<Ws192Geo>(h, pl, x8, x16, ln_s, ln_bias_int, ln_sc, ln_dy, q, k, v, B, T, H, ldv)
-                                : launch_qkv_ws_g<Ws384Geo>(h, pl, x8, x16, ln_s, ln_bias_int, ln_sc, ln_dy, q, k, v, B, T, H, ldv);
+                         int B, int T, int H, int ldv = 0, bool clsq = false) {
+    return pl->K == Ws192Geo::K ? launch_qkv_ws_g<Ws192Geo>(h, pl, x8, x16, ln_s, ln_bias_int, ln_sc, ln_dy, q, k, v, B, T, H, ldv, clsq)
+                                : launch_qkv_ws_g<Ws384Geo>(h, pl, x8, x16, ln_s, ln_bias_int, ln_sc, ln_dy, q, k, v, B, T, H, ldv, clsq);
 }
 
 template <class G>
@@ -743,6 +754,21 @@
     return launch_qkv_ws(h, pl, nullptr, x16, scale, bias_int, sc, ln_dy, q, k, vt, B, T, H, ldv);
 }
 
+int ivit_layernorm_linear_i8_qkv_clsq_planned(ivit_handle h, ivit_linear_plan pl, const int16_t *x16, float scale, const float *bias_int,
+                                              const float *sc, const ivit_dyadic *ln_dy, int8_t *q, int8_t *k, int8_t *vt, int B, int T,
+                                              int H, int dh, int ldv) {
+    CHECK_H(h);
+    REQUIRE(h, pl && x16 && bias_int && sc && ln_dy && q && k && vt && B > 0 && T > 0 && H > 0 && dh > 0, "bad arguments");
+    REQUIRE(h, pl->N == 3 * H * dh && pl->K == H * dh, "plan shape is not [3*H*dh, H*dh]");
+    REQUIRE(h, ldv == 0 || (ldv >= T && ldv % 16 == 0), "ldv: 0 (v row-major [B*H, T, dh]) or a multiple of 16 >= T (v^T)");
+    if (!qkv_ws_ok(pl, B, T, H, dh, ldv)) {
+        snprintf(h->err, sizeof(h->err), "%s: needs ivit_linear_plan_prepare_ws on a K = 192 or 384, dh = 64 plan, B*H*T*64 < 2^31, and K = 192 "
+                                         "with B*H*64*ldv < 2^31 for v^T", __func__);
+        return IVIT_ERR_UNSUPPORTED;
+    }
+    return launch_qkv_ws(h, pl, nullptr, x16, scale, bias_int, sc, ln_dy, q, k, vt, B, T, H, ldv, true);
+}
+
 }
 
 struct ivit_mlp_plan_s {
@@ -1091,6 +1117,36 @@
                                                float s_softmax, const float *rowtab, int dmin, ivit_dyadic dy_pv, int8_t *ctx_cls,
                                                const int16_t *x16, int16_t *x_cls, int B, int H, int T, int dh, int ldv) {
     return attention_rowlut(h, q, k, vt, dy_qk, s_softmax, rowtab, dmin, dy_pv, ctx_cls, B, H, T, dh, ldv, true, x16, x_cls);
+}
+
+extern "C" int ivit_attention_cls_rowlut(ivit_handle h, const int8_t *q, const int8_t *k, const int8_t *v, ivit_dyadic dy_qk, float s_softmax,
+                                         const float *rowtab, int dmin, ivit_dyadic dy_pv, int8_t *ctx_cls, const int16_t *x16,
+                                         int16_t *x_cls, int B, int H, int T, int dh) {
+    CHECK_H(h);
+    REQUIRE(h, q && k && v && ctx_cls && B > 0 && H > 0 && T > 0 && s_softmax > 0.f, "bad arguments");
+    REQUIRE(h, rowtab && ((uintptr_t)rowtab & 15) == 0 && dmin <= 0, "bad row table (16-byte aligned, dmin <= 0)");
+    REQUIRE(h, (x16 == nullptr) == (x_cls == nullptr), "x16 and x_cls go together (both null: no identity rows)");
+    REQUIRE(h, (((uintptr_t)x16 | (uintptr_t)x_cls | (uintptr_t)ctx_cls | (uintptr_t)q | (uintptr_t)k | (uintptr_t)v) & 15) == 0,
+            "q, k, v, ctx_cls, x16 and x_cls must be 16-byte aligned");
+    if (dh != 64 || T > ATC_TMAX) {
+        snprintf(h->err, sizeof(h->err), "%s: built for dh == 64, T <= %d", __func__, ATC_TMAX);
+        return IVIT_ERR_UNSUPPORTED;
+    }
+    if (1 - dmin > 64) {
+        snprintf(h->err, sizeof(h->err), "%s: a table line holds 64 entries, this scale needs %d (use ivit_attention_fused_lut_cls)", __func__, 1 - dmin);
+        return IVIT_ERR_UNSUPPORTED;
+    }
+    if (!attn_fast(dy_qk, dy_pv)) {
+        snprintf(h->err, sizeof(h->err), "%s: requant multipliers out of the fast range (use ivit_attention_fused_lut_cls)", __func__);
+        return IVIT_ERR_UNSUPPORTED;
+    }
+    AttnClsArgs a;
+    a.q = q; a.k = k; a.v = v; a.ctx = ctx_cls; a.rowtab = rowtab; a.x16 = x16; a.x_cls = x_cls;
+    a.BH = B * H; a.T = T; a.H = H; a.dmin = dmin;
+    a.c_qk = dy_qk.m * dy_qk.r; a.c_pv = dy_pv.m * dy_pv.r;
+    attn_cls_wave_kernel<<<(unsigned)((a.BH + ATC_WAVES - 1) / ATC_WAVES), ATC_WAVES * 64, 0, h->stream>>>(a);
+    LAUNCH_CHECK(h);
+    return IVIT_OK;
 }
 
 __global__ __launch_bounds__(256) void gather_rows16_kernel(const int16_t *__restrict__ x, long long row_stride, int C8, long long n,
diff --git a/i-vit_amd/csrc/ivit_model.h b/i-vit_amd/csrc/ivit_model.h
--- a/i-vit_amd/csrc/ivit_model.h
+++ b/i-vit_amd/csrc/ivit_model.h
@@ -163,8 +163,14 @@
     const int T = m->T, H = m->cfg.num_heads, dh = m->cfg.embed_dim / H;
     if (m->has_rowtab[i]) {
         const float *rowtab = m->rowtab + (size_t)i * 256 * 64;
-        return cls ? ivit_attention_fused_rowlut_cls(h, q, k, vt, b.dy_qk, b.s_softmax, rowtab, b.exp_dmin, b.dy_pv, ctx, x16, x_cls, B, H, T, dh, ldv)
-                   : ivit_attention_fused_rowlut(h, q, k, vt, b.dy_qk, b.s_softmax, rowtab, b.exp_dmin, b.dy_pv, ctx, B, H, T, dh, ldv);
+        if (cls)
+            return fused_or(ldv == 0 ? ivit_attention_cls_rowlut(h, q, k, vt, b.dy_qk, b.s_softmax, rowtab, b.exp_dmin, b.dy_pv, ctx, x16, x_cls, B, H, T, dh)
+                                     : IVIT_ERR_UNSUPPORTED,
+                            [&] {
+                                return ivit_attention_fused_rowlut_cls(h, q, k, vt, b.dy_qk, b.s_softmax, rowtab, b.exp_dmin, b.dy_pv, ctx, x16, x_cls,
+                                                                       B, H, T, dh, ldv);
+                            });
+        return ivit_attention_fused_rowlut(h, q, k, vt, b.dy_qk, b.s_softmax, rowtab, b.exp_dmin, b.dy_pv, ctx, B, H, T, dh, ldv);
     }
     if (b.exp_aq)
         return cls ? ivit_attention_fused_lut_cls(h, q, k, vt, b.dy_qk, b.s_softmax, b.exp_aq, b.exp_t, b.exp_cls, b.exp_nc, b.exp_tcount, b.exp_dmin,
@@ -198,8 +204,8 @@
         const int ldv = (m->fused_attention && m->has_rowtab[i]) ? 0 : ld;
         const bool tail = i == c.depth - 1 && cls_tail(m);
         const int Mb = tail ? B : M;
-        RUN(fused_or(qkv_plan_fuses(m, i, B) ? ivit_layernorm_linear_i8_qkv_ldv_planned(h, m->plans[4 * i], x, b.s_ln1, b.n1_bias_int, b.n1_sc, b.n1_dy,
-                                                                                        q, k, vt, B, T, H, dh, ldv)
+        RUN(fused_or(qkv_plan_fuses(m, i, B) ? (tail ? ivit_layernorm_linear_i8_qkv_clsq_planned : ivit_layernorm_linear_i8_qkv_ldv_planned)(
+                                                   h, m->plans[4 * i], x, b.s_ln1, b.n1_bias_int, b.n1_sc, b.n1_dy, q, k, vt, B, T, H, dh, ldv)
                                              : IVIT_ERR_UNSUPPORTED,
                      [&] {
                          RUN(ivit_layernorm_requant(h, x, M, D, D, b.s_ln1, b.n1_bias_int, b.n1_sc, b.n1_dy, a8));
diff --git a/include/ivit.h b/include/ivit.h
--- a/include/ivit.h
+++ b/include/ivit.h
@@ -81,6 +81,9 @@
 int ivit_layernorm_linear_i8_qkv_ldv_planned(ivit_handle h, ivit_linear_plan p, const int16_t *x16, float scale,
                                              const float *bias_int, const float *sc, const ivit_dyadic *ln_dy, int8_t *q,
                                              int8_t *k, int8_t *vt, int B, int T, int H, int dh, int ldv);
+int ivit_layernorm_linear_i8_qkv_clsq_planned(ivit_handle h, ivit_linear_plan p, const int16_t *x16, float scale,
+                                              const float *bias_int, const float *sc, const ivit_dyadic *ln_dy, int8_t *q,
+                                              int8_t *k, int8_t *vt, int B, int T, int H, int dh, int ldv);
 
 int ivit_bmm_nt_i8(ivit_handle h, const int8_t *A, const int8_t *B, int32_t *C, int nb, int M,
                    int N, int K, int lda, int ldb, int ldc, int64_t strideA, int64_t strideB,
@@ -119,6 +122,9 @@
 int ivit_attention_fused_rowlut_cls(ivit_handle h, const int8_t *q, const int8_t *k, const int8_t *vt,
                                     ivit_dyadic dy_qk, float s_softmax, const float *rowtab, int dmin, ivit_dyadic dy_pv,
                                     int8_t *ctx_cls, const int16_t *x16, int16_t *x_cls, int B, int H, int T, int dh, int ldv);
+int ivit_attention_cls_rowlut(ivit_handle h, const int8_t *q, const int8_t *k, const int8_t *v,
+                              ivit_dyadic dy_qk, float s_softmax, const float *rowtab, int dmin, ivit_dyadic dy_pv,
+                              int8_t *ctx_cls, const int16_t *x16, int16_t *x_cls, int B, int H, int T, int dh);
 int ivit_gather_rows_i16(ivit_handle h, const int16_t *x, int64_t rows, int C, int64_t row_stride, int16_t *out);
 
 int ivit_requant_i32(ivit_handle h, const int32_t *z, const ivit_dyadic *dy, int nch,
```
